# Lzcstan/DrugLAMP

Hardware: AMD Instinct MI355X
Metric: drug-protein pairs/sec training step (higher is better)
Workload: dtype bf16; 1 GPU; DrugLAMP training step (cls step, epoch 1; fwd+bwd+grad all-reduce+AdamW), BindingDB-shaped synthetic pairs (512 drug nodes/tokens, 2304 protein tokens = 256 sites, pre-extracted 384-d/640-d LLM embeddings), global batch 256 = 256 per GPU x 1; per_gpu_batch=256, global_batch=256, parallelism=dp1, step_kind=cls, epoch=1, hip_graph=False, protein_seq_len=2304, distinct_batches=8, first_touch_steps=8, padding_rows=computed once, protein_cnn_rows=distinct rows, streams=independent branches on side HIP streams

## Files before the change

### druglamp_amd/_lib.py

```python
from __future__ import annotations

import ctypes as C
import os

import torch

_HERE = os.path.dirname(os.path.abspath(__file__))
_variant = os.environ.get("DL_USE_STUDY_LIB", "")
if _variant and not _variant.endswith(".so"):
    raise RuntimeError("DL_USE_STUDY_LIB=%s: the -DDL_STUDY build (libdruglamp_hip_study.so) was removed; commit 97fb613 is the last "
                       "that builds it (python -m druglamp_amd.build --study).  Only a variant library name (libdruglamp_hip_<variant>.so) "
                       "is accepted." % _variant)
LIB_PATH = os.path.join(_HERE, "lib", _variant or "libdruglamp_hip.so")

DL_F32, DL_BF16 = 0, 1

c_i64, c_i32, c_f32, c_u64, c_vp, c_sz = C.c_int64, C.c_int32, C.c_float, C.c_uint64, C.c_void_p, C.c_size_t


class ReduceItem(C.Structure):
    _fields_ = [
        ("kind", c_i32), ("out_dtype", c_i32),
        ("src", c_vp), ("out", c_vp),
        ("mn", c_i64), ("ldc", c_i64),
        ("N", c_i32), ("splits", c_i32), ("accumulate", c_i32), ("M", c_i32),
        ("cs_slabs", c_vp), ("cs_out", c_vp),
    ]


REDUCE_BATCH_MAX = 24
GEMM_GROUP_MAX = 16


class GemmArgs(C.Structure):
    _fields_ = [
        ("X", c_vp), ("ldx", c_i64), ("x_kslow", c_i32),
        ("W", c_vp), ("ldw", c_i64), ("w_kslow", c_i32),
        ("C", c_vp), ("ldc", c_i64),
        ("M", c_i64), ("N", c_i64), ("K", c_i64),
        ("in_dtype", c_i32), ("out_dtype", c_i32),
        ("bias", c_vp),
        ("residual", c_vp), ("ldr", c_i64),
        ("res_row_mod", c_i64),
        ("res_before_dropout", c_i32),
        ("act", c_i32),
        ("pre_out", c_vp), ("ldp", c_i64),
        ("dact_pre", c_vp), ("lddp", c_i64),
        ("dropout_p", c_f32), ("dropout_seed", c_u64),
        ("accumulate", c_i32),
        ("split_k", c_i32), ("workspace", c_vp), ("workspace_bytes", c_sz),
        ("x_colsum", c_vp),
        ("dropout_seed_offset", c_vp),
        ("algo", c_i32),
        ("tile_tickets", c_vp),
        ("deferred", C.POINTER(ReduceItem)),
        ("prof_tag", c_i32),
    ]


FLAG_PROT_PERIOD, FLAG_DRUG_TOKEN_PAD, FLAG_GCN_NODE_PAD, FLAG_PLAN_ROWS, FLAG_PAIR_INDEX = 1, 2, 4, 8, 16
FLAG_KEY_TABLE = 32
TAG_OTHER, TAG_QKV_OUT, TAG_FFN, TAG_CONV, TAG_WGRAD, TAG_ADAPTOR = 0, 1, 2, 3, 4, 5
TAG_NAMES = {0: "other", 1: "qkv_out", 2: "ffn", 3: "conv", 4: "wgrad", 5: "adaptor"}


class AttnFwdArgs(C.Structure):
    _fields_ = [
        ("Q", c_vp), ("K", c_vp), ("V", c_vp), ("O", c_vp), ("LSE", c_vp), ("raw_logits", c_vp),
        ("q_ps", c_i64), ("q_hs", c_i64), ("q_rs", c_i64),
        ("k_ps", c_i64), ("k_hs", c_i64), ("k_rs", c_i64),
        ("v_ps", c_i64), ("v_hs", c_i64), ("v_rs", c_i64),
        ("o_ps", c_i64), ("o_hs", c_i64), ("o_rs", c_i64), ("o_ss", c_i64),
        ("n_problems", c_i32), ("n_heads", c_i32), ("n_segments", c_i32), ("partner_shift", c_i32),
        ("Lq", c_i32), ("Lk", c_i32), ("head_dim", c_i32), ("dtype", c_i32),
        ("scale", c_f32),
        ("algo", c_i32),
        ("key_tail_rows", c_i32), ("key_tail_weight", c_f32),
    ]


class AttnBwdArgs(C.Structure):
    _fields_ = [
        ("Q", c_vp), ("K", c_vp), ("V", c_vp), ("O", c_vp), ("dO", c_vp),
        ("LSE", c_vp), ("Delta", c_vp),
        ("dQ", c_vp), ("dK", c_vp), ("dV", c_vp),
        ("q_ps", c_i64), ("q_hs", c_i64), ("q_rs", c_i64),
        ("k_ps", c_i64), ("k_hs", c_i64), ("k_rs", c_i64),
        ("v_ps", c_i64), ("v_hs", c_i64), ("v_rs", c_i64),
        ("o_ps", c_i64), ("o_hs", c_i64), ("o_rs", c_i64), ("o_ss", c_i64),
        ("do_ps", c_i64), ("do_hs", c_i64), ("do_rs", c_i64), ("do_ss", c_i64),
        ("dq_ps", c_i64), ("dq_hs", c_i64), ("dq_rs", c_i64),
        ("dk_ps", c_i64), ("dk_hs", c_i64), ("dk_rs", c_i64),
        ("dv_ps", c_i64), ("dv_hs", c_i64), ("dv_rs", c_i64),
        ("n_problems", c_i32), ("n_heads", c_i32), ("n_segments", c_i32), ("partner_shift", c_i32),
        ("Lq", c_i32), ("Lk", c_i32), ("head_dim", c_i32), ("dtype", c_i32),
        ("scale", c_f32),
        ("algo", c_i32),
        ("key_tail_rows", c_i32), ("key_tail_weight", c_f32),
    ]


class AttnProbsArgs(C.Structure):
    _fields_ = [
        ("Q", c_vp), ("K", c_vp), ("LSE", c_vp), ("out", c_vp), ("out_ld", c_i64),
        ("q_ps", c_i64), ("q_hs", c_i64), ("q_rs", c_i64),
        ("k_ps", c_i64), ("k_hs", c_i64), ("k_rs", c_i64),
        ("n_problems", c_i32), ("n_heads", c_i32), ("n_segments", c_i32), ("partner_shift", c_i32),
        ("Lq", c_i32), ("Lk", c_i32), ("head_dim", c_i32), ("dtype", c_i32),
        ("scale", c_f32),
        ("head_mean", c_i32), ("key_tail_rows", c_i32), ("key_tail_weight", c_f32), ("expand_tail", c_i32),
        ("workspace", c_vp), ("workspace_bytes", c_sz),
    ]


class PgcaPairsArgs(C.Structure):
    _fields_ = [
        ("Q", c_vp), ("K", c_vp), ("V", c_vp), ("left", c_vp), ("out", c_vp), ("bias", c_vp),
        ("q_index", c_vp), ("kv_index", c_vp), ("flags", c_vp),
        ("q_es", c_i64), ("q_rs", c_i64), ("k_es", c_i64), ("k_rs", c_i64), ("v_es", c_i64), ("v_rs", c_i64),
        ("left_es", c_i64), ("left_rs", c_i64), ("out_ps", c_i64), ("out_rs", c_i64),
        ("n_pairs", c_i32), ("n_q", c_i32), ("n_kv", c_i32), ("Lq", c_i32), ("Lk", c_i32), ("head_dim", c_i32), ("dtype", c_i32),
        ("left_cols", c_i32), ("out_col0", c_i32),
        ("scale", c_f32),
        ("key_tail_rows", c_i32), ("key_tail_weight", c_f32),
    ]


class PgcaPairsRaggedArgs(C.Structure):
    _fields_ = [
        ("Q", c_vp), ("K", c_vp), ("V", c_vp), ("left", c_vp), ("out", c_vp), ("bias", c_vp),
        ("q_index", c_vp), ("kv_index", c_vp), ("kv_row0", c_vp), ("kv_keys", c_vp), ("kv_tail_weight", c_vp), ("flags", c_vp),
        ("q_es", c_i64), ("q_rs", c_i64), ("k_rs", c_i64), ("v_rs", c_i64),
        ("left_es", c_i64), ("left_rs", c_i64), ("out_ps", c_i64), ("out_rs", c_i64), ("kv_total_rows", c_i64),
        ("n_pairs", c_i32), ("n_q", c_i32), ("n_kv", c_i32), ("Lq", c_i32), ("head_dim", c_i32), ("dtype", c_i32),
        ("left_cols", c_i32), ("out_col0", c_i32),
        ("scale", c_f32),
        ("key_tail_rows", c_i32),
    ]


class NtxentSide(C.Structure):
    _fields_ = [("q", c_vp), ("k", c_vp), ("n", c_i64), ("gid_offset", c_i64), ("lse", c_vp)]


class NtxentArgs(C.Structure):
    _fields_ = [("a", NtxentSide), ("b", NtxentSide), ("n_global", c_i64), ("d", c_i64), ("dtype", c_i32),
                ("temperature", c_f32)]


SIGNATURES = {
    "dl_last_error": (C.c_char_p, []),
    "dl_version": (c_i32, []),
    "dl_gemm_workspace_bytes": (c_sz, [C.POINTER(GemmArgs)]),
    "dl_gemm": (c_i32, [C.POINTER(GemmArgs), c_vp]),
    "dl_gemm_pair": (c_i32, [C.POINTER(GemmArgs), C.POINTER(GemmArgs), c_vp]),
    "dl_gemm_group_plan": (c_i32, [C.POINTER(GemmArgs), c_i32, C.POINTER(c_i32)]),
    "dl_gemm_group": (c_i32, [C.POINTER(GemmArgs), c_i32, c_vp]),
    "dl_reduce_batch": (c_i32, [C.POINTER(ReduceItem), c_i32, c_vp]),
    "dl_colsum": (c_i32, [c_vp, c_i64, c_i64, c_i64, c_i32, c_vp, c_i32, c_vp, c_sz, c_vp]),
    "dl_colsum_workspace_bytes": (c_sz, [c_i64, c_i64]),
    "dl_bn_workspace_bytes": (c_sz, [c_i64, c_i64]),
    "dl_bn_stats": (c_i32, [c_vp, c_i64, c_i64, c_i64, c_i64, c_i64, c_i32, c_vp, c_vp, c_sz, c_vp]),
    "dl_bn_apply_fwd": (c_i32, [c_vp, c_vp, c_vp, c_vp, c_vp, c_vp, c_i64, c_i64, c_i64, c_i64, c_i64, c_i32, c_vp]),
    "dl_bn_bwd_reduce": (c_i32, [c_vp, c_vp, c_vp, c_vp, c_i64, c_i64, c_i64, c_i64, c_i64, c_i32, c_vp, c_vp, c_sz, c_vp]),
    "dl_bn_tail_fix": (c_i32, [c_vp, c_vp, c_vp, c_vp, c_vp, c_vp, c_f32, c_i32, c_i64, c_i64, c_i64, c_i64, c_i32, c_vp]),
    "dl_bn_apply_relu_fwd": (c_i32, [c_vp, c_vp, c_vp, c_vp, c_vp, c_vp, c_i64, c_i64, c_i32, c_vp]),
    "dl_bn_relu_bwd": (c_i32, [c_vp, c_vp, c_vp, c_vp, c_vp, c_vp, c_f32, c_vp, c_vp, c_i64, c_i64, c_i32, c_vp, c_sz, c_vp]),
    "dl_bn_bwd_apply": (c_i32, [c_vp, c_vp, c_vp, c_vp, c_vp, c_vp, c_f32, c_i32, c_vp, c_i64, c_i64, c_i64, c_i64, c_i64,
                                c_i32, c_vp]),
    "dl_layernorm_fwd": (c_i32, [c_vp, c_i64, c_vp, c_vp, c_vp, c_i64, c_vp, c_vp, c_i64, c_i64, c_f32, c_i32, c_vp]),
    "dl_layernorm_bwd_workspace_bytes": (c_sz, [c_i64, c_i64]),
    "dl_layernorm_bwd": (c_i32, [c_vp, c_i64, c_i64, c_vp, c_i64, c_vp, c_vp, c_vp, c_vp, c_i64, c_vp, c_i64, c_vp, c_vp,
                                 c_i32, c_i64, c_i64, c_i32, c_vp, c_sz, C.POINTER(ReduceItem), c_vp]),
    "dl_attn_fwd": (c_i32, [C.POINTER(AttnFwdArgs), c_vp]),
    "dl_attn_bwd": (c_i32, [C.POINTER(AttnBwdArgs), c_vp]),
    "dl_attn_probs_workspace_bytes": (c_sz, [C.POINTER(AttnProbsArgs)]),
    "dl_attn_probs": (c_i32, [C.POINTER(AttnProbsArgs), c_vp]),
    "dl_pgca_pairs_fwd": (c_i32, [C.POINTER(PgcaPairsArgs), c_vp]),
    "dl_pgca_pairs_ragged_fwd": (c_i32, [C.POINTER(PgcaPairsRaggedArgs), c_vp]),
    "dl_token_gate_fwd": (c_i32, [c_vp, c_vp, c_vp, c_vp, c_i64, c_i64, c_i64, c_i32, c_i32, c_i32, c_vp]),
    "dl_token_gate_bwd": (c_i32, [c_vp, c_vp, c_vp, c_vp, c_vp, c_i64, c_i64, c_i64, c_i32, c_i32, c_i32, c_vp]),
    "dl_gate_dpre": (c_i32, [c_vp, c_vp, c_vp, c_vp, c_i64, c_i64, c_i32, c_i32, c_vp]),
    "dl_add_rowmod_dropout": (c_i32, [c_vp, c_vp, c_vp, c_i64, c_i64, c_i64, c_f32, c_u64, c_vp, c_i32, c_vp]),
    "dl_dropout_apply": (c_i32, [c_vp, c_vp, c_i64, c_i64, c_i64, c_i64, c_f32, c_u64, c_vp, c_i32, c_vp]),
    "dl_fill_pool": (c_i32, [c_vp, c_vp, c_vp, c_i64, c_i64, c_i64, c_i32, c_i32, c_i32, c_vp]),
    "dl_cnn_sitepool_fwd": (c_i32, [c_vp, c_vp, c_i64, c_i64, c_i64, c_i32, c_i32, c_i32, c_vp]),
    "dl_cnn_sitepool_bwd": (c_i32, [c_vp, c_vp, c_i64, c_i64, c_i64, c_i32, c_i32, c_i32, c_vp]),
    "dl_bn_stats_finalize": (c_i32, [c_vp, c_i64, c_i64, c_i64, c_i64, c_i64, c_vp, c_i32, c_i64, c_f32, c_f32, c_vp, c_vp, c_vp, c_vp, c_vp, c_vp, c_vp, c_sz, c_vp]),
    "dl_bn_finalize": (c_i32, [c_vp, c_i64, c_f32, c_f32, c_vp, c_vp, c_vp, c_vp, c_vp, c_i64, c_vp]),
    "dl_interleave_streams": (c_i32, [c_vp, c_vp, c_i64, c_i64, c_i32, c_i32, c_vp]),
    "dl_norm_adjacency": (c_i32, [c_vp, c_vp, c_i64, c_i32, c_i32, c_vp]),
    "dl_graph_aggregate": (c_i32, [c_vp, c_vp, c_vp, c_i64, c_i32, c_i32, c_i32, c_i32, c_i32, c_vp]),
    "dl_concat2": (c_i32, [c_vp, c_vp, c_vp, c_i64, c_i64, c_i64, c_i32, c_vp]),
    "dl_gather_pad": (c_i32, [c_vp, c_vp, c_vp, c_vp, c_i64, c_i64, c_i64, c_i32, c_i32, c_vp]),
    "dl_embed_pad": (c_i32, [c_vp, c_vp, c_vp, c_vp, c_i64, c_i64, c_i32, c_i32, c_i32, c_i32, c_vp]),
    "dl_weight_prep": (c_i32, [c_vp, c_vp, c_i32, c_i32, c_vp]),
    "dl_gelu_bwd": (c_i32, [c_vp, c_vp, c_vp, c_i64, c_i32, c_vp]),
    "dl_cast": (c_i32, [c_vp, c_i32, c_vp, c_i32, c_i64, c_vp]),
    "dl_rowmod_sum": (c_i32, [c_vp, c_vp, c_i64, c_i64, c_i64, c_i32, c_i32, c_vp]),
    "dl_cos_rowloss_fwd": (c_i32, [c_vp, c_vp, c_vp, c_vp, c_i64, c_i64, c_vp]),
    "dl_cos_rowloss_bwd": (c_i32, [c_vp, c_vp, c_f32, c_vp, c_i64, c_i64, c_vp]),
    "dl_ntxent_fwd_ex": (c_i32, [C.POINTER(NtxentArgs), c_vp, c_vp, c_vp, c_vp]),
    "dl_ntxent_bwd_ex": (c_i32, [C.POINTER(NtxentArgs), c_f32, c_vp, c_vp, c_vp]),
    "dl_ntxent_workspace_bytes": (c_sz, [c_i64, c_i64]),
    "dl_ntxent_fwd": (c_i32, [c_vp, c_vp, c_i64, c_i64, c_f32, c_vp, c_vp, c_vp, c_sz, c_vp]),
    "dl_ntxent_bwd": (c_i32, [c_vp, c_vp, c_i64, c_i64, c_f32, c_vp, c_f32, c_vp, c_vp, c_vp]),
    "dl_triplet_sigcos_buffer_floats": (c_sz, [c_i64, c_i64]),
    "dl_triplet_sigcos_fwd": (c_i32, [c_vp, c_vp, c_vp, c_i64, c_i64, c_i64, c_f32, c_vp, c_vp, c_vp, c_vp]),
    "dl_triplet_sigcos_bwd": (c_i32, [c_vp, c_vp, c_vp, c_vp, c_i64, c_i64, c_i64, c_f32, c_vp, c_f32, c_vp, c_vp, c_vp]),
    "dl_adamw_step": (c_i32, [c_vp, c_vp, c_vp, c_vp, c_i64, c_f32, c_f32, c_f32, c_f32, c_f32, c_i64, c_f32, c_vp,
                              c_i32, c_vp]),
    "dl_bn_stats_rw": (c_i32, [c_vp, c_i64, c_i64, c_vp, c_i32, c_vp, c_vp, c_sz, c_vp]),
    "dl_bn_apply_fwd_rw": (c_i32, [c_vp, c_vp, c_vp, c_vp, c_vp, c_vp, c_i64, c_i64, c_vp, c_i32, c_vp]),
    "dl_bn_bwd_reduce_rw": (c_i32, [c_vp, c_vp, c_vp, c_vp, c_i64, c_i64, c_vp, c_i32, c_vp, c_vp, c_sz, c_vp]),
    "dl_bn_bwd_apply_rw": (c_i32, [c_vp, c_vp, c_vp, c_vp, c_vp, c_vp, c_f32, c_i32, c_vp, c_i64, c_i64, c_vp, c_i32, c_vp]),
    "dl_cnn_sitepool_rows_fwd": (c_i32, [c_vp, c_vp, c_vp, c_i64, c_i64, c_i64, c_i32, c_i32, c_vp]),
    "dl_cnn_sitepool_rows_bwd": (c_i32, [c_vp, c_vp, c_vp, c_vp, c_i64, c_i64, c_i64, c_i64, c_i32, c_i32, c_vp]),
    "dl_embed_rows": (c_i32, [c_vp, c_vp, c_vp, c_vp, c_vp, c_i64, c_i32, c_i32, c_vp, c_i64, c_i64, c_vp, c_i32, c_vp]),
    "dl_rows_gather": (c_i32, [c_vp, c_vp, c_vp, c_i64, c_i64, c_vp]),
    "dl_rows_sum_strided": (c_i32, [c_vp, c_vp, c_vp, c_i64, c_i64, c_i32, c_vp]),
    "dl_rows_equal_check": (c_i32, [c_vp, c_i64, c_i64, c_i64, c_i64, C.c_uint32, c_vp, c_vp]),
    "dl_ce_rows_workspace_bytes": (c_sz, [c_i64]),
    "dl_ce_rows_fwd": (c_i32, [c_vp, c_i64, c_vp, c_i64, c_i32, c_i64, c_i32, c_vp, c_vp, c_vp, c_sz, c_vp]),
    "dl_ce_rows_bwd": (c_i32, [c_vp, c_i64, c_vp, c_i64, c_i32, c_i64, c_i32, c_vp, c_vp, c_vp, c_vp, c_i64, c_i32, c_vp]),
    "dl_protein_plan_build": (c_i32, [c_vp, c_i64, c_i64, c_i64, c_vp, c_vp, c_vp, c_vp, c_vp, c_vp, c_vp]),
    "dl_prof_enable": (c_i32, [c_i32, c_i32]),
    "dl_prof_collect": (c_i32, [c_i32, C.POINTER(c_i64), C.POINTER(C.c_double), C.POINTER(C.c_double),
                                C.POINTER(C.c_double)]),
    "dl_prof_totals": (c_i32, [c_i32, C.POINTER(c_i64), C.POINTER(C.c_double), C.POINTER(C.c_double)]),
    "dl_prof_collect_tag": (c_i32, [c_i32, c_i32, C.POINTER(c_i64), C.POINTER(C.c_double), C.POINTER(C.c_double), C.POINTER(C.c_double),
                                    C.POINTER(c_i64), C.POINTER(C.c_double), C.POINTER(C.c_double)]),
}

_lib = None

AUDIT = os.environ.get("DL_GRAPH_PTR_AUDIT") == "1"
_audit_log = None


def audit_begin() -> None:
    global _audit_log
    _audit_log = []


def audit_end():
    global _audit_log
    log, _audit_log = _audit_log, None
    return log or []


def _struct_ptrs(obj, out, name):
    for fname, ftype in getattr(obj, "_fields_", []):
        v = getattr(obj, fname)
        if ftype is c_vp:
            if v:
                out.append(("%s.%s" % (name, fname), int(v)))
        elif isinstance(v, C.Structure):
            _struct_ptrs(v, out, "%s.%s" % (name, fname))


def _audited(name, fn, argtypes):
    def call(*args):
        if _audit_log is not None:
            import torch
            if torch.cuda.is_current_stream_capturing():
                found = []
                n_items = next((a for a, t in zip(args, argtypes) if t is c_i32), 0) if name == "dl_reduce_batch" else 0
                for i, (a, t) in enumerate(zip(args, argtypes)):
                    if t is c_vp:
                        v = a.value if isinstance(a, C.c_void_p) else a
                        if v:
                            found.append(("arg%d" % i, int(v)))
                    elif isinstance(a, C.Array):
                        for k in range(int(n_items) or len(a)):
                            _struct_ptrs(a[k], found, "arg%d[%d]" % (i, k))
                    elif isinstance(a, C.Structure):
                        _struct_ptrs(a, found, "arg%d" % i)
                    elif hasattr(a, "_obj") and isinstance(getattr(a, "_obj"), C.Structure):
                        _struct_ptrs(a._obj, found, "arg%d" % i)
                    elif hasattr(a, "contents") and a:
                        try:
                            _struct_ptrs(a.contents, found, "arg%d" % i)
                        except ValueError:
                            pass
                _audit_log.extend((name, w, v) for w, v in found)
        return fn(*args)
    return call


def lib():
    global _lib
    if _lib is None:
        if not os.path.exists(LIB_PATH):
            raise RuntimeError(
                "libdruglamp_hip.so is missing (%s). Build it with `python -m druglamp_amd.build`; "
                "the HIP hot path has no CPU fallback." % LIB_PATH)
        L = C.CDLL(LIB_PATH)
        for name, (res, args) in SIGNATURES.items():
            fn = getattr(L, name)
            fn.restype = res
            fn.argtypes = args
            if AUDIT and name not in ("dl_last_error", "dl_version") and not name.endswith("_bytes") and not name.endswith("_floats") \
                    and not name.startswith("dl_prof_"):
                setattr(L, name, _audited(name, fn, args))
        _lib = L
    return _lib


_DEBUG_SYNC = bool(os.environ.get("DL_DEBUG_SYNC"))


def check(rc: int, what: str = "") -> None:
    if _DEBUG_SYNC:
        import sys
        import torch
        print("[dl] %s" % what, file=sys.stderr, flush=True)
        torch.cuda.synchronize()
        print("[dl-ok] %s" % what, file=sys.stderr, flush=True)
    if rc != 0:
        msg = lib().dl_last_error()
        raise RuntimeError("druglamp_hip %s failed (status %d): %s" % (what, rc, msg.decode() if msg else "?"))
```

### druglamp_amd/csrc/norm.hip

```cpp
#include "common.cuh"

namespace {
constexpr int LN_MAXV = 8;
constexpr int LN_BWD_ROWS = 32;

constexpr int LN_FWD_RPW = 2;
template <typename T, int NV_>
__global__ __launch_bounds__(256) void ln_fwd_kernel(const T* __restrict__ x, int64_t ldx,
                                                     const float* __restrict__ gamma,
                                                     const float* __restrict__ beta, T* __restrict__ y,
                                                     int64_t ldy, float* __restrict__ mean_out,
                                                     float* __restrict__ rstd_out, int64_t M, int D,
                                                     float eps) {
  const int lane = threadIdx.x & 63, wave = threadIdx.x >> 6;
  const int64_t row0 = ((int64_t)blockIdx.x * 4 + wave) * LN_FWD_RPW;
  if (row0 >= M) return;
  const int nv = D >> 2;
  f32x4 v[LN_FWD_RPW][NV_];
#pragma unroll
  for (int r = 0; r < LN_FWD_RPW; ++r)
#pragma unroll
    for (int j = 0; j < NV_; ++j) {
      const int c = lane + 64 * j;
      v[r][j] = f32x4{0.f, 0.f, 0.f, 0.f};
      if (c < nv && row0 + r < M) v[r][j] = load4<T>(x + (row0 + r) * ldx + c * 4);
    }
  f32x4 gm[NV_], bt[NV_];
#pragma unroll
  for (int j = 0; j < NV_; ++j) {
    const int c = lane + 64 * j;
    gm[j] = bt[j] = f32x4{0.f, 0.f, 0.f, 0.f};
    if (c < nv) { gm[j] = *reinterpret_cast<const f32x4*>(gamma + c * 4); bt[j] = *reinterpret_cast<const f32x4*>(beta + c * 4); }
  }
#pragma unroll
  for (int r = 0; r < LN_FWD_RPW; ++r) {
    const int64_t row = row0 + r;
    if (row >= M) break;
    float s = 0.f;
#pragma unroll
    for (int j = 0; j < NV_; ++j) s += (v[r][j][0] + v[r][j][1]) + (v[r][j][2] + v[r][j][3]);
    const float mean = wave_sum(s) / (float)D;
    float q = 0.f;
#pragma unroll
    for (int j = 0; j < NV_; ++j) {
      const int c = lane + 64 * j;
      if (c < nv) {
#pragma unroll
        for (int e = 0; e < 4; ++e) { const float d = v[r][j][e] - mean; q += d * d; }
      }
    }
    const float var = wave_sum(q) / (float)D;
    const float rstd = rsqrtf(var + eps);
#pragma unroll
    for (int j = 0; j < NV_; ++j) {
      const int c = lane + 64 * j;
      if (c < nv) {
        f32x4 o;
#pragma unroll
        for (int e = 0; e < 4; ++e) o[e] = (v[r][j][e] - mean) * rstd * gm[j][e] + bt[j][e];
        store4<T>(y + row * ldy + c * 4, o);
      }
    }
    if (lane == 0) {
      if (mean_out) mean_out[row] = mean;
      if (rstd_out) rstd_out[row] = rstd;
    }
  }
}

template <typename T, int NV_>
__global__ __launch_bounds__(256) void ln_bwd_kernel(const T* __restrict__ dy, int64_t lddy, int64_t dy_share,
                                                     const T* __restrict__ x, int64_t ldx,
                                                     const float* __restrict__ mean,
                                                     const float* __restrict__ rstd,
                                                     const float* __restrict__ gamma,
                                                     const T* __restrict__ dres, int64_t lddres,
                                                     T* __restrict__ dx, int64_t lddx,
                                                     float* __restrict__ partial, int64_t M, int D) {
  extern __shared__ __attribute__((aligned(16))) char ln_smem[];
  float* sm = reinterpret_cast<float*>(ln_smem);
  const int lane = threadIdx.x & 63, wave = threadIdx.x >> 6;
  const int nv = D >> 2;
  f32x4 gm[NV_], dg[NV_], db[NV_];
#pragma unroll
  for (int j = 0; j < NV_; ++j) {
    const int c = lane + 64 * j;
    dg[j] = f32x4{0.f, 0.f, 0.f, 0.f};
    db[j] = f32x4{0.f, 0.f, 0.f, 0.f};
    gm[j] = (c < nv) ? *reinterpret_cast<const f32x4*>(gamma + c * 4) : f32x4{0.f, 0.f, 0.f, 0.f};
  }
  const int64_t r0 = (int64_t)blockIdx.x * LN_BWD_ROWS;
  for (int rr = wave; rr < LN_BWD_ROWS; rr += 8) {
    const int64_t rowA = r0 + rr, rowB = r0 + rr + 4;
    if (rowA >= M) break;
    const bool hasB = rowB < M;
    const int64_t dyA = dy_share == 1 ? rowA : rowA / dy_share, dyB = dy_share == 1 ? rowB : rowB / dy_share;
    f32x4 xa[NV_], da[NV_], xb[NV_], db_[NV_], ra[NV_], rb[NV_];
#pragma unroll
    for (int j = 0; j < NV_; ++j) {
      const int c = lane + 64 * j;
      ra[j] = f32x4{0.f, 0.f, 0.f, 0.f}; rb[j] = ra[j];
      if (c < nv) {
        xa[j] = load4<T>(x + rowA * ldx + c * 4);
        da[j] = load4<T>(dy + dyA * lddy + c * 4);
        if (dres) ra[j] = load4<T>(dres + rowA * lddres + c * 4);
        if (hasB) {
          xb[j] = load4<T>(x + rowB * ldx + c * 4);
          db_[j] = load4<T>(dy + dyB * lddy + c * 4);
          if (dres) rb[j] = load4<T>(dres + rowB * lddres + c * 4);
        }
      }
    }
#pragma unroll
    for (int half = 0; half < 2; ++half) {
      if (half == 1 && !hasB) break;
      const int64_t row = half == 0 ? rowA : rowB;
      const float mu = mean[row], rs = rstd[row];
      f32x4 xh[NV_], g[NV_];
      float c1 = 0.f, c2 = 0.f;
#pragma unroll
      for (int j = 0; j < NV_; ++j) {
        const int c = lane + 64 * j;
        if (c < nv) {
          const f32x4 xv = half == 0 ? xa[j] : xb[j];
          const f32x4 dv = half == 0 ? da[j] : db_[j];
#pragma unroll
          for (int e = 0; e < 4; ++e) {
            xh[j][e] = (xv[e] - mu) * rs;
            g[j][e] = dv[e] * gm[j][e];
            c1 += g[j][e];
            c2 += g[j][e] * xh[j][e];
            dg[j][e] += dv[e] * xh[j][e];
            db[j][e] += dv[e];
          }
        }
      }
      c1 = wave_sum(c1) / (float)D;
      c2 = wave_sum(c2) / (float)D;
#pragma unroll
      for (int j = 0; j < NV_; ++j) {
        const int c = lane + 64 * j;
        if (c < nv) {
          f32x4 o;
#pragma unroll
          for (int e = 0; e < 4; ++e) o[e] = rs * (g[j][e] - c1 - xh[j][e] * c2);
          o += half == 0 ? ra[j] : rb[j];
          store4<T>(dx + row * lddx + c * 4, o);
        }
      }
    }
  }
#pragma unroll
  for (int j = 0; j < NV_; ++j) {
    const int c = lane + 64 * j;
    if (c < nv) {
      *reinterpret_cast<f32x4*>(sm + (wave * 2 + 0) * D + c * 4) = dg[j];
      *reinterpret_cast<f32x4*>(sm + (wave * 2 + 1) * D + c * 4) = db[j];
    }
  }
  __syncthreads();
  for (int i = threadIdx.x; i < 2 * D; i += 256) {
    const int which = i / D, col = i % D;
    float s = 0.f;
#pragma unroll
    for (int w = 0; w < 4; ++w) s += sm[(w * 2 + which) * D + col];
    partial[((int64_t)blockIdx.x * 2 + which) * D + col] = s;
  }
}

template <int LPR> __device__ __forceinline__ float seg_sum(float v) {
  v = row16_sum(v);
  const float lo = lane_f32(v, 0) + lane_f32(v, 16), hi = lane_f32(v, 32) + lane_f32(v, 48);
  if constexpr (LPR == 64) return lo + hi;
  else return (threadIdx.x & 32) ? hi : lo;
}
__device__ __forceinline__ void unpack8(u32x4 w, float (&f)[8]) {
#pragma unroll
  for (int e = 0; e < 4; ++e) {
    f[2 * e] = bf16lo(w[e]); f[2 * e + 1] = bf16hi(w[e]);
#ifdef DL_UNPACK_NOP
    asm volatile("s_nop 1" : "+v"(f[2 * e]));
#endif
  }
}
__device__ __forceinline__ u32x4 pack8(const float (&f)[8]) {
  return u32x4{pack_bf16x2(f[0], f[1]), pack_bf16x2(f[2], f[3]), pack_bf16x2(f[4], f[5]), pack_bf16x2(f[6], f[7])};
}
constexpr int LN16_PASSES = 4;

template <int D>
__global__ __launch_bounds__(256) void ln_fwd16_kernel(const bf16_t* __restrict__ x, int64_t ldx, const float* __restrict__ gamma,
                                                       const float* __restrict__ beta, bf16_t* __restrict__ y, int64_t ldy,
                                                       float* __restrict__ mean_out, float* __restrict__ rstd_out, int64_t M, float eps) {
  constexpr int LPR = D / 8, RPP = 64 / LPR, P = LN16_PASSES;
  const int lane = threadIdx.x & 63, wave = threadIdx.x >> 6, sub = lane / LPR, cl = lane % LPR;
  const int64_t row0 = ((int64_t)blockIdx.x * 4 + wave) * (RPP * P) + sub;
  u32x4 w[P];
#pragma unroll
  for (int q = 0; q < P; ++q) {
    const int64_t row = row0 + q * RPP;
    w[q] = u32x4{0u, 0u, 0u, 0u};
    if (row < M) w[q] = *reinterpret_cast<const u32x4*>(x + row * ldx + cl * 8);
  }
  float gm[8], bt[8];
  { const f32x4 a = *reinterpret_cast<const f32x4*>(gamma + cl * 8), b = *reinterpret_cast<const f32x4*>(gamma + cl * 8 + 4);
    const f32x4 c = *reinterpret_cast<const f32x4*>(beta + cl * 8), d = *reinterpret_cast<const f32x4*>(beta + cl * 8 + 4);
#pragma unroll
    for (int e = 0; e < 4; ++e) { gm[e] = a[e]; gm[4 + e] = b[e]; bt[e] = c[e]; bt[4 + e] = d[e]; } }
#pragma unroll
  for (int q = 0; q < P; ++q) {
    const int64_t row = row0 + q * RPP;
    float v[8];
    unpack8(w[q], v);
    float s = 0.f;
#pragma unroll
    for (int e = 0; e < 8; ++e) s += v[e];
    const float mean = seg_sum<LPR>(s) * (1.0f / D);
    float sq = 0.f;
#pragma unroll
    for (int e = 0; e < 8; ++e) { const float d = v[e] - mean; sq += d * d; }
    const float rstd = rsqrtf(seg_sum<LPR>(sq) * (1.0f / D) + eps);
    if (row < M) {
      float o[8];
#pragma unroll
      for (int e = 0; e < 8; ++e) o[e] = (v[e] - mean) * rstd * gm[e] + bt[e];
      store16_fam<1>(y + row * ldy + cl * 8, pack8(o));
      if (cl == 0) {
        if (mean_out) mean_out[row] = mean;
        if (rstd_out) rstd_out[row] = rstd;
      }
    }
  }
}

template <int D>
__global__ __launch_bounds__(256) void ln_bwd16_kernel(const bf16_t* __restrict__ dy, int64_t lddy, int64_t dy_share,
                                                       const bf16_t* __restrict__ x, int64_t ldx, const float* __restrict__ mean,
                                                       const float* __restrict__ rstd, const float* __restrict__ gamma,
                                                       const bf16_t* __restrict__ dres, int64_t lddres, bf16_t* __restrict__ dx,
                                                       int64_t lddx, float* __restrict__ partial, int64_t M) {
  constexpr int LPR = D / 8, RPP = 64 / LPR, P = LN16_PASSES, NIT = LN_BWD_ROWS / (4 * RPP * P);
  static_assert(NIT >= 1 && NIT * 4 * RPP * P == LN_BWD_ROWS, "a workgroup covers LN_BWD_ROWS rows");
  __shared__ __attribute__((aligned(16))) float sm[4 * RPP * 2 * D];
  const int lane = threadIdx.x & 63, wave = threadIdx.x >> 6, sub = lane / LPR, cl = lane % LPR;
  float gm[8], dg[8], db[8];
  { const f32x4 a = *reinterpret_cast<const f32x4*>(gamma + cl * 8), b = *reinterpret_cast<const f32x4*>(gamma + cl * 8 + 4);
#pragma unroll
    for (int e = 0; e < 4; ++e) { gm[e] = a[e]; gm[4 + e] = b[e]; } }
#pragma unroll
  for (int e = 0; e < 8; ++e) { dg[e] = 0.f; db[e] = 0.f; }
#pragma unroll 1
  for (int it = 0; it < NIT; ++it) {
    const int64_t row0 = (int64_t)blockIdx.x * LN_BWD_ROWS + (it * 4 + wave) * (RPP * P) + sub;
    u32x4 wx[P], wd[P], wr[P];
    float mu[P], rs[P];
#pragma unroll
    for (int q = 0; q < P; ++q) {
      const int64_t row = row0 + q * RPP;
      wx[q] = wd[q] = wr[q] = u32x4{0u, 0u, 0u, 0u};
      mu[q] = 0.f; rs[q] = 0.f;
      if (row < M) {
        const int64_t dr = dy_share == 1 ? row : row / dy_share;
        wx[q] = (DL_NT_MASK & 16) ? load16_nt(x + row * ldx + cl * 8) : *reinterpret_cast<const u32x4*>(x + row * ldx + cl * 8);
        wd[q] = *reinterpret_cast<const u32x4*>(dy + dr * lddy + cl * 8);
        if (dres) wr[q] = *reinterpret_cast<const u32x4*>(dres + row * lddres + cl * 8);
        mu[q] = mean[row]; rs[q] = rstd[row];
      }
    }
#pragma unroll
    for (int q = 0; q < P; ++q) {
      const int64_t row = row0 + q * RPP;
      float xv[8], dv[8], g[8];
      unpack8(wx[q], xv);
      unpack8(wd[q], dv);
      float c1 = 0.f, c2 = 0.f;
#pragma unroll
      for (int e = 0; e < 8; ++e) {
        xv[e] = (xv[e] - mu[q]) * rs[q];
        g[e] = dv[e] * gm[e];
        c1 += g[e];
        c2 += g[e] * xv[e];
        dg[e] += dv[e] * xv[e];
        db[e] += dv[e];
      }
      c1 = seg_sum<LPR>(c1) * (1.0f / D);
      c2 = seg_sum<LPR>(c2) * (1.0f / D);
      if (row < M) {
        float rv[8], o[8];
        unpack8(wr[q], rv);
#pragma unroll
        for (int e = 0; e < 8; ++e) o[e] = rs[q] * (g[e] - c1 - xv[e] * c2) + rv[e];
        store16_fam<1>(dx + row * lddx + cl * 8, pack8(o));
      }
    }
  }
  float* mine = sm + (size_t)(wave * RPP + sub) * 2 * D;
  *reinterpret_cast<f32x4*>(mine + cl * 8) = f32x4{dg[0], dg[1], dg[2], dg[3]};
  *reinterpret_cast<f32x4*>(mine + cl * 8 + 4) = f32x4{dg[4], dg[5], dg[6], dg[7]};
  *reinterpret_cast<f32x4*>(mine + D + cl * 8) = f32x4{db[0], db[1], db[2], db[3]};
  *reinterpret_cast<f32x4*>(mine + D + cl * 8 + 4) = f32x4{db[4], db[5], db[6], db[7]};
  __syncthreads();
  for (int i = threadIdx.x; i < 2 * D; i += 256) {
    float s = 0.f;
#pragma unroll
    for (int w = 0; w < 4 * RPP; ++w) s += sm[(size_t)w * 2 * D + i];
    partial[(int64_t)blockIdx.x * 2 * D + i] = s;
  }
}

}

extern "C" int dl_layernorm_fwd(const void* x, int64_t ldx, const float* gamma, const float* beta,
                                void* y, int64_t ldy, float* mean, float* rstd, int64_t M, int64_t D,
                                float eps, int32_t dtype, dl_stream stream) {
  hipStream_t s = (hipStream_t)stream;
  DL_CHECK_ARG(x && y && gamma && beta, DL_ERR_ARG, "dl_layernorm_fwd: null pointer");
  DL_CHECK_ARG(M > 0 && D > 0 && D % 4 == 0 && D <= 256 * LN_MAXV, DL_ERR_SHAPE,
               "dl_layernorm_fwd: D=%ld must be a multiple of 4 and <= %d", (long)D, 256 * LN_MAXV);
  DL_CHECK_ARG(ldx % 4 == 0 && ldy % 4 == 0, DL_ERR_ALIGN, "dl_layernorm_fwd: ld must be multiple of 4");
  const uint32_t blocks = (uint32_t)((M + 4 * LN_FWD_RPW - 1) / (4 * LN_FWD_RPW));
  dl_prof_before(3, s);
  if (dtype == DL_BF16 && (D == 256 || D == 512) && ldx % 8 == 0 && ldy % 8 == 0 && (((uintptr_t)x | (uintptr_t)y) & 15) == 0 &&
      (((uintptr_t)gamma | (uintptr_t)beta) & 15) == 0) {
    if (D == 256) {
      constexpr int RPB = 4 * 2 * LN16_PASSES;
      const uint32_t nb = (uint32_t)((M + RPB - 1) / RPB);
      hipLaunchKernelGGL((ln_fwd16_kernel<256>), dim3(nb), dim3(256), 0, s, (const bf16_t*)x, ldx, gamma, beta, (bf16_t*)y, ldy, mean, rstd, M, eps);
    } else {
      constexpr int RPB = 4 * 1 * LN16_PASSES;
      const uint32_t nb = (uint32_t)((M + RPB - 1) / RPB);
      hipLaunchKernelGGL((ln_fwd16_kernel<512>), dim3(nb), dim3(256), 0, s, (const bf16_t*)x, ldx, gamma, beta, (bf16_t*)y, ldy, mean, rstd, M, eps);
    }
    DL_CHECK_LAUNCH("dl_layernorm_fwd");
    dl_prof_after(3, s, 8.0 * M * D, 2.0 * M * D * dl_dtype_size(dtype));
    return DL_OK;
  }
#define LN_FWD(TT, NVV) hipLaunchKernelGGL((ln_fwd_kernel<TT, NVV>), dim3(blocks), dim3(256), 0, s, (const TT*)x, ldx, \
                                          gamma, beta, (TT*)y, ldy, mean, rstd, M, (int)D, eps)
  const int nvg = (int)((D + 255) / 256);
  if (dtype == DL_BF16) { if (nvg <= 1) LN_FWD(bf16_t, 1); else if (nvg <= 2) LN_FWD(bf16_t, 2); else if (nvg <= 4) LN_FWD(bf16_t, 4); else LN_FWD(bf16_t, 8); }
  else { if (nvg <= 1) LN_FWD(float, 1); else if (nvg <= 2) LN_FWD(float, 2); else if (nvg <= 4) LN_FWD(float, 4); else LN_FWD(float, 8); }
#undef LN_FWD
  DL_CHECK_LAUNCH("dl_layernorm_fwd");
  dl_prof_after(3, s, 8.0 * M * D, 2.0 * M * D * dl_dtype_size(dtype));
  return DL_OK;
}

extern "C" size_t dl_layernorm_bwd_workspace_bytes(int64_t M, int64_t D) {
  const int64_t nb = (M + LN_BWD_ROWS - 1) / LN_BWD_ROWS;
  return (size_t)nb * 2 * (size_t)D * sizeof(float);
}

extern "C" int dl_layernorm_bwd(const void* dy, int64_t lddy, int64_t dy_share, const void* x, int64_t ldx,
                                const float* mean, const float* rstd, const float* gamma,
                                const void* dres, int64_t lddres, void* dx, int64_t lddx, float* dgamma,
                                float* dbeta, int32_t accumulate, int64_t M, int64_t D, int32_t dtype,
                                void* workspace, size_t workspace_bytes, dl_reduce_item* deferred, dl_stream stream) {
  hipStream_t s = (hipStream_t)stream;
  if (deferred) deferred->kind = DL_REDUCE_NONE;
  DL_CHECK_ARG(dy && x && mean && rstd && gamma && dx, DL_ERR_ARG, "dl_layernorm_bwd: null pointer");
  DL_CHECK_ARG(dy_share >= 1, DL_ERR_ARG, "dl_layernorm_bwd: dy_share=%ld must be >= 1", (long)dy_share);
  DL_CHECK_ARG(M > 0 && D > 0 && D % 4 == 0 && D <= 256 * LN_MAXV, DL_ERR_SHAPE,
               "dl_layernorm_bwd: D=%ld must be a multiple of 4 and <= %d", (long)D, 256 * LN_MAXV);
  DL_CHECK_ARG(workspace && workspace_bytes >= dl_layernorm_bwd_workspace_bytes(M, D),
               DL_ERR_WORKSPACE, "dl_layernorm_bwd: workspace too small");
  const int nb = (int)((M + LN_BWD_ROWS - 1) / LN_BWD_ROWS);
  const size_t smem = 4 * 2 * (size_t)D * sizeof(float);
#define LN_BWD(TT, NVV) hipLaunchKernelGGL((ln_bwd_kernel<TT, NVV>), dim3(nb), dim3(256), smem, s, (const TT*)dy, lddy, dy_share, \
                                          (const TT*)x, ldx, mean, rstd, gamma, (const TT*)dres, lddres, (TT*)dx, lddx, \
                                          (float*)workspace, M, (int)D)
  const int nvg = (int)((D + 255) / 256);
  const bool v16 = dtype == DL_BF16 && (D == 256 || D == 512) && lddy % 8 == 0 && ldx % 8 == 0 && lddx % 8 == 0 &&
                   (!dres || lddres % 8 == 0) && (((uintptr_t)dy | (uintptr_t)x | (uintptr_t)dx | (uintptr_t)dres | (uintptr_t)gamma) & 15) == 0;
  if (v16 && D == 256)
    hipLaunchKernelGGL((ln_bwd16_kernel<256>), dim3(nb), dim3(256), 0, s, (const bf16_t*)dy, lddy, dy_share, (const bf16_t*)x, ldx, mean, rstd,
                       gamma, (const bf16_t*)dres, lddres, (bf16_t*)dx, lddx, (float*)workspace, M);
  else if (v16)
    hipLaunchKernelGGL((ln_bwd16_kernel<512>), dim3(nb), dim3(256), 0, s, (const bf16_t*)dy, lddy, dy_share, (const bf16_t*)x, ldx, mean, rstd,
                       gamma, (const bf16_t*)dres, lddres, (bf16_t*)dx, lddx, (float*)workspace, M);
  else
  if (dtype == DL_BF16) { if (nvg <= 1) LN_BWD(bf16_t, 1); else if (nvg <= 2) LN_BWD(bf16_t, 2); else if (nvg <= 4) LN_BWD(bf16_t, 4); else LN_BWD(bf16_t, 8); }
  else { if (nvg <= 1) LN_BWD(float, 1); else if (nvg <= 2) LN_BWD(float, 2); else if (nvg <= 4) LN_BWD(float, 4); else LN_BWD(float, 8); }
#undef LN_BWD
  DL_CHECK_LAUNCH("dl_layernorm_bwd");
  if (dgamma && dbeta == dgamma + D && deferred) {
    dl_reduce_item& it = *deferred;
    it.kind = DL_REDUCE_PARTIALS; it.out_dtype = DL_F32; it.src = (const float*)workspace; it.out = dgamma;
    it.mn = 2 * D; it.ldc = 0; it.N = (int32_t)(2 * D); it.splits = nb; it.accumulate = accumulate; it.M = 0;
    it.cs_slabs = nullptr; it.cs_out = nullptr;
    return DL_OK;
  }
  if (dgamma && dbeta == dgamma + D) {
    hipLaunchKernelGGL(dl_reduce_partials_kernel, dim3((uint32_t)((2 * D + DL_REDUCE_COLS - 1) / DL_REDUCE_COLS)), dim3(1024), 0, s,
                       (const float*)workspace, nb, (int64_t)(2 * D), (int)(2 * D), dgamma, accumulate);
  } else {
    if (dgamma)
      hipLaunchKernelGGL(dl_reduce_partials_kernel, dim3((uint32_t)((D + DL_REDUCE_COLS - 1) / DL_REDUCE_COLS)), dim3(1024), 0, s,
                         (const float*)workspace, nb, (int64_t)(2 * D), (int)D, dgamma, accumulate);
    if (dbeta)
      hipLaunchKernelGGL(dl_reduce_partials_kernel, dim3((uint32_t)((D + DL_REDUCE_COLS - 1) / DL_REDUCE_COLS)), dim3(1024), 0, s,
                         (const float*)workspace + D, nb, (int64_t)(2 * D), (int)D, dbeta, accumulate);
  }
  DL_CHECK_LAUNCH("dl_layernorm_bwd(final)");
  return DL_OK;
}
```

### druglamp_amd/functional.py

```python
from __future__ import annotations

import functools
import contextlib
import os
import math
import weakref
from typing import List, Optional, Sequence

import torch

from . import ops

_param_epoch = 0
def _maybe_deferring():
    return contextlib.nullcontext() if os.environ.get("DL_DEFER_REDUCTIONS", "1") == "0" else ops.deferred_reductions()


def _deferring(fn):
    if os.environ.get("DL_DEFER_REDUCTIONS", "1") == "0":
        return fn

    @functools.wraps(fn)
    def wrapped(*a, **k):
        with ops.deferred_reductions():
            return fn(*a, **k)
    return wrapped


_lowp_cache = {}
_lowp_tables = {}
_lowp_retired = []
_derived_cache = {}


def bump_param_epoch() -> None:
    global _param_epoch
    _param_epoch += 1


def planned_image_count() -> int:
    return sum(1 for e in _lowp_cache.values() if e.planned)


class _LowpEntry:
    __slots__ = ("refs", "transpose", "dtype", "image", "versions", "epoch", "planned", "pad", "conv")

    def __init__(self, params, transpose, dtype, image, planned, pad=None, conv=None):
        self.refs = tuple(weakref.ref(p) for p in params)
        self.transpose, self.dtype, self.image, self.planned, self.pad = transpose, dtype, image, planned, pad
        self.conv = conv
        self.versions = tuple(p._version for p in params)
        self.epoch = _param_epoch

    def params(self):
        ps = tuple(r() for r in self.refs)
        return None if any(p is None for p in ps) else ps


def _build_conv_image(w, dtype, backward):
    with torch.no_grad():
        co, ci, k = w.shape
        g = w.detach().flip(2).permute(1, 2, 0).reshape(ci, k * co) if backward else w.detach().permute(0, 2, 1).reshape(co, k * ci)
        g = g.contiguous()
        return ops.cast(g, dtype) if g.dtype != dtype else g


def _build_image(params, dtype, transpose, pad=None):
    with torch.no_grad():
        w = params[0].detach() if len(params) == 1 else torch.cat([p.detach() for p in params], dim=0)
        if pad is not None:
            g = torch.zeros(pad, dtype=w.dtype, device=w.device)
            g[:w.shape[0], :w.shape[1]] = w
            w = g
        if transpose:
            w = w.t().contiguous()
        if w.dtype != dtype:
            w = ops.cast(w, dtype)
        elif not w.is_contiguous():
            w = w.contiguous()
    return w


def _refresh_all_images() -> None:
    import numpy as np
    groups = {}
    for key in list(_lowp_cache.keys()):
        e = _lowp_cache[key]
        ps = e.params()
        if ps is None:
            del _lowp_cache[key]
            continue
        if not e.planned:
            e.image = _build_conv_image(ps[0], e.dtype, e.conv == "b") if e.conv else _build_image(ps, e.dtype, e.transpose, e.pad)
            e.versions, e.epoch = tuple(p._version for p in ps), _param_epoch
            continue
        groups.setdefault((ps[0].device, e.dtype), []).append((e, ps))
    item_t = np.dtype([("src", "<u8"), ("dst", "<u8"), ("ld", "<i8"), ("rows", "<i4"), ("cols", "<i4"),
                       ("row0", "<i4"), ("transpose", "<i4"), ("cs", "<i8")])
    for gkey, lst in groups.items():
        tab = _lowp_tables.get(gkey)
        sig = tuple(id(e) for e, _ in lst) + tuple(p.data_ptr() for _, ps in lst for p in ps)
        if tab is None or tab[0] != sig:
            items, bmap = [], []
            for e, ps in lst:
                if e.conv:
                    co, ci, k = ps[0].shape
                    for o in range(co):
                        src = ps[0].data_ptr() + o * ci * k * 4
                        if e.conv == "f":
                            items.append((src, e.image.data_ptr(), 1, ci, k, o * k * ci, 2, ci))
                        else:
                            items.append((src, e.image.data_ptr(), k * co, ci, k, (k - 1) * co + o, 2, -co))
                        ntile = ((ci + 63) // 64) * ((k + 63) // 64)
                        bmap.extend((len(items) - 1, t) for t in range(ntile))
                    continue
                row0 = 0
                for p_ in ps:
                    r, c = p_.shape if p_.dim() == 2 else (1, p_.shape[0])
                    ld = e.image.shape[1] if e.image.dim() == 2 else c
                    items.append((p_.data_ptr(), e.image.data_ptr(), ld, r, c, row0, 1 if e.transpose else 0, 0))
                    ntile = ((r + 63) // 64) * ((c + 63) // 64)
                    bmap.extend((len(items) - 1, t) for t in range(ntile))
                    row0 += r
            items_np = np.array(items, dtype=item_t)
            items_dev = torch.from_numpy(items_np.view(np.uint8).copy()).to(gkey[0])
            bmap_dev = torch.tensor(bmap, dtype=torch.int32).reshape(-1).to(gkey[0])
            if tab is not None:
                _lowp_retired.append(tab)
            tab = (sig, items_dev, bmap_dev, len(bmap))
            _lowp_tables[gkey] = tab
        ops.weight_prep(tab[1], tab[2], tab[3], gkey[1])
        for e, ps in lst:
            e.versions, e.epoch = tuple(p._version for p in ps), _param_epoch


def refresh_images() -> None:
    _refresh_all_images()


def ensure_images_current() -> None:
    if any(e.epoch != _param_epoch for e in _lowp_cache.values()):
        _refresh_all_images()


def lowp(params: Sequence[torch.Tensor], dtype: torch.dtype, transpose: bool = False, pad=None) -> torch.Tensor:
    if len(params) == 1 and not transpose and pad is None and params[0].dtype == dtype:
        return params[0].detach()
    key = (tuple(id(p) for p in params) + (("T",) if transpose else ()) + (("pad",) + tuple(pad) if pad else ()), dtype)
    e = _lowp_cache.get(key)
    if e is not None and all(r() is p for r, p in zip(e.refs, params)):
        if e.epoch != _param_epoch or e.versions != tuple(p._version for p in params):
            _refresh_all_images()
        return e.image
    planned = all(p.dim() == 2 and p.dtype == torch.float32 and p.is_contiguous() and p.is_cuda for p in params) or \
        (not transpose and pad is None and len({p.shape for p in params}) == 1 and
         all(p.dim() == 1 and p.dtype == torch.float32 and p.is_contiguous() and p.is_cuda for p in params))
    if len(_lowp_cache) > 4096:
        _lowp_retired.append((dict(_lowp_cache), dict(_lowp_tables)))
        _lowp_cache.clear()
        _lowp_tables.clear()
    image = _build_image(params, dtype, transpose, pad)
    _lowp_cache[key] = _LowpEntry(params, transpose, dtype, image, planned, pad)
    return image


def _f32(t: Optional[torch.Tensor]) -> Optional[torch.Tensor]:
    return None if t is None else t.detach()


def _n_params(paired: bool) -> int:
    return 18 if paired else 16


class _Stream:

    def __init__(self, ps: Sequence[torch.Tensor], paired: bool, cdt: torch.dtype):
        it = iter(ps)
        self.ln1w, self.ln1b = next(it), next(it)
        qw, qb, kw, kb, vw, vb = (next(it) for _ in range(6))
        self.qkv_w = lowp((qw, kw, vw), cdt)
        self.qkv_wT = lowp((qw, kw, vw), cdt, True)
        self.qkv_b = lowp((qb, kb, vb), torch.float32)
        if paired:
            fw, fb = next(it), next(it)
            self.fc_w, self.fc_b = lowp((fw,), cdt), _f32(fb)
            self.fc_wT = lowp((fw,), cdt, True)
        ow, ob = next(it), next(it)
        self.out_w, self.out_b = lowp((ow,), cdt), _f32(ob)
        self.out_wT = lowp((ow,), cdt, True)
        self.ln2w, self.ln2b = next(it), next(it)
        w1, b1, w2, b2 = (next(it) for _ in range(4))
        self.w1, self.b1 = lowp((w1,), cdt), _f32(b1)
        self.w2, self.b2 = lowp((w2,), cdt), _f32(b2)
        self.w1T, self.w2T = lowp((w1,), cdt, True), lowp((w2,), cdt, True)


from ._lib import TAG_QKV_OUT as _TAG_QKV_OUT, TAG_FFN as _TAG_FFN, TAG_CONV as _TAG_CONV, TAG_ADAPTOR as _TAG_ADAPTOR

PAIR_GEMMS = os.environ.get("DL_PAIR_GEMMS", "1") != "0"
GATE_DPRE_KERNEL = os.environ.get("DL_GATE_DPRE", "1") != "0"


def _gemm_s(xs, ws, **kw):
    if len(xs) == 2 and PAIR_GEMMS:
        return list(ops.gemm_pair(xs, ws, **kw))
    if len(xs) == 2:
        return [ops.gemm(xs[i], ws[i], **{k: (v[i] if isinstance(v, (tuple, list)) else v) for k, v in kw.items()}) for i in range(2)]
    return [ops.gemm(xs[0], ws[0], **{k: (v[0] if isinstance(v, (tuple, list)) else v) for k, v in kw.items()})]


class TransformerBlockFn(torch.autograd.Function):

    @staticmethod
    def forward(ctx, x, paired, H, p_drop, training, eps, *params):
        S, B, L, d = x.shape
        assert S == (2 if paired else 1)
        cdt = x.dtype
        M = B * L
        npar = _n_params(paired)
        streams = [_Stream(params[s * npar:(s + 1) * npar], paired, cdt) for s in range(S)]
        x = x.contiguous()
        xs = [x[s].reshape(M, d) for s in range(S)]
        nseg = 2 if paired else 1
        hd = d // H
        p_eff = float(p_drop) if (training and p_drop > 0) else 0.0

        qkv = torch.empty((S, M, 3 * d), dtype=cdt, device=x.device)
        xn, stats1 = [], []
        for s, st in enumerate(streams):
            y, mean, rstd = ops.layernorm_fwd(xs[s], st.ln1w.detach(), st.ln1b.detach(), eps)
            xn.append(y)
            stats1.append((mean, rstd))
        with ops.prof_tag(_TAG_QKV_OUT):
            _gemm_s(xn, [st.qkv_w for st in streams], M=M, N=3 * d, K=d, bias=[st.qkv_b for st in streams],
                    out=[qkv[s] for s in range(S)])
        a = torch.empty((S, M, nseg * d), dtype=cdt, device=x.device)
        qs = (L * 3 * d, hd, 3 * d)
        os_ = (L * nseg * d, hd, nseg * d)
        lse = ops.attn_fwd(qkv, qkv[..., d:], qkv[..., 2 * d:], n_problems=S * B, n_heads=H, n_segments=nseg,
                           partner_shift=B if paired else 0, Lq=L, Lk=L, head_dim=hd, scale=1.0 / math.sqrt(hd),
                           q_strides=qs, k_strides=qs, v_strides=qs, out=a, o_strides=os_, o_ss=d)
        out = torch.empty_like(x)
        saved: List[torch.Tensor] = [x, qkv, a, lse]
        seeds = [((ops.next_seed(), ops.next_seed()) if p_eff > 0 else (0, 0)) for _ in range(S)]
        with ops.prof_tag(_TAG_QKV_OUT):
            if paired:
                f = _gemm_s([a[s] for s in range(S)], [st.fc_w for st in streams], M=M, N=d, K=2 * d, bias=[st.fc_b for st in streams])
            else:
                f = [a[s] for s in range(S)]
            x1 = _gemm_s(f, [st.out_w for st in streams], M=M, N=d, K=d, bias=[st.out_b for st in streams], residual=xs)
        ln2 = [ops.layernorm_fwd(x1[s], st.ln2w.detach(), st.ln2b.detach(), eps) for s, st in enumerate(streams)]
        hn = [t[0] for t in ln2]
        pre = [torch.empty((M, 4 * d), dtype=cdt, device=x.device) for _ in range(S)]
        with ops.prof_tag(_TAG_FFN):
            act = _gemm_s(hn, [st.w1 for st in streams], M=M, N=4 * d, K=d, bias=[st.b1 for st in streams], act=1, pre_out=pre,
                          dropout_p=p_eff, seed=[sd[0] for sd in seeds])
            _gemm_s(act, [st.w2 for st in streams], M=M, N=d, K=4 * d, bias=[st.b2 for st in streams], dropout_p=p_eff,
                    seed=[sd[1] for sd in seeds], residual=x1, out=[out[s].reshape(M, d) for s in range(S)])
        for s, st in enumerate(streams):
            saved += [xn[s], stats1[s][0], stats1[s][1], f[s], x1[s], hn[s], ln2[s][1], ln2[s][2], pre[s], act[s],
                      st.qkv_wT, st.out_wT, st.w1T, st.w2T, st.fc_wT if paired else st.out_wT,
                      st.ln1w.detach(), st.ln2w.detach()]
        ctx.save_for_backward(*saved)
        ctx.cfg = (paired, H, p_eff, S, B, L, d, seeds)
        return out

    @staticmethod
    @_deferring
    def backward(ctx, dout):
        paired, H, p_eff, S, B, L, d, seeds = ctx.cfg
        sv = ctx.saved_tensors
        x, qkv, a, lse = sv[:4]
        per = 17
        M = B * L
        nseg = 2 if paired else 1
        hd = d // H
        cdt = x.dtype
        dout = dout.contiguous()
        da = torch.empty_like(a)
        SV = [sv[4 + s * per: 4 + (s + 1) * per] for s in range(S)]
        col = lambda i: [SV[s][i] for s in range(S)]
        (xn_, _m1, _r1, f_, x1_, hn_, mean2_, rstd2_, pre_, act_, qkvw_, outw_, w1_, w2_, fcw_, _l1, ln2w_) = [col(i) for i in range(per)]
        dys = [dout[s].reshape(M, d) for s in range(S)]
        g2 = [ops.dropout_apply(dys[s], p_eff, seeds[s][1]) if p_eff > 0 else dys[s] for s in range(S)]
        wg2 = [_wgrad(g2[s], act_[s], d, 4 * d, M, d, 4 * d) for s in range(S)]
        with ops.prof_tag(_TAG_FFN):
            g1 = _gemm_s(g2, w2_, M=M, N=4 * d, K=d, dact_pre=pre_, dropout_p=p_eff, seed=[seeds[s][0] for s in range(S)])
            wg1 = [_wgrad(g1[s], hn_[s], 4 * d, d, M, 4 * d, d) for s in range(S)]
            dhn = _gemm_s(g1, w1_, M=M, N=d, K=4 * d)
        lnb = [ops.layernorm_bwd(dhn[s], x1_[s], mean2_[s], rstd2_[s], ln2w_[s], dres=dys[s]) for s in range(S)]
        dx1_all = [t[0] for t in lnb]
        wgo = [_wgrad(dx1_all[s], f_[s], d, d, M, d, d) for s in range(S)]
        grads_tail = []
        _tag_qo = ops.prof_tag(_TAG_QKV_OUT)
        _tag_qo.__enter__()
        if paired:
            df = _gemm_s(dx1_all, outw_, M=M, N=d, K=d)
            wgf = [_wgrad(df[s], a[s], d, 2 * d, M, d, 2 * d) for s in range(S)]
            _gemm_s(df, fcw_, M=M, N=2 * d, K=d, out=[da[s] for s in range(S)])
            for s in range(S):
                grads_tail.append((wgf[s][0], wgf[s][1], wgo[s][0], wgo[s][1], lnb[s][1], lnb[s][2], wg1[s][0], wg1[s][1],
                                   wg2[s][0], wg2[s][1]))
        else:
            _gemm_s(dx1_all, outw_, M=M, N=d, K=d, out=[da[s] for s in range(S)])
            for s in range(S):
                grads_tail.append((wgo[s][0], wgo[s][1], lnb[s][1], lnb[s][2], wg1[s][0], wg1[s][1], wg2[s][0], wg2[s][1]))
        _tag_qo.__exit__(None, None, None)
        dqkv = torch.empty_like(qkv)
        qs = (L * 3 * d, hd, 3 * d)
        os_ = (L * nseg * d, hd, nseg * d)
        ops.attn_bwd(qkv, qkv[..., d:], qkv[..., 2 * d:], a, da, lse, n_problems=S * B, n_heads=H, n_segments=nseg,
                     partner_shift=B if paired else 0, Lq=L, Lk=L, head_dim=hd, scale=1.0 / math.sqrt(hd),
                     q_strides=qs, k_strides=qs, v_strides=qs, o_strides=os_, o_ss=d, do_strides=os_, do_ss=d,
                     dq=dqkv, dq_strides=qs, dk=dqkv[..., d:], dk_strides=qs, dv=dqkv[..., 2 * d:], dv_strides=qs)
        dx = torch.empty_like(x)
        out_grads: List[Optional[torch.Tensor]] = []
        wgq = [_wgrad(dqkv[s], xn_[s], 3 * d, d, M, 3 * d, d) for s in range(S)]
        with ops.prof_tag(_TAG_QKV_OUT):
            dxn = _gemm_s([dqkv[s] for s in range(S)], qkvw_, M=M, N=d, K=3 * d)
        for s in range(S):
            dwqkv, dbqkv = wgq[s]
            _, dg1, dbt1 = ops.layernorm_bwd(dxn[s], x[s].reshape(M, d), SV[s][1], SV[s][2], SV[s][15], dres=dx1_all[s],
                                             out=dx[s].reshape(M, d))
            out_grads += [dg1, dbt1, dwqkv[0:d], dbqkv[0:d], dwqkv[d:2 * d], dbqkv[d:2 * d], dwqkv[2 * d:],
                          dbqkv[2 * d:]]
            out_grads += list(grads_tail[s])
        return (dx, None, None, None, None, None) + tuple(out_grads)


def transformer_block(x, paired: bool, H: int, p_drop: float, training: bool, eps: float, params):
    return TransformerBlockFn.apply(x, paired, H, p_drop, training, eps, *params)


class LinearFn(torch.autograd.Function):

    @staticmethod
    def forward(ctx, x, weight, bias, pe, p_drop, training):
        cdt = x.dtype
        K, N = x.shape[-1], weight.shape[0]
        x2 = x.reshape(-1, K).contiguous()
        M = x2.shape[0]
        w = lowp((weight,), cdt)
        wT = lowp((weight,), cdt, transpose=True) if (ctx.needs_input_grad[0] and cdt == torch.bfloat16 and N % 8 == 0) else None
        p_eff = float(p_drop) if (training and p_drop > 0) else 0.0
        seed = ops.next_seed() if p_eff > 0 else 0
        if pe is None:
            y = ops.gemm(x2, w, M=M, N=N, K=K, bias=_f32(bias))
        else:
            pe2 = lowp((pe,), cdt).reshape(-1, N)
            y = ops.gemm(x2, w, M=M, N=N, K=K, bias=_f32(bias), residual=pe2, res_row_mod=pe2.shape[0],
                         res_before_dropout=True, dropout_p=p_eff, seed=seed)
        ctx.save_for_backward(x2, w, wT)
        ctx.cfg = (x.shape, M, N, K, p_eff, seed, bias is not None, None if pe is None else tuple(pe.shape))
        return y.reshape(*x.shape[:-1], N)

    @staticmethod
    def backward(ctx, dy):
        x2, w, wT = ctx.saved_tensors
        xshape, M, N, K, p_eff, seed, has_bias, pe_shape = ctx.cfg
        g = dy.reshape(M, N).contiguous()
        if p_eff > 0:
            g = ops.dropout_apply(g, p_eff, seed)
        dx = None
        if ctx.needs_input_grad[0]:
            dx = (ops.gemm(g, wT, M=M, N=K, K=N) if wT is not None else ops.gemm(g, w, M=M, N=K, K=N, w_kslow=True, ldw=K)).reshape(xshape)
        want_b = has_bias and ctx.needs_input_grad[2]
        if ctx.needs_input_grad[1]:
            dw, db = _wgrad(g, x2, N, K, M, N, K, want_bias=want_b)
        else:
            dw, db = None, (ops.colsum(g) if want_b else None)
        dpe = None
        if pe_shape is not None and ctx.needs_input_grad[3]:
            dpe = ops.rowmod_sum(g, pe_shape[-2]).reshape(pe_shape)
        return dx, dw, db, dpe, None, None


def linear(x, weight, bias=None):
    return LinearFn.apply(x, weight, bias, None, 0.0, False)


class AddPeDropoutFn(torch.autograd.Function):

    @staticmethod
    def forward(ctx, x, pe, p_drop, training):
        D = x.shape[-1]
        x2 = x.reshape(-1, D).contiguous()
        p_eff = float(p_drop) if (training and p_drop > 0) else 0.0
        seed = ops.next_seed() if p_eff > 0 else 0
        y = ops.add_rowmod_dropout(x2, lowp((pe,), x.dtype).reshape(-1, D), p_eff, seed)
        ctx.cfg = (x.shape, tuple(pe.shape), p_eff, seed)
        return y.reshape(x.shape)

    @staticmethod
    def backward(ctx, dy):
        xshape, pe_shape, p_eff, seed = ctx.cfg
        D = xshape[-1]
        g = dy.reshape(-1, D).contiguous()
        if p_eff > 0:
            g = ops.dropout_apply(g, p_eff, seed)
        dpe = ops.rowmod_sum(g, pe_shape[-2]).reshape(pe_shape) if ctx.needs_input_grad[1] else None
        return g.reshape(xshape), dpe, None, None


class LayerNormFn(torch.autograd.Function):
    @staticmethod
    def forward(ctx, x, weight, bias, eps):
        D = x.shape[-1]
        x2 = x.reshape(-1, D).contiguous()
        y, mean, rstd = ops.layernorm_fwd(x2, weight.detach(), bias.detach(), eps)
        ctx.save_for_backward(x2, mean, rstd, weight.detach())
        ctx.shape = x.shape
        return y.reshape(x.shape)

    @staticmethod
    def backward(ctx, dy):
        x2, mean, rstd, w = ctx.saved_tensors
        if dy.dim() == 3 and dy.stride(1) == 0 and dy.stride(2) == 1 and dy.shape[1] > 1:
            dx, dg, db = ops.layernorm_bwd(dy[:, 0], x2, mean, rstd, w, dy_share=dy.shape[1])
        else:
            dx, dg, db = ops.layernorm_bwd(dy.reshape(x2.shape).contiguous(), x2, mean, rstd, w)
        return dx.reshape(ctx.shape), dg, db, None


def layer_norm(x, weight, bias, eps):
    return LayerNormFn.apply(x, weight, bias, eps)


class GuidedCrossAttentionFn(torch.autograd.Function):

    @staticmethod
    def forward(ctx, query, key, in_w, in_b, out_w, out_b, H, need_raw, key_tail=None, need_probs=False):
        if need_raw and need_probs:
            raise ValueError("GuidedCrossAttentionFn: need_raw and need_probs are alternatives for the second output")
        Lq, B, E = query.shape
        Lk = key.shape[0]
        cdt = query.dtype
        hd = E // H
        q2 = query.transpose(0, 1).contiguous().view(B * Lq, E)
        k2 = key.transpose(0, 1).contiguous().view(B * Lk, E)
        w = lowp((in_w,), cdt)
        b = _f32(in_b)
        qp = ops.gemm(q2, w[:E], M=B * Lq, N=E, K=E, bias=None if b is None else b[:E])
        kv = ops.gemm(k2, w[E:], M=B * Lk, N=2 * E, K=E, bias=None if b is None else b[E:])
        o = torch.empty((B * Lq, E), dtype=cdt, device=query.device)
        raw = torch.empty((B, H, Lq, Lk), dtype=torch.float32, device=query.device) if need_raw else None
        scale = float(hd) ** -0.5
        lse = ops.attn_fwd(qp, kv, kv[:, E:], n_problems=B, n_heads=H, n_segments=1, partner_shift=0, Lq=Lq, Lk=Lk,
                           head_dim=hd, scale=scale, q_strides=(Lq * E, hd, E), k_strides=(Lk * 2 * E, hd, 2 * E),
                           v_strides=(Lk * 2 * E, hd, 2 * E), out=o, o_strides=(Lq * E, hd, E), o_ss=0, raw_logits=raw,
                           key_tail=key_tail)
        if need_probs:
            raw = ops.attn_probs(qp, kv, lse=lse, head_mean=True, key_tail=key_tail, expand_tail=key_tail is not None,
                                 n_problems=B, n_heads=H, n_segments=1, partner_shift=0, Lq=Lq, Lk=Lk, head_dim=hd, scale=scale,
                                 q_strides=(Lq * E, hd, E), k_strides=(Lk * 2 * E, hd, 2 * E))[0]
        ow = lowp((out_w,), cdt)
        y = ops.gemm(o, ow, M=B * Lq, N=E, K=E, bias=_f32(out_b))
        wT = lowp((in_w,), cdt, transpose=True) if cdt == torch.bfloat16 else None
        owT = lowp((out_w,), cdt, transpose=True) if cdt == torch.bfloat16 else None
        ctx.save_for_backward(q2, k2, w, qp, kv, o, lse, ow, wT, owT)
        if key_tail is not None and need_raw:
            raise ValueError("GuidedCrossAttentionFn: the raw logits are those of all key rows; not available with key_tail")
        ctx.cfg = (Lq, Lk, B, E, H, scale, in_b is not None, out_b is not None, key_tail)
        ctx.mark_non_differentiable(*([raw] if raw is not None else []))
        ctx.set_materialize_grads(False)
        return y.view(B, Lq, E).transpose(0, 1), raw

    @staticmethod
    @_deferring
    def backward(ctx, dy, _draw):
        q2, k2, w, qp, kv, o, lse, ow, wT, owT = ctx.saved_tensors
        Lq, Lk, B, E, H, scale, has_inb, has_outb, key_tail = ctx.cfg
        hd = E // H
        g = dy.transpose(0, 1).contiguous().view(B * Lq, E)
        dwo, dbo = _wgrad(g, o, E, E, Lq * B, E, E, want_bias=has_outb)
        do = ops.gemm(g, owT, M=Lq * B, N=E, K=E) if owT is not None else ops.gemm(g, ow, M=Lq * B, N=E, K=E, w_kslow=True, ldw=E)
        dqp = torch.empty_like(qp)
        dkv = torch.empty_like(kv)
        ops.attn_bwd(qp, kv, kv[:, E:], o, do, lse, n_problems=B, n_heads=H, n_segments=1, partner_shift=0, Lq=Lq,
                     Lk=Lk, head_dim=hd, scale=scale, q_strides=(Lq * E, hd, E), k_strides=(Lk * 2 * E, hd, 2 * E),
                     v_strides=(Lk * 2 * E, hd, 2 * E), o_strides=(Lq * E, hd, E), o_ss=0, do_strides=(Lq * E, hd, E),
                     do_ss=0, dq=dqp, dq_strides=(Lq * E, hd, E), dk=dkv, dk_strides=(Lk * 2 * E, hd, 2 * E),
                     dv=dkv[:, E:], dv_strides=(Lk * 2 * E, hd, 2 * E), key_tail=key_tail)
        din_w = torch.empty((3 * E, E), dtype=torch.float32, device=g.device)
        din_b = torch.empty(3 * E, dtype=torch.float32, device=g.device) if has_inb else None
        _wgrad(dqp, q2, E, E, Lq * B, E, E, want_bias=has_inb, out_w=din_w[:E], out_b=None if din_b is None else din_b[:E])
        _wgrad(dkv, k2, 2 * E, E, Lk * B, 2 * E, E, want_bias=has_inb, out_w=din_w[E:], out_b=None if din_b is None else din_b[E:])
        if wT is not None:
            dquery = ops.gemm(dqp, wT, M=Lq * B, N=E, K=E, ldw=3 * E).view(B, Lq, E).transpose(0, 1)
            dkey = ops.gemm(dkv, wT[:, E:], M=Lk * B, N=E, K=2 * E, ldw=3 * E).view(B, Lk, E).transpose(0, 1)
        else:
            dquery = ops.gemm(dqp, w[:E], M=Lq * B, N=E, K=E, w_kslow=True, ldw=E).view(B, Lq, E).transpose(0, 1)
            dkey = ops.gemm(dkv, w[E:], M=Lk * B, N=E, K=2 * E, w_kslow=True, ldw=E).view(B, Lk, E).transpose(0, 1)
        return dquery, dkey, din_w, din_b, dwo, dbo, None, None, None, None


class TokenGateFn(torch.autograd.Function):

    @staticmethod
    def forward(ctx, v, w1, b1, w2, b2, H, add_residual):
        B, L, D = v.shape
        cdt = v.dtype
        M = B * L
        dd = w1.shape[0]
        v2 = v.reshape(M, D).contiguous()
        lw1, lw2 = lowp((w1,), cdt), lowp((w2,), cdt)
        pre = torch.empty((M, dd), dtype=cdt, device=v.device)
        hid = ops.gemm(v2, lw1, M=M, N=dd, K=D, bias=_f32(b1), act=1, pre_out=pre)
        logits = ops.gemm(hid, lw2, M=M, N=H, K=dd, bias=_f32(b2))
        out, gate = ops.token_gate_fwd(v2.reshape(B, L, D), logits.reshape(B, L, H), H, add_residual)
        ctx.save_for_backward(v2, lw1, lw2, pre, hid, gate)
        ctx.cfg = (B, L, D, H, dd, add_residual)
        ctx.w1, ctx.w2 = w1, w2
        return out

    @staticmethod
    @_deferring
    def backward(ctx, dout):
        v2, lw1, lw2, pre, hid, gate = ctx.saved_tensors
        B, L, D, H, dd, add_residual = ctx.cfg
        M = B * L
        cdt = v2.dtype
        dv_gate, dlogits = ops.token_gate_bwd(dout.contiguous(), v2.reshape(B, L, D), gate, H, add_residual)
        dl2 = dlogits.reshape(M, H)
        dw2, db2 = _wgrad(dl2, hid, H, dd, M, H, dd)
        if GATE_DPRE_KERNEL and H == 8 and dd % 8 == 0 and dd <= 2048 and dl2.is_contiguous():
            dpre = ops.gate_dpre(dl2, lw2, pre)
        elif cdt == torch.bfloat16 and H <= 64 and dd % 8 == 0:
            dl2p = torch.zeros((M, 64), dtype=cdt, device=dl2.device)
            dl2p[:, :H] = dl2
            w2t = lowp((ctx.w2,), cdt, transpose=True, pad=(64, dd))
            dpre = ops.gemm(dl2p, w2t, M=M, N=dd, K=64, dact_pre=pre)
        else:
            dpre = ops.gemm(dl2, lw2, M=M, N=dd, K=H, w_kslow=True, ldw=dd, dact_pre=pre)
        dw1, db1 = _wgrad(dpre, v2, dd, D, M, dd, D)
        dv = ops.gemm(dpre, lowp((ctx.w1,), cdt, transpose=True), M=M, N=D, K=dd, residual=dv_gate.reshape(M, D))
        return dv.reshape(B, L, D), dw1, db1, dw2, db2, None, None


def _cast_keep_layout(x: torch.Tensor, dtype: torch.dtype) -> torch.Tensor:
    if x.is_contiguous():
        return ops.cast(x, dtype)
    perm = sorted(range(x.dim()), key=lambda i: -x.stride(i))
    xp = x.permute(perm)
    if not xp.is_contiguous():
        return ops.cast(x.contiguous(), dtype)
    inv = [0] * len(perm)
    for i, d in enumerate(perm):
        inv[d] = i
    return ops.cast(xp, dtype).permute(inv)


class CastFn(torch.autograd.Function):
    @staticmethod
    def forward(ctx, x, dtype):
        ctx.src = x.dtype
        return _cast_keep_layout(x, dtype)

    @staticmethod
    def backward(ctx, dy):
        return _cast_keep_layout(dy, ctx.src), None


def cast(x: torch.Tensor, dtype: torch.dtype) -> torch.Tensor:
    return x if x.dtype == dtype else CastFn.apply(x, dtype)


@torch.no_grad()
def attention_maps(x, blk, H: int, paired: bool):
    S, B, L, d = x.shape
    hd = d // H
    M = B * L
    maps = []
    qkvs = []
    for s in range(S):
        ps = blk.stream_params(s)
        xn, _, _ = ops.layernorm_fwd(x[s].reshape(M, d).contiguous(), ps[0].detach(), ps[1].detach(), 1e-6)
        w = lowp((ps[2], ps[4], ps[6]), x.dtype)
        b = lowp((ps[3], ps[5], ps[7]), torch.float32)
        qkvs.append(ops.gemm(xn, w, M=M, N=3 * d, K=d, bias=b))
    qs = (L * 3 * d, hd, 3 * d)

    def raw_of(qbuf, kbuf):
        raw = torch.empty((B, H, L, L), dtype=torch.float32, device=x.device)
        scratch = torch.empty((M, d), dtype=x.dtype, device=x.device)
        ops.attn_fwd(qbuf, kbuf[:, d:], kbuf[:, 2 * d:], n_problems=B, n_heads=H, n_segments=1, partner_shift=0, Lq=L,
                     Lk=L, head_dim=hd, scale=1.0 / math.sqrt(hd), q_strides=qs, k_strides=qs, v_strides=qs,
                     out=scratch, o_strides=(L * d, hd, d), o_ss=0, need_lse=False, raw_logits=raw)
        return torch.softmax(raw, dim=-1)

    w = raw_of(qkvs[0], qkvs[0])
    gw = raw_of(qkvs[1], qkvs[0]) if paired else None
    return w, gw


def _wgrad(g, x, M, N, K, ldx, ldw, want_bias=True, out_w=None, out_b=None):
    db = (out_b if out_b is not None else torch.empty(M, dtype=torch.float32, device=g.device)) if want_bias else None
    dw = ops.gemm(g, x, M=M, N=N, K=K, x_kslow=True, w_kslow=True, ldx=ldx, ldw=ldw, out_dtype=torch.float32,
                  split_k=0, x_colsum=db, out=out_w)
    return dw, db


class CosRowLossFn(torch.autograd.Function):

    @staticmethod
    def forward(ctx, x, y):
        x = x.float().contiguous()
        y = y.detach().float().contiguous()
        rows = ops.cos_rowloss_fwd(x, y)
        ctx.save_for_backward(x, y)
        return rows

    @staticmethod
    def backward(ctx, drows):
        x, y = ctx.saved_tensors
        dx = ops.cos_rowloss_bwd(x, y, 1.0)
        return dx * drows.unsqueeze(-1), None


class CrossEntropyRowsFn(torch.autograd.Function):

    @staticmethod
    def forward(ctx, logits, labels, C, ignore_index):
        logits = logits if logits.stride(-1) == 1 else logits.contiguous()
        labels = labels.reshape(-1).contiguous()
        out2, lse = ops.ce_rows_fwd(logits, labels, C, ignore_index)
        ctx.save_for_backward(logits, labels, lse, out2)
        ctx.cfg = (C, ignore_index)
        return out2[0]

    @staticmethod
    def backward(ctx, g):
        logits, labels, lse, out2 = ctx.saved_tensors
        C, ignore_index = ctx.cfg
        return ops.ce_rows_bwd(logits, labels, C, ignore_index, lse, out2, g.float().contiguous()), None, None, None


class NTXentFn(torch.autograd.Function):

    @staticmethod
    def forward(ctx, q, k, temperature, global_batch=False):
        import torch.distributed as dist
        if q.dtype not in (torch.float32, torch.bfloat16):
            q = q.float()
        q = q.contiguous()
        k = k.to(q.dtype).contiguous()
        world = dist.get_world_size() if (global_batch and dist.is_available() and dist.is_initialized()) else 1
        n = q.shape[0]
        if world > 1:
            rank = dist.get_rank()
            qa = torch.empty((world * n, q.shape[1]), dtype=q.dtype, device=q.device)
            ka = torch.empty_like(qa)
            dist.all_gather_into_tensor(qa, q)
            dist.all_gather_into_tensor(ka, k)
            loss, lse, _ = ops.ntxent_fwd_ex(q, k, qa, ka, rank * n, 0, world * n, temperature)
            ctx.save_for_backward(q, k, lse, qa, ka)
            ctx.dist = (rank, world)
        else:
            loss, lse, _ = ops.ntxent_fwd_ex(q, k, q, k, 0, 0, n, temperature)
            ctx.save_for_backward(q, k, lse)
            ctx.dist = None
        ctx.t = temperature
        return loss.reshape(())

    @staticmethod
    def backward(ctx, dl):
        t = ctx.t
        if ctx.dist is None:
            q, k, lse = ctx.saved_tensors
            n = q.shape[0]
            dq, dk = ops.ntxent_bwd_ex(q, k, q, k, 0, 0, n, t, lse, lse, 1.0 / (2 * n))
            return (dq * dl).to(q.dtype), (dk * dl).to(k.dtype), None, None
        import torch.distributed as dist
        q, k, lse, qa, ka = ctx.saved_tensors
        rank, world = ctx.dist
        n = q.shape[0]
        gs = 1.0 / (2 * n)
        dq, dk = ops.ntxent_bwd_ex(q, k, qa, ka, rank * n, 0, world * n, t, lse, None, gs)
        dqa, dka = ops.ntxent_bwd_ex(qa, ka, q, k, 0, rank * n, world * n, t, None, lse, gs)
        both = torch.stack((dqa, dka)).reshape(2, world, n, -1).transpose(0, 1).contiguous()
        mine = torch.empty((2, n, q.shape[1]), dtype=torch.float32, device=q.device)
        if dist.get_backend() == "gloo":
            dist.all_reduce(both, op=dist.ReduceOp.SUM)
            mine.copy_(both[rank])
        else:
            dist.reduce_scatter_tensor(mine, both, op=dist.ReduceOp.SUM)
        return ((dq + mine[0]) * dl).to(q.dtype), ((dk + mine[1]) * dl).to(k.dtype), None, None


class TripletSigCosFn(torch.autograd.Function):

    @staticmethod
    def forward(ctx, p_lats, d_lats, gt, margin):
        p = p_lats.float().contiguous()
        d = d_lats.float().contiguous()
        loss, ntri, buf = ops.triplet_sigcos_fwd(p, d, gt, margin)
        ctx.save_for_backward(p, d, gt, buf, ntri)
        ctx.margin = margin
        return loss.reshape(())

    @staticmethod
    def backward(ctx, dl):
        p, d, gt, buf, ntri = ctx.saved_tensors
        dp, dd = ops.triplet_sigcos_bwd(p, d, gt, ctx.margin, buf, ntri, 1.0)
        return dp * dl, dd * dl, None, None


_CNN_HALO = 4


def _conv_weight(w: torch.Tensor, dtype: torch.dtype, backward: bool) -> torch.Tensor:
    key = ((id(w), "convb" if backward else "convf"), dtype)
    e = _lowp_cache.get(key)
    if e is not None and e.refs[0]() is w:
        if e.epoch != _param_epoch or e.versions != (w._version,):
            _refresh_all_images()
        return e.image
    planned = w.dim() == 3 and w.dtype == torch.float32 and w.is_contiguous() and w.is_cuda
    image = _build_conv_image(w, dtype, backward)
    _lowp_cache[key] = _LowpEntry((w,), False, dtype, image, planned, None, "b" if backward else "f")
    return image


class ProteinCNNFn(torch.autograd.Function):

    @staticmethod
    def forward(ctx, x, training, eps, pool_site_len, momenta, raw_dx, rw, n_stat, *params):
        if rw is not None:
            if x.dim() != 2 or pool_site_len:
# ... 523 lines not shown
```

### druglamp_amd/model/PMMA.py

```python
from __future__ import annotations

import copy

import torch
import torch.nn as nn

from .. import functional as Fn


def _cfg_get(cfg, name):
    return cfg[name] if isinstance(cfg, dict) and name in cfg else getattr(cfg, name)


class Attention(nn.Module):

    def __init__(self, config, vis, mm=True):
        super().__init__()
        self.vis = vis
        hs = config.hidden_size
        self.num_attention_heads = _cfg_get(config.transformer, "num_heads")
        self.attn_head_size = int(hs / self.num_attention_heads)
        self.query, self.key, self.value = nn.Linear(hs, hs), nn.Linear(hs, hs), nn.Linear(hs, hs)
        if mm:
            self.query_mol, self.key_mol, self.value_mol = nn.Linear(hs, hs), nn.Linear(hs, hs), nn.Linear(hs, hs)
            self.out_mol = nn.Linear(hs, hs)
            self.fc = nn.Linear(hs * 2, hs)
            self.fc_mol = nn.Linear(hs * 2, hs)
        self.out = nn.Linear(hs, hs)


class Mlp(nn.Module):

    def __init__(self, config):
        super().__init__()
        self.fc1 = nn.Linear(config.hidden_size, config.hidden_size * 4)
        self.fc2 = nn.Linear(config.hidden_size * 4, config.hidden_size)
        nn.init.xavier_uniform_(self.fc1.weight)
        nn.init.xavier_uniform_(self.fc2.weight)
        nn.init.normal_(self.fc1.bias, std=1e-6)
        nn.init.normal_(self.fc2.bias, std=1e-6)


class PMMABlock(nn.Module):

    def __init__(self, config, vis, mm=False):
        super().__init__()
        self.hidden_size = config.hidden_size
        self.mm = mm
        self.attention_norm = nn.LayerNorm(config.hidden_size, eps=1e-6)
        self.ffn_norm = nn.LayerNorm(config.hidden_size, eps=1e-6)
        if mm:
            self.att_norm_mol = nn.LayerNorm(config.hidden_size, eps=1e-6)
            self.ffn_norm_mol = nn.LayerNorm(config.hidden_size, eps=1e-6)
            self.ffn_mol = Mlp(config)
        self.ffn = Mlp(config)
        self.attn = Attention(config, vis, mm)

    def stream_params(self, s: int):
        a = self.attn
        if s == 0:
            ln1, ln2, ffn = self.attention_norm, self.ffn_norm, self.ffn
            q, k, v, out = a.query, a.key, a.value, a.out
            fc = a.fc if self.mm else None
        else:
            ln1, ln2, ffn = self.att_norm_mol, self.ffn_norm_mol, self.ffn_mol
            q, k, v, out, fc = a.query_mol, a.key_mol, a.value_mol, a.out_mol, a.fc_mol
        ps = [ln1.weight, ln1.bias, q.weight, q.bias, k.weight, k.bias, v.weight, v.bias]
        if fc is not None:
            ps += [fc.weight, fc.bias]
        ps += [out.weight, out.bias, ln2.weight, ln2.bias, ffn.fc1.weight, ffn.fc1.bias, ffn.fc2.weight, ffn.fc2.bias]
        return ps


class Embeddings(nn.Module):

    def __init__(self, config, mol_len):
        super().__init__()
        self.embedding = nn.Linear(config.hidden_size, config.hidden_size)
        self.mol_embeddings = nn.Linear(config.hidden_size, config.hidden_size)
        self.pe_prot = nn.Parameter(torch.zeros(1, config.feat_len, config.hidden_size))
        self.pe_mol = nn.Parameter(torch.zeros(1, mol_len, config.hidden_size))
        self.p_drop = _cfg_get(config.transformer, "dropout_rate")


class Encoder(nn.Module):

    def __init__(self, config, vis):
        super().__init__()
        self.vis = vis
        self.layer_with_mol = nn.ModuleList()
        self.encoder_norm = nn.LayerNorm(config.hidden_size * 2, eps=1e-6)
        for i in range(_cfg_get(config.transformer, "num_p_plus_s_layers")):
            if i < 2:
                layer = PMMABlock(config, vis, mm=True)
            else:
                if i == 2:
                    config.hidden_size = config.hidden_size * 2
                layer = PMMABlock(config, vis)
            self.layer_with_mol.append(copy.deepcopy(layer))


class PairedMultimodelAttention(nn.Module):

    def __init__(self, config, vis=True):
        super().__init__()
        self.num_heads = _cfg_get(config.transformer, "num_heads")
        self.p_drop = _cfg_get(config.transformer, "dropout_rate")
        self.embeddings = Embeddings(config, mol_len=config.mol_len)
        self.encoder = Encoder(config, vis)
        self.vis = vis
        self.compute_dtype = torch.float32
        self.keep_compute_dtype = False

    def forward(self, prot, mol=None):
        if mol is None:
            raise ValueError("PairedMultimodelAttention needs both streams (the reference's mol=None path "
                             "fails at encoder.py:50 as well)")
        if prot.shape != mol.shape:
            raise RuntimeError("PMMA paired attention needs equal-shaped streams, got %s and %s"
                               % (tuple(prot.shape), tuple(mol.shape)))
        cdt = self.compute_dtype
        emb, enc = self.embeddings, self.encoder
        H, p, tr = self.num_heads, self.p_drop, self.training
        prot = Fn.cast(prot, cdt)
        mol = Fn.cast(mol, cdt)
        mol = Fn.LinearFn.apply(mol, emb.mol_embeddings.weight, emb.mol_embeddings.bias, emb.pe_mol, p, tr)
        prot = Fn.AddPeDropoutFn.apply(prot, emb.pe_prot, p, tr)
        x = torch.stack((prot, mol), dim=0)
        attn_maps, guided_maps = [], []
        for i, blk in enumerate(enc.layer_with_mol):
            if i < 2:
                if self.vis:
                    w, gw = Fn.attention_maps(x, blk, H, paired=True)
                    attn_maps.append(w)
                    guided_maps.append(gw)
                x = Fn.transformer_block(x, True, H, p, tr, 1e-6, blk.stream_params(0) + blk.stream_params(1))
            else:
                if i == 2:
                    x = _concat_streams(x)
                if self.vis:
                    w, _ = Fn.attention_maps(x, blk, H, paired=False)
                    attn_maps.append(w)
                    guided_maps.append(None)
                x = Fn.transformer_block(x, False, H, p, tr, 1e-6, blk.stream_params(0))
        if x.shape[0] == 2:
            x = _concat_streams(x)
        encoded = Fn.layer_norm(x.reshape(x.shape[1:]), enc.encoder_norm.weight, enc.encoder_norm.bias, 1e-6)
        return (encoded if self.keep_compute_dtype else Fn.cast(encoded, torch.float32)), attn_maps, guided_maps


class _ConcatStreamsFn(torch.autograd.Function):

    @staticmethod
    def forward(ctx, x):
        from .. import ops
        return ops.interleave_streams(x).unsqueeze(0)

    @staticmethod
    def backward(ctx, g):
        from .. import ops
        return ops.interleave_streams(g[0], inverse=True)


def _concat_streams(x):
    S, B, L, d = x.shape
    if S == 2 and x.is_cuda and (d * x.element_size()) % 16 == 0:
        return _ConcatStreamsFn.apply(x)
    return x.permute(1, 2, 0, 3).reshape(1, B, L, S * d)


class MultiHeadLinearAttention(nn.Module):

    def __init__(self, d_model, nhead, d_diff=32, dropout=0.1, activation="tanh"):
        super().__init__()
        if activation != "gelu":
            raise NotImplementedError("MultiHeadLinearAttention: only activation='gelu' is implemented")
        if dropout not in (0, 0.0):
            raise NotImplementedError("MultiHeadLinearAttention: dropout must be 0 (mlha_dropout = 0)")
        self.nhead = nhead
        self.lin1 = nn.Linear(d_model, d_diff)
        self.lin2 = nn.Linear(d_diff, nhead)
        self.compute_dtype = torch.float32

    def forward(self, v, add_residual: bool = False):
        x = Fn.cast(v, self.compute_dtype)
        out = Fn.TokenGateFn.apply(x, self.lin1.weight, self.lin1.bias, self.lin2.weight, self.lin2.bias, self.nhead,
                                   add_residual)
        return Fn.cast(out, v.dtype)
```

### druglamp_amd/ops.py

```python
from __future__ import annotations

import contextlib
import ctypes as C
import math
import os
from typing import Optional

import torch

from . import _lib
from ._lib import DL_BF16, DL_F32, AttnBwdArgs, AttnFwdArgs, AttnProbsArgs, GemmArgs, PgcaPairsArgs, PgcaPairsRaggedArgs, check

_DT = {torch.float32: DL_F32, torch.bfloat16: DL_BF16}


def _dt(t: torch.Tensor) -> int:
    try:
        return _DT[t.dtype]
    except KeyError:
        raise TypeError("druglamp_amd: unsupported dtype %s (float32 / bfloat16 only)" % t.dtype)


_raw_stream = getattr(torch._C, "_cuda_getCurrentRawStream", None)
_cur_device = getattr(torch._C, "_cuda_getDevice", None)


def _stream() -> int:
    if _raw_stream is not None and _cur_device is not None:
        return _raw_stream(_cur_device())
    return torch.cuda.current_stream().cuda_stream


def _need_gpu(*ts: torch.Tensor) -> None:
    for t in ts:
        if t is not None and not t.is_cuda:
            raise RuntimeError("druglamp_amd: the HIP hot path needs device tensors (got a %s tensor); "
                               "there is no CPU fallback" % t.device)


def _ptr(t: Optional[torch.Tensor]):
    return None if t is None else t.data_ptr()


class _Workspace:

    def __init__(self):
        self.bufs = {}

    def get(self, nbytes: int, device) -> torch.Tensor:
        if device.type == "cuda" and torch.cuda.is_current_stream_capturing():
            return torch.empty(max(nbytes, 16), dtype=torch.uint8, device=device)
        key = (device.type, device.index, _stream() if device.type == "cuda" else 0)
        buf = self.bufs.get(key)
        if buf is None or buf.numel() < nbytes:
            buf = torch.empty(max(nbytes, 1 << 20), dtype=torch.uint8, device=device)
            self.bufs[key] = buf
        return buf


_ws = _Workspace()
_ws2 = _Workspace()


_prof_tag = 0


class prof_tag:
    __slots__ = ("tag", "prev")

    def __init__(self, tag: int):
        self.tag = tag

    def __enter__(self):
        global _prof_tag
        self.prev = _prof_tag
        _prof_tag = self.tag
        return self

    def __exit__(self, *exc):
        global _prof_tag
        _prof_tag = self.prev
        return False


def _gemm_args(x: torch.Tensor, w: torch.Tensor, *, M: int, N: int, K: int, x_kslow=False, w_kslow=False,
               ldx: Optional[int] = None, ldw: Optional[int] = None, bias=None, residual=None, res_row_mod=0,
               res_before_dropout=False, act=0, pre_out=None, dact_pre=None, dropout_p=0.0, seed=0, out=None,
               out_dtype=None, accumulate=False, split_k=-1, x_colsum=None, algo=0):
    _need_gpu(x, w)
    out_dtype = out_dtype or x.dtype
    if out is None:
        out = torch.empty((M, N), dtype=out_dtype, device=x.device)
    a = GemmArgs()
    a.X, a.W, a.C = x.data_ptr(), w.data_ptr(), out.data_ptr()
    a.ldx = ldx if ldx is not None else (M if x_kslow else K)
    a.ldw = ldw if ldw is not None else (N if w_kslow else K)
    a.ldc = out.stride(0) if out.dim() == 2 else N
    a.x_kslow, a.w_kslow = int(x_kslow), int(w_kslow)
    a.M, a.N, a.K = M, N, K
    a.in_dtype, a.out_dtype = _dt(x), _dt(out)
    a.bias = _ptr(bias)
    a.residual = _ptr(residual)
    a.ldr = N if residual is None else residual.stride(-2)
    a.res_row_mod = res_row_mod
    a.res_before_dropout = int(res_before_dropout)
    a.act = act
    a.pre_out = _ptr(pre_out)
    a.ldp = N
    a.dact_pre = _ptr(dact_pre)
    a.lddp = N
    a.dropout_p = float(dropout_p)
    a.dropout_seed = int(seed)
    a.accumulate = int(accumulate)
    a.split_k = split_k
    a.x_colsum = _ptr(x_colsum)
    a.dropout_seed_offset = _seed_offset_ptr(x.device) if dropout_p > 0 else None
    a.algo = algo
    a.tile_tickets = _tickets_ptr(x.device)
    a.prof_tag = _lib.TAG_WGRAD if (x_kslow and w_kslow and _prof_tag != _lib.TAG_CONV) else _prof_tag
    return a, out


def gemm(x: torch.Tensor, w: torch.Tensor, **kw) -> torch.Tensor:
    a, out = _gemm_args(x, w, **kw)
    accumulate, x_colsum = kw.get("accumulate", False), kw.get("x_colsum")
    if (_wgroup is not None and a.x_kslow and a.w_kslow and a.split_k == 0 and not accumulate
            and (a.K <= group_wgrad_max_k or a.M * a.N < group_wgrad_small_mn)
            and x.dtype == torch.bfloat16 and out.dtype == torch.float32 and a.bias is None and a.residual is None and not a.act):
        _wgroup.append((a, out, x_colsum, x, w))
        return out
    _gemm_launch(a, out, x, accumulate, x_colsum)
    return out


def _gemm_launch(a, out, x, accumulate, x_colsum) -> None:
    L = _lib.lib()
    if accumulate and (_pending or _wgroup):
        flush_reductions()
    nbytes = L.dl_gemm_workspace_bytes(C.byref(a))
    item = None
    if nbytes:
        if _pending is not None and not accumulate:
            ws = torch.empty(nbytes, dtype=torch.uint8, device=x.device)
            item = _lib.ReduceItem()
            a.deferred = C.pointer(item)
        else:
            ws = _ws.get(nbytes, x.device)
        a.workspace, a.workspace_bytes = ws.data_ptr(), ws.numel()
    check(L.dl_gemm(C.byref(a), _stream()), "dl_gemm")
    if item is not None and item.kind != 0:
        _pending.append((item, ws, out, x_colsum))


group_wgrad_max_k = int(os.environ.get("DL_GROUP_WGRAD_MAX_K", "65536"))
group_wgrad_small_mn = int(os.environ.get("DL_GROUP_WGRAD_SMALL_MN", "655360"))
group_wgrad_min_n = 2
_wgroup = None


def flush_wgrads() -> None:
    if not _wgroup:
        return
    L = _lib.lib()
    todo = list(_wgroup)
    del _wgroup[:]
    for i in range(0, len(todo), _lib.GEMM_GROUP_MAX):
        part = todo[i:i + _lib.GEMM_GROUP_MAX]
        n = len(part)
        arr = (GemmArgs * n)(*[t[0] for t in part])
        splits = (C.c_int32 * n)()
        if n < group_wgrad_min_n or L.dl_gemm_group_plan(arr, n, splits) != 0:
            for a, out, x_colsum, x, _w in part:
                _gemm_launch(a, out, x, False, x_colsum)
            continue
        keep = []
        for k, (a, out, x_colsum, x, _w) in enumerate(part):
            nbytes = int(splits[k]) * a.M * (a.N + (1 if x_colsum is not None else 0)) * 4
            ws = torch.empty(nbytes, dtype=torch.uint8, device=x.device)
            item = _lib.ReduceItem()
            arr[k].workspace, arr[k].workspace_bytes = ws.data_ptr(), nbytes
            arr[k].deferred = C.pointer(item)
            keep.append((item, ws, out, x_colsum))
        check(L.dl_gemm_group(arr, n, _stream()), "dl_gemm_group")
        _pending.extend(keep)


def gemm_pair(xs, ws, **kw):
    L = _lib.lib()
    per = [{k: (v[i] if isinstance(v, (tuple, list)) else v) for k, v in kw.items()} for i in range(2)]
    (a0, o0), (a1, o1) = _gemm_args(xs[0], ws[0], **per[0]), _gemm_args(xs[1], ws[1], **per[1])
    if L.dl_gemm_workspace_bytes(C.byref(a0)) or L.dl_gemm_workspace_bytes(C.byref(a1)):
        return gemm(xs[0], ws[0], **per[0]), gemm(xs[1], ws[1], **per[1])
    check(L.dl_gemm_pair(C.byref(a0), C.byref(a1), _stream()), "dl_gemm_pair")
    return o0, o1


_pending = None


@contextlib.contextmanager
def deferred_reductions():
    global _pending, _wgroup
    if _pending is not None:
        yield
        return
    _pending = []
    _wgroup = [] if (group_wgrad_max_k > 0 or group_wgrad_small_mn > 0) else None
    try:
        yield
    finally:
        try:
            flush_reductions()
        finally:
            _pending = None
            _wgroup = None


def flush_reductions() -> None:
    flush_wgrads()
    if not _pending:
        return
    L = _lib.lib()
    todo = list(_pending)
    del _pending[:]
    for i in range(0, len(todo), _lib.REDUCE_BATCH_MAX):
        part = todo[i:i + _lib.REDUCE_BATCH_MAX]
        arr = (_lib.ReduceItem * len(part))(*[t[0] for t in part])
        check(L.dl_reduce_batch(arr, len(part), _stream()), "dl_reduce_batch")


_tickets = {}
_tickets_on = False


def dynamic_tiles(on: bool) -> None:
    global _tickets_on
    _tickets_on = bool(on)


def reset_tickets() -> None:
    for t in _tickets.values():
        t.zero_()


def _tickets_ptr(device):
    if not _tickets_on:
        return None
    key = (device.type, device.index)
    t = _tickets.get(key)
    if t is None:
        t = _tickets[key] = torch.zeros(2, dtype=torch.int32, device=device)
    return t.data_ptr()


def colsum(x2d: torch.Tensor, out: Optional[torch.Tensor] = None, accumulate=False) -> torch.Tensor:
    _need_gpu(x2d)
    L = _lib.lib()
    M, N = x2d.shape
    if out is None:
        out = torch.empty(N, dtype=torch.float32, device=x2d.device)
    ws = _ws2.get(L.dl_colsum_workspace_bytes(M, N), x2d.device)
    check(L.dl_colsum(x2d.data_ptr(), x2d.stride(0), M, N, _dt(x2d), out.data_ptr(), int(accumulate),
                      ws.data_ptr(), ws.numel(), _stream()), "dl_colsum")
    return out


def layernorm_fwd(x2d, gamma, beta, eps):
    _need_gpu(x2d, gamma, beta)
    L = _lib.lib()
    M, D = x2d.shape
    y = torch.empty_like(x2d)
    mean = torch.empty(M, dtype=torch.float32, device=x2d.device)
    rstd = torch.empty(M, dtype=torch.float32, device=x2d.device)
    check(L.dl_layernorm_fwd(x2d.data_ptr(), x2d.stride(0), gamma.data_ptr(), beta.data_ptr(), y.data_ptr(),
                             y.stride(0), mean.data_ptr(), rstd.data_ptr(), M, D, float(eps), _dt(x2d), _stream()),
          "dl_layernorm_fwd")
    return y, mean, rstd


def layernorm_bwd(dy2d, x2d, mean, rstd, gamma, dres=None, need_param_grads=True, out=None, dy_share=1):
    L = _lib.lib()
    M, D = x2d.shape
    if dy2d.shape[0] * dy_share != M:
        raise ValueError("layernorm_bwd: dy has %d rows, x %d, dy_share %d" % (dy2d.shape[0], M, dy_share))
    dx = torch.empty_like(x2d) if out is None else out
    dgamma = dbeta = None
    if need_param_grads:
        gb = torch.empty((2, D), dtype=torch.float32, device=x2d.device)
        dgamma, dbeta = gb[0], gb[1]
    nbytes = L.dl_layernorm_bwd_workspace_bytes(M, D)
    item = None
    if _pending is not None and need_param_grads:
        ws = torch.empty(nbytes, dtype=torch.uint8, device=x2d.device)
        item = _lib.ReduceItem()
    else:
        ws = _ws.get(nbytes, x2d.device)
    check(L.dl_layernorm_bwd(dy2d.data_ptr(), dy2d.stride(0), int(dy_share), x2d.data_ptr(), x2d.stride(0), mean.data_ptr(),
                             rstd.data_ptr(), gamma.data_ptr(), _ptr(dres), 0 if dres is None else dres.stride(0),
                             dx.data_ptr(), dx.stride(0), _ptr(dgamma), _ptr(dbeta), 0, M, D, _dt(x2d),
                             ws.data_ptr(), ws.numel(), None if item is None else C.pointer(item), _stream()), "dl_layernorm_bwd")
    if item is not None and item.kind != 0:
        _pending.append((item, ws, gb, None))
    return dx, dgamma, dbeta


def cast(src: torch.Tensor, dtype: torch.dtype) -> torch.Tensor:
    if src.dtype == dtype:
        return src
    _need_gpu(src)
    src = src.contiguous()
    dst = torch.empty(src.shape, dtype=dtype, device=src.device)
    check(_lib.lib().dl_cast(src.data_ptr(), _dt(src), dst.data_ptr(), _DT[dtype], src.numel(), _stream()), "dl_cast")
    return dst


def attn_fwd(q, k, v, *, n_problems, n_heads, n_segments, partner_shift, Lq, Lk, head_dim, scale,
             q_strides, k_strides, v_strides, out, o_strides, o_ss, need_lse=True, raw_logits=None, algo=0, key_tail=None):
    _need_gpu(q, k, v, out)
    a = AttnFwdArgs()
    a.Q, a.K, a.V, a.O = q.data_ptr(), k.data_ptr(), v.data_ptr(), out.data_ptr()
    lse = None
    if need_lse:
        lse = torch.empty((n_segments, n_problems, n_heads, Lq), dtype=torch.float32, device=q.device)
    a.LSE = _ptr(lse)
    a.raw_logits = _ptr(raw_logits)
    a.q_ps, a.q_hs, a.q_rs = q_strides
    a.k_ps, a.k_hs, a.k_rs = k_strides
    a.v_ps, a.v_hs, a.v_rs = v_strides
    a.o_ps, a.o_hs, a.o_rs = o_strides
    a.o_ss = o_ss
    a.n_problems, a.n_heads, a.n_segments, a.partner_shift = n_problems, n_heads, n_segments, partner_shift
    a.Lq, a.Lk, a.head_dim, a.dtype = Lq, Lk, head_dim, _dt(q)
    a.scale = float(scale)
    a.algo = algo
    if key_tail is not None:
        a.key_tail_rows, a.key_tail_weight = int(key_tail[0]), float(key_tail[1])
    check(_lib.lib().dl_attn_fwd(C.byref(a), _stream()), "dl_attn_fwd")
    return lse


_ATTN_BWD_ALGO = int(os.environ.get("DL_ATTN_BWD_ALGO", "0"))


def attn_bwd(q, k, v, o, do, lse, *, n_problems, n_heads, n_segments, partner_shift, Lq, Lk, head_dim, scale,
             q_strides, k_strides, v_strides, o_strides, o_ss, do_strides, do_ss, dq, dq_strides, dk, dk_strides,
             dv, dv_strides, algo=0, key_tail=None):
    _need_gpu(q, k, v, o, do)
    a = AttnBwdArgs()
    delta = torch.empty_like(lse)
    a.Q, a.K, a.V, a.O, a.dO = q.data_ptr(), k.data_ptr(), v.data_ptr(), o.data_ptr(), do.data_ptr()
    a.LSE, a.Delta = lse.data_ptr(), delta.data_ptr()
    a.dQ, a.dK, a.dV = dq.data_ptr(), dk.data_ptr(), dv.data_ptr()
    a.q_ps, a.q_hs, a.q_rs = q_strides
    a.k_ps, a.k_hs, a.k_rs = k_strides
    a.v_ps, a.v_hs, a.v_rs = v_strides
    a.o_ps, a.o_hs, a.o_rs = o_strides
    a.o_ss = o_ss
    a.do_ps, a.do_hs, a.do_rs = do_strides
    a.do_ss = do_ss
    a.dq_ps, a.dq_hs, a.dq_rs = dq_strides
    a.dk_ps, a.dk_hs, a.dk_rs = dk_strides
    a.dv_ps, a.dv_hs, a.dv_rs = dv_strides
    a.n_problems, a.n_heads, a.n_segments, a.partner_shift = n_problems, n_heads, n_segments, partner_shift
    a.Lq, a.Lk, a.head_dim, a.dtype = Lq, Lk, head_dim, _dt(q)
    a.scale = float(scale)
    a.algo = algo if algo else _ATTN_BWD_ALGO
    if key_tail is not None:
        a.key_tail_rows, a.key_tail_weight = int(key_tail[0]), float(key_tail[1])
    check(_lib.lib().dl_attn_bwd(C.byref(a), _stream()), "dl_attn_bwd")


def attn_probs(q, k, *, n_problems, n_heads, n_segments, partner_shift, Lq, Lk, head_dim, scale, q_strides, k_strides,
               lse=None, head_mean=False, key_tail=None, expand_tail=False, out=None, out_ld=None):
    _need_gpu(q, k, lse, out)
    a = AttnProbsArgs()
    a.Q, a.K, a.LSE = q.data_ptr(), k.data_ptr(), _ptr(lse)
    a.q_ps, a.q_hs, a.q_rs = q_strides
    a.k_ps, a.k_hs, a.k_rs = k_strides
    a.n_problems, a.n_heads, a.n_segments, a.partner_shift = n_problems, n_heads, n_segments, partner_shift
    a.Lq, a.Lk, a.head_dim, a.dtype = Lq, Lk, head_dim, _dt(q)
    a.scale = float(scale)
    a.head_mean, a.expand_tail = int(bool(head_mean)), int(bool(expand_tail))
    cols = Lk
    if key_tail is not None:
        a.key_tail_rows, a.key_tail_weight = int(key_tail[0]), float(key_tail[1])
        if expand_tail:
            cols = Lk - int(key_tail[0]) + int(key_tail[0]) * int(key_tail[1])
    if lse is not None and (lse.dtype != torch.float32 or not lse.is_contiguous() or lse.numel() != n_segments * n_problems * n_heads * Lq):
        raise ValueError("attn_probs: lse must be a contiguous float32 tensor of (n_segments, n_problems, n_heads, Lq)")
    if out is None:
        shape = (n_segments, n_problems, Lq, cols) if head_mean else (n_segments, n_problems, n_heads, Lq, cols)
        out = torch.empty(shape, dtype=torch.float32, device=q.device)
        out_ld = cols
    else:
        rows = n_segments * n_problems * (1 if head_mean else n_heads) * Lq
        if out.dtype != torch.float32 or out_ld is None or not out.is_contiguous() or out.device != q.device:
            raise ValueError("attn_probs: out must be a contiguous float32 tensor on q's device and come with its row pitch out_ld")
        if out_ld < cols or out.numel() < (rows - 1) * int(out_ld) + cols:
            raise ValueError("attn_probs: out holds %d elements, %d rows of %d columns at pitch %d need %d"
                             % (out.numel(), rows, cols, out_ld, (rows - 1) * int(out_ld) + cols))
    a.out, a.out_ld = out.data_ptr(), int(out_ld)
    L = _lib.lib()
    if lse is None:
        ws = _ws.get(L.dl_attn_probs_workspace_bytes(C.byref(a)), q.device)
        a.workspace, a.workspace_bytes = ws.data_ptr(), ws.numel()
    check(L.dl_attn_probs(C.byref(a), _stream()), "dl_attn_probs")
    return out


def _pgca_pairs_common(who, a, q, store, store_name, store_dims, q_index, kv_index, scale, left, bias, out):
    if (q.dim() != 3 or store.dim() != len(store_dims) + 1 or q.shape[2] != 128 or store.shape[-1] != 256 or q.stride(2) != 1
            or store.stride(-1) != 1):
        raise ValueError("%s: q must be (n_q, Lq, 128) and %s (%s, 256) with contiguous columns" % (who, store_name, ", ".join(store_dims)))
    if store.dtype != q.dtype:
        raise ValueError("%s: q is %s, %s is %s" % (who, q.dtype, store_name, store.dtype))
    for t in (q_index, kv_index):
        if t.dtype != torch.int32 or t.dim() != 1 or not t.is_contiguous() or t.numel() != q_index.numel():
            raise ValueError("%s: q_index / kv_index must be contiguous int32 vectors of one length" % who)
    n_pairs, (n_q, Lq, E) = q_index.numel(), q.shape
    left_cols = 0
    if left is not None:
        if left.dim() != 3 or left.shape[:2] != q.shape[:2] or left.dtype != q.dtype or left.stride(2) != 1:
            raise ValueError("%s: left must be (n_q, Lq, cols) of q's dtype with contiguous columns" % who)
        left_cols = left.shape[2]
    if bias is not None and (bias.dtype != torch.float32 or bias.numel() != E or not bias.is_contiguous()):
        raise ValueError("%s: bias must be a contiguous float32 vector of %d" % (who, E))
    cols = left_cols + E
    if out is None:
        out = torch.empty((n_pairs, Lq, cols), dtype=q.dtype, device=q.device)
    elif (out.dim() != 3 or out.dtype != q.dtype or out.device != q.device or out.shape[0] != n_pairs or out.shape[1] != Lq
          or out.shape[2] < cols or out.stride(2) != 1 or out.stride(1) < cols or (n_pairs > 1 and out.stride(0) < (Lq - 1) * out.stride(1) + cols)):
        raise ValueError("%s: out must be a %s tensor of (%d, %d, >= %d) on q's device with contiguous columns and "
                         "non-overlapping rows (got %s, strides %s)" % (who, q.dtype, n_pairs, Lq, cols, tuple(out.shape), out.stride()))
    a.Q, a.K, a.V, a.left, a.out, a.bias = q.data_ptr(), store.data_ptr(), store.data_ptr() + E * store.element_size(), _ptr(left), out.data_ptr(), _ptr(bias)
    a.q_index, a.kv_index, a.flags = q_index.data_ptr(), kv_index.data_ptr(), guard_flags(q.device).data_ptr()
    a.q_es, a.q_rs = q.stride(0), q.stride(1)
    a.k_rs = a.v_rs = store.stride(-2)
    if left is not None:
        a.left_es, a.left_rs = left.stride(0), left.stride(1)
    a.out_ps, a.out_rs = out.stride(0), out.stride(1)
    a.n_pairs, a.n_q, a.Lq, a.head_dim, a.dtype = n_pairs, n_q, Lq, E, _dt(q)
    a.left_cols, a.out_col0 = left_cols, left_cols
    a.scale = float(scale)
    return out


def pgca_pairs(q, kv, q_index, kv_index, *, scale, left=None, bias=None, key_tail=None, out=None):
    _need_gpu(q, kv, q_index, kv_index, left, bias, out)
    a = PgcaPairsArgs()
    out = _pgca_pairs_common("pgca_pairs", a, q, kv, "kv", ("n_kv", "Lk"), q_index, kv_index, scale, left, bias, out)
    a.k_es = a.v_es = kv.stride(0)
    a.n_kv, a.Lk = kv.shape[:2]
    if key_tail is not None:
        a.key_tail_rows, a.key_tail_weight = int(key_tail[0]), float(key_tail[1])
    check(_lib.lib().dl_pgca_pairs_fwd(C.byref(a), _stream()), "dl_pgca_pairs_fwd")
    return out


def pgca_pairs_ragged(q, rows, row0, n_keys, tail_weight, q_index, kv_index, *, scale, key_tail_rows, left=None, bias=None, out=None):
    _need_gpu(q, rows, row0, n_keys, tail_weight, q_index, kv_index, left, bias, out)
    for t, dt, what in ((row0, torch.int64, "row0 int64"), (n_keys, torch.int32, "n_keys int32"), (tail_weight, torch.float32, "tail_weight float32")):
        if t.dtype != dt or t.dim() != 1 or not t.is_contiguous() or t.numel() != row0.numel() or t.device != q.device:
            raise ValueError("pgca_pairs_ragged: the key table is three contiguous vectors of one length on q's device "
                             "(row0 int64, n_keys int32, tail_weight float32); %s is %s %s" % (what, t.dtype, tuple(t.shape)))
    if int(key_tail_rows) < 0:
        raise ValueError("pgca_pairs_ragged: key_tail_rows %d is negative" % int(key_tail_rows))
    a = PgcaPairsRaggedArgs()
    out = _pgca_pairs_common("pgca_pairs_ragged", a, q, rows, "rows", ("R",), q_index, kv_index, scale, left, bias, out)
    a.kv_row0, a.kv_keys, a.kv_tail_weight = row0.data_ptr(), n_keys.data_ptr(), tail_weight.data_ptr()
    a.kv_total_rows, a.n_kv = rows.shape[0], row0.numel()
    a.key_tail_rows = int(key_tail_rows)
    check(_lib.lib().dl_pgca_pairs_ragged_fwd(C.byref(a), _stream()), "dl_pgca_pairs_ragged_fwd")
    return out


def dropout_apply(x2d: torch.Tensor, p: float, seed: int) -> torch.Tensor:
    y = torch.empty_like(x2d)
    rows, D = x2d.shape
    check(_lib.lib().dl_dropout_apply(x2d.data_ptr(), y.data_ptr(), rows, D, x2d.stride(0), y.stride(0), float(p),
                                      int(seed), _seed_offset_ptr(x2d.device), _dt(x2d), _stream()), "dl_dropout_apply")
    return y


_seed_gen = torch.Generator(device="cpu")
_seed_gen.manual_seed(0x5EED)


def manual_seed(seed: int) -> None:
    _seed_gen.manual_seed(int(seed))


_seed_offsets = {}
_seed_offset_on = False


def seed_offset_tensor(device) -> torch.Tensor:
    key = (device.type, device.index)
    t = _seed_offsets.get(key)
    if t is None:
        t = torch.zeros(1, dtype=torch.int64, device=device)
        _seed_offsets[key] = t
    return t


def use_seed_offset(on: bool) -> None:
    global _seed_offset_on
    _seed_offset_on = bool(on)


def _seed_offset_ptr(device):
    return seed_offset_tensor(device).data_ptr() if _seed_offset_on else None


def next_seed() -> int:
    return int(torch.randint(0, 2 ** 62, (1,), generator=_seed_gen).item())


def rowmod_sum(x2d: torch.Tensor, L: int) -> torch.Tensor:
    M, D = x2d.shape
    out = torch.empty((L, D), dtype=torch.float32, device=x2d.device)
    check(_lib.lib().dl_rowmod_sum(x2d.data_ptr(), out.data_ptr(), M, D, L, 0, _dt(x2d), _stream()), "dl_rowmod_sum")
    return out


def add_rowmod_dropout(x2d: torch.Tensor, pe2d: Optional[torch.Tensor], p: float, seed: int) -> torch.Tensor:
    M, D = x2d.shape
    y = torch.empty_like(x2d)
    Lr = pe2d.shape[0] if pe2d is not None else 1
    check(_lib.lib().dl_add_rowmod_dropout(x2d.data_ptr(), _ptr(pe2d), y.data_ptr(), M, D, Lr, float(p), int(seed),
                                           _seed_offset_ptr(x2d.device) if p > 0 else None, _dt(x2d), _stream()),
          "dl_add_rowmod_dropout")
    return y


def token_gate_fwd(v: torch.Tensor, logits: torch.Tensor, H: int, add_residual: bool):
    B, L, D = v.shape
    out = torch.empty_like(v)
    gate = torch.empty((B, H, L), dtype=torch.float32, device=v.device)
    check(_lib.lib().dl_token_gate_fwd(v.data_ptr(), logits.data_ptr(), out.data_ptr(), gate.data_ptr(), B, L, D, H,
                                       int(add_residual), _dt(v), _stream()), "dl_token_gate_fwd")
    return out, gate


def token_gate_bwd(dout, v, gate, H: int, add_residual: bool):
    B, L, D = v.shape
    dv = torch.empty_like(v)
    dlogits = torch.empty((B, L, H), dtype=v.dtype, device=v.device)
    check(_lib.lib().dl_token_gate_bwd(dout.data_ptr(), v.data_ptr(), gate.data_ptr(), dv.data_ptr(),
                                       dlogits.data_ptr(), B, L, D, H, int(add_residual), _dt(v), _stream()),
          "dl_token_gate_bwd")
    return dv, dlogits


def adamw_step(param, grad, exp_avg, exp_avg_sq, *, lr, beta1=0.9, beta2=0.999, eps=1e-8, weight_decay=1e-2, step,
               grad_scale=1.0, lowp=None):
    n = param.numel()
    check(_lib.lib().dl_adamw_step(param.data_ptr(), grad.data_ptr(), exp_avg.data_ptr(), exp_avg_sq.data_ptr(), n,
                                   float(lr), float(beta1), float(beta2), float(eps), float(weight_decay), int(step),
                                   float(grad_scale), _ptr(lowp), _DT[lowp.dtype] if lowp is not None else 0,
                                   _stream()), "dl_adamw_step")


def cos_rowloss_fwd(x, y):
    n, D = x.shape
    row = torch.empty(n, dtype=torch.float32, device=x.device)
    check(_lib.lib().dl_cos_rowloss_fwd(x.data_ptr(), y.data_ptr(), row.data_ptr(), None, n, D, _stream()),
          "dl_cos_rowloss_fwd")
    return row


def cos_rowloss_bwd(x, y, grad_scale: float):
    n, D = x.shape
    dx = torch.empty_like(x)
    check(_lib.lib().dl_cos_rowloss_bwd(x.data_ptr(), y.data_ptr(), float(grad_scale), dx.data_ptr(), n, D, _stream()),
          "dl_cos_rowloss_bwd")
    return dx


def ntxent_fwd(q, k, temperature: float):
    n, d = q.shape
    L = _lib.lib()
    loss = torch.empty(1, dtype=torch.float32, device=q.device)
    lse = torch.empty(2 * n, dtype=torch.float32, device=q.device)
    ws = _ws.get(L.dl_ntxent_workspace_bytes(n, d), q.device)
    check(L.dl_ntxent_fwd(q.data_ptr(), k.data_ptr(), n, d, float(temperature), loss.data_ptr(), lse.data_ptr(),
                          ws.data_ptr(), ws.numel(), _stream()), "dl_ntxent_fwd")
    return loss, lse


def ntxent_bwd(q, k, temperature: float, lse, grad_out: float):
    n, d = q.shape
    dq, dk = torch.empty_like(q), torch.empty_like(k)
    check(_lib.lib().dl_ntxent_bwd(q.data_ptr(), k.data_ptr(), n, d, float(temperature), lse.data_ptr(),
                                   float(grad_out), dq.data_ptr(), dk.data_ptr(), _stream()), "dl_ntxent_bwd")
    return dq, dk


def _ntx_args(aq, ak, bq, bk, off_a, off_b, n_global, temperature, lse_a=None, lse_b=None):
    _need_gpu(aq, ak, bq, bk)
    assert aq.dtype == ak.dtype == bq.dtype == bk.dtype and aq.dtype in (torch.float32, torch.bfloat16)
    assert aq.is_contiguous() and ak.is_contiguous() and bq.is_contiguous() and bk.is_contiguous()
    assert aq.shape == ak.shape and bq.shape == bk.shape and aq.shape[1] == bq.shape[1]
    a = _lib.NtxentArgs()
    a.a.q, a.a.k, a.a.n, a.a.gid_offset = aq.data_ptr(), ak.data_ptr(), aq.shape[0], int(off_a)
    a.b.q, a.b.k, a.b.n, a.b.gid_offset = bq.data_ptr(), bk.data_ptr(), bq.shape[0], int(off_b)
    a.a.lse = lse_a.data_ptr() if lse_a is not None else None
    a.b.lse = lse_b.data_ptr() if lse_b is not None else None
    a.n_global, a.d, a.dtype, a.temperature = int(n_global), aq.shape[1], _dt(aq), float(temperature)
    return a


def ntxent_fwd_ex(aq, ak, bq, bk, off_a: int, off_b: int, n_global: int, temperature: float):
    a = _ntx_args(aq, ak, bq, bk, off_a, off_b, n_global, temperature)
    n2 = 2 * aq.shape[0]
    loss = torch.empty(1, dtype=torch.float32, device=aq.device)
    lse = torch.empty(n2, dtype=torch.float32, device=aq.device)
    row_loss = torch.empty(n2, dtype=torch.float32, device=aq.device)
    check(_lib.lib().dl_ntxent_fwd_ex(a, lse.data_ptr(), row_loss.data_ptr(), loss.data_ptr(), _stream()), "dl_ntxent_fwd_ex")
    return loss, lse, row_loss


def ntxent_bwd_ex(aq, ak, bq, bk, off_a: int, off_b: int, n_global: int, temperature: float, lse_a, lse_b, grad_scale: float):
    a = _ntx_args(aq, ak, bq, bk, off_a, off_b, n_global, temperature, lse_a, lse_b)
    da_q = torch.empty(aq.shape, dtype=torch.float32, device=aq.device)
    da_k = torch.empty(ak.shape, dtype=torch.float32, device=aq.device)
    check(_lib.lib().dl_ntxent_bwd_ex(a, float(grad_scale), da_q.data_ptr(), da_k.data_ptr(), _stream()), "dl_ntxent_bwd_ex")
    return da_q, da_k


def triplet_sigcos_fwd(p_lats, d_lats, gt_i8, margin: float):
    n_p, dim = p_lats.shape
    n_d = d_lats.shape[0]
    L = _lib.lib()
    buf = torch.empty(L.dl_triplet_sigcos_buffer_floats(n_p, n_d), dtype=torch.float32, device=p_lats.device)
    loss = torch.empty(1, dtype=torch.float32, device=p_lats.device)
    ntri = torch.empty(1, dtype=torch.float32, device=p_lats.device)
    check(L.dl_triplet_sigcos_fwd(p_lats.data_ptr(), d_lats.data_ptr(), gt_i8.data_ptr(), n_p, n_d, dim, float(margin),
                                  buf.data_ptr(), loss.data_ptr(), ntri.data_ptr(), _stream()), "dl_triplet_sigcos_fwd")
    return loss, ntri, buf


def triplet_sigcos_bwd(p_lats, d_lats, gt_i8, margin: float, buf, ntri, grad_out: float):
    n_p, dim = p_lats.shape
    n_d = d_lats.shape[0]
    dp, dd = torch.empty_like(p_lats), torch.empty_like(d_lats)
    check(_lib.lib().dl_triplet_sigcos_bwd(p_lats.data_ptr(), d_lats.data_ptr(), gt_i8.data_ptr(), buf.data_ptr(), n_p,
                                           n_d, dim, float(margin), ntri.data_ptr(), float(grad_out), dp.data_ptr(),
                                           dd.data_ptr(), _stream()), "dl_triplet_sigcos_bwd")
    return dp, dd


def bn_stats(y2d, win, halo, valid, rw=None):
    R, Cc = y2d.shape
    L = _lib.lib()
    sums = torch.empty(2 * Cc, dtype=torch.float32, device=y2d.device)
    ws = _ws2.get(L.dl_bn_workspace_bytes(R, Cc), y2d.device)
    if rw is not None:
        check(L.dl_bn_stats_rw(y2d.data_ptr(), R, Cc, rw.data_ptr(), _dt(y2d), sums.data_ptr(), ws.data_ptr(), ws.numel(),
                               _stream()), "dl_bn_stats_rw")
        return sums
    check(L.dl_bn_stats(y2d.data_ptr(), R, Cc, win, halo, valid, _dt(y2d), sums.data_ptr(), ws.data_ptr(), ws.numel(),
                        _stream()), "dl_bn_stats")
    return sums


def bn_stats_finalize(y2d, win, halo, valid, n, eps, momentum=0.0, running_mean=None, running_var=None, rw=None):
    R, Cc = y2d.shape
    L = _lib.lib()
    out = torch.empty((3, Cc), dtype=torch.float32, device=y2d.device)
    ws = _ws2.get(L.dl_bn_workspace_bytes(R, Cc), y2d.device)
    check(L.dl_bn_stats_finalize(y2d.data_ptr(), R, Cc, win, halo, valid, _ptr(rw), _dt(y2d), int(n), float(eps), float(momentum), None,
                                 out[0].data_ptr(), out[1].data_ptr(), out[2].data_ptr(), _ptr(running_mean), _ptr(running_var),
                                 ws.data_ptr(), ws.numel(), _stream()), "dl_bn_stats_finalize")
    return out[0], out[1], out[2]


def bn_finalize(sums, n, eps, momentum=0.0, running_mean=None, running_var=None):
    Cc = sums.numel() // 2
    out = torch.empty((3, Cc), dtype=torch.float32, device=sums.device)
    check(_lib.lib().dl_bn_finalize(sums.data_ptr(), int(n), float(eps), float(momentum), out[0].data_ptr(), out[1].data_ptr(),
                                    out[2].data_ptr(), _ptr(running_mean), _ptr(running_var), Cc, _stream()), "dl_bn_finalize")
    return out[0], out[1], out[2]


def bn_apply_fwd(y2d, mean, rstd, gamma, beta, win, halo, valid, rw=None):
    R, Cc = y2d.shape
    z = torch.empty_like(y2d)
    if rw is not None:
        check(_lib.lib().dl_bn_apply_fwd_rw(y2d.data_ptr(), z.data_ptr(), mean.data_ptr(), rstd.data_ptr(), gamma.data_ptr(),
                                            beta.data_ptr(), R, Cc, rw.data_ptr(), _dt(y2d), _stream()), "dl_bn_apply_fwd_rw")
        return z
    check(_lib.lib().dl_bn_apply_fwd(y2d.data_ptr(), z.data_ptr(), mean.data_ptr(), rstd.data_ptr(), gamma.data_ptr(),
                                     beta.data_ptr(), R, Cc, win, halo, valid, _dt(y2d), _stream()), "dl_bn_apply_fwd")
    return z


def bn_bwd_reduce(dz2d, y2d, mean, rstd, win, halo, valid, rw=None):
    R, Cc = y2d.shape
    L = _lib.lib()
    sums = torch.empty(2 * Cc, dtype=torch.float32, device=y2d.device)
    ws = _ws2.get(L.dl_bn_workspace_bytes(R, Cc), y2d.device)
    if rw is not None:
        check(L.dl_bn_bwd_reduce_rw(dz2d.data_ptr(), y2d.data_ptr(), mean.data_ptr(), rstd.data_ptr(), R, Cc, rw.data_ptr(),
                                    _dt(y2d), sums.data_ptr(), ws.data_ptr(), ws.numel(), _stream()), "dl_bn_bwd_reduce_rw")
        return sums
    check(L.dl_bn_bwd_reduce(dz2d.data_ptr(), y2d.data_ptr(), mean.data_ptr(), rstd.data_ptr(), R, Cc, win, halo, valid,
                             _dt(y2d), sums.data_ptr(), ws.data_ptr(), ws.numel(), _stream()), "dl_bn_bwd_reduce")
    return sums


def bn_bwd_apply(dz2d, y2d, mean, rstd, gamma, sums, inv_n, relu_mask, win, halo, valid, rw=None):
    R, Cc = y2d.shape
    dy = torch.empty_like(y2d)
    if rw is not None:
        check(_lib.lib().dl_bn_bwd_apply_rw(dz2d.data_ptr(), y2d.data_ptr(), mean.data_ptr(), rstd.data_ptr(), gamma.data_ptr(),
                                            sums.data_ptr(), float(inv_n), int(relu_mask), dy.data_ptr(), R, Cc, rw.data_ptr(),
                                            _dt(y2d), _stream()), "dl_bn_bwd_apply_rw")
        return dy
    check(_lib.lib().dl_bn_bwd_apply(dz2d.data_ptr(), y2d.data_ptr(), mean.data_ptr(), rstd.data_ptr(), gamma.data_ptr(),
                                     sums.data_ptr(), float(inv_n), int(relu_mask), dy.data_ptr(), R, Cc, win, halo, valid,
                                     _dt(y2d), _stream()), "dl_bn_bwd_apply")
    return dy


def bn_apply_relu_fwd(y2d, mean, rstd, gamma, beta):
    R, Cc = y2d.shape
    z = torch.empty_like(y2d)
    check(_lib.lib().dl_bn_apply_relu_fwd(y2d.data_ptr(), z.data_ptr(), mean.data_ptr(), rstd.data_ptr(), gamma.data_ptr(), beta.data_ptr(),
                                          R, Cc, _dt(y2d), _stream()), "dl_bn_apply_relu_fwd")
    return z


def bn_relu_bwd(dz2d, y2d, mean, rstd, gamma, beta, inv_n):
    R, Cc = y2d.shape
    L = _lib.lib()
    dy = torch.empty_like(y2d)
    sums = torch.empty(2 * Cc, dtype=torch.float32, device=y2d.device)
    ws = _ws2.get(L.dl_bn_workspace_bytes(R, Cc), y2d.device)
    check(L.dl_bn_relu_bwd(dz2d.data_ptr(), y2d.data_ptr(), mean.data_ptr(), rstd.data_ptr(), gamma.data_ptr(), beta.data_ptr(),
                           float(inv_n), dy.data_ptr(), sums.data_ptr(), R, Cc, _dt(y2d), ws.data_ptr(), ws.numel(), _stream()),
          "dl_bn_relu_bwd")
    return dy, sums


def bn_tail_fix(dy2d, y2d, mean, rstd, gamma, sums, inv_n, w, win, lead):
    R, Cc = y2d.shape
    check(_lib.lib().dl_bn_tail_fix(dy2d.data_ptr(), y2d.data_ptr(), mean.data_ptr(), rstd.data_ptr(), gamma.data_ptr(),
                                    sums.data_ptr(), float(inv_n), int(w), R, Cc, int(win), int(lead), _dt(y2d), _stream()),
          "dl_bn_tail_fix")
    return dy2d


def ce_rows_fwd(logits2d, labels, C: int, ignore_index: int):
    _need_gpu(logits2d, labels)
    N, ld = logits2d.shape[0], logits2d.stride(0)
    L = _lib.lib()
    lse = torch.empty(N, dtype=torch.float32, device=logits2d.device)
    out2 = torch.empty(2, dtype=torch.float32, device=logits2d.device)
    ws = _ws2.get(L.dl_ce_rows_workspace_bytes(N), logits2d.device)
    check(L.dl_ce_rows_fwd(logits2d.data_ptr(), ld, labels.data_ptr(), N, C, int(ignore_index), _dt(logits2d), lse.data_ptr(),
                           out2.data_ptr(), ws.data_ptr(), ws.numel(), _stream()), "dl_ce_rows_fwd")
    return out2, lse


def ce_rows_bwd(logits2d, labels, C: int, ignore_index: int, lse, out2, grad_out):
    N, Cp = logits2d.shape
    d = torch.empty((N, Cp), dtype=logits2d.dtype, device=logits2d.device)
    check(_lib.lib().dl_ce_rows_bwd(logits2d.data_ptr(), logits2d.stride(0), labels.data_ptr(), N, C, int(ignore_index), _dt(logits2d),
                                    lse.data_ptr(), out2.data_ptr(), grad_out.data_ptr(), d.data_ptr(), Cp, Cp, _stream()), "dl_ce_rows_bwd")
    return d


def gate_dpre(dl2d, w2, pre2d):
    _need_gpu(dl2d, w2, pre2d)
    M, H = dl2d.shape
    dd = pre2d.shape[1]
    out = torch.empty_like(pre2d)
    check(_lib.lib().dl_gate_dpre(dl2d.data_ptr(), w2.data_ptr(), pre2d.data_ptr(), out.data_ptr(), M, dd, H, _dt(pre2d), _stream()),
          "dl_gate_dpre")
    return out


def gelu_bwd(dy2d, pre2d):
    dx = torch.empty_like(dy2d)
    check(_lib.lib().dl_gelu_bwd(dy2d.data_ptr(), pre2d.data_ptr(), dx.data_ptr(), dy2d.numel(), _dt(dy2d), _stream()),
          "dl_gelu_bwd")
    return dx


def fill_pool(x: torch.Tensor, site_len: int, out_dtype: torch.dtype):
    _need_gpu(x)
    x = x.contiguous()
    B, S, F = x.shape
    Fp = (F + 1 + 7) // 8 * 8
    fill = torch.empty((B, S), dtype=x.dtype, device=x.device)
    pooled = torch.empty((B, S // site_len, Fp), dtype=out_dtype, device=x.device)
    check(_lib.lib().dl_fill_pool(x.data_ptr(), fill.data_ptr(), pooled.data_ptr(), B, S, F, site_len, _dt(x),
                                  _DT[out_dtype], _stream()), "dl_fill_pool")
    return fill, pooled


_weight_prep_launches = 0


def weight_prep_launches() -> int:
    return _weight_prep_launches


def weight_prep(items_dev: torch.Tensor, block_map_dev: torch.Tensor, n_blocks: int, out_dtype: torch.dtype) -> None:
    global _weight_prep_launches
    _need_gpu(items_dev, block_map_dev)
    _weight_prep_launches += 1
    check(_lib.lib().dl_weight_prep(items_dev.data_ptr(), block_map_dev.data_ptr(), int(n_blocks), _DT[out_dtype],
                                    _stream()), "dl_weight_prep")


def cnn_sitepool_fwd(z: torch.Tensor, L: int, halo: int, site_len: int) -> torch.Tensor:
    _need_gpu(z)
    B, LP, C = z.shape
    out = torch.empty((B, L // site_len, C), dtype=z.dtype, device=z.device)
    check(_lib.lib().dl_cnn_sitepool_fwd(z.data_ptr(), out.data_ptr(), B, L, C, halo, site_len, _dt(z), _stream()),
          "dl_cnn_sitepool_fwd")
    return out


def cnn_sitepool_bwd(dpooled: torch.Tensor, L: int, halo: int, site_len: int) -> torch.Tensor:
    _need_gpu(dpooled)
    dpooled = dpooled.contiguous()
    B, _, C = dpooled.shape
    dz = torch.empty((B, L + 2 * halo, C), dtype=dpooled.dtype, device=dpooled.device)
# ... 198 lines not shown
```

### include/druglamp_hip.h

```cpp
#ifndef DRUGLAMP_HIP_H
#define DRUGLAMP_HIP_H

#include <stddef.h>
#include <stdint.h>

#ifdef __cplusplus
extern "C" {
#endif

typedef enum { DL_OK = 0, DL_ERR_ARG = -1, DL_ERR_SHAPE = -2, DL_ERR_ALIGN = -3,
               DL_ERR_WORKSPACE = -4, DL_ERR_LAUNCH = -5, DL_ERR_UNSUPPORTED = -6 } dl_status;

typedef enum { DL_F32 = 0, DL_BF16 = 1 } dl_dtype;

typedef void* dl_stream;

const char* dl_last_error(void);
int dl_version(void);

typedef struct dl_reduce_item {
  int32_t kind;
  int32_t out_dtype;
  const float* src;
  void* out;
  int64_t mn;
  int64_t ldc;
  int32_t N;
  int32_t splits;
  int32_t accumulate;
  int32_t M;
  const float* cs_slabs;
  float* cs_out;
} dl_reduce_item;
enum { DL_REDUCE_NONE = 0, DL_REDUCE_SPLITK = 1, DL_REDUCE_PARTIALS = 2 };
enum { DL_REDUCE_BATCH_MAX = 24 };
int dl_reduce_batch(const dl_reduce_item* items, int32_t n, dl_stream s);

typedef struct {
  const void* X; int64_t ldx; int32_t x_kslow;
  const void* W; int64_t ldw; int32_t w_kslow;
  void* C; int64_t ldc;
  int64_t M, N, K;
  int32_t in_dtype, out_dtype;
  const float* bias;
  const void* residual; int64_t ldr;
  int64_t res_row_mod;
  int32_t res_before_dropout;
  int32_t act;
  void* pre_out; int64_t ldp;
  const void* dact_pre; int64_t lddp;
  float dropout_p; uint64_t dropout_seed;
  int32_t accumulate;
  int32_t split_k; void* workspace; size_t workspace_bytes;
  float* x_colsum;
  const uint64_t* dropout_seed_offset;
  int32_t algo;
  int32_t* tile_tickets;
  dl_reduce_item* deferred;
  int32_t prof_tag;
} dl_gemm_args;
enum { DL_TAG_OTHER = 0, DL_TAG_QKV_OUT = 1, DL_TAG_FFN = 2, DL_TAG_CONV = 3, DL_TAG_WGRAD = 4, DL_TAG_ADAPTOR = 5 };
enum { DL_GEMM_ALGO_AUTO = 0, DL_GEMM_ALGO_TILE128 = 1 };

size_t dl_gemm_workspace_bytes(const dl_gemm_args* a);
int dl_gemm(const dl_gemm_args* a, dl_stream s);
int dl_gemm_pair(const dl_gemm_args* a, const dl_gemm_args* b, dl_stream s);
int dl_gemm_group_plan(const dl_gemm_args* args, int32_t n, int32_t* splits_out);
int dl_gemm_group(const dl_gemm_args* args, int32_t n, dl_stream s);

int dl_colsum(const void* X, int64_t ldx, int64_t M, int64_t N, int32_t dtype, float* out,
              int32_t accumulate, void* workspace, size_t workspace_bytes, dl_stream s);
size_t dl_colsum_workspace_bytes(int64_t M, int64_t N);

size_t dl_bn_workspace_bytes(int64_t R, int64_t C);
int dl_bn_stats(const void* y, int64_t R, int64_t C, int64_t win, int64_t halo, int64_t valid,
                int32_t dtype, float* sums, void* workspace, size_t workspace_bytes, dl_stream s);
int dl_bn_finalize(const float* sums, int64_t n, float eps, float momentum, float* mean, float* var, float* rstd,
                   float* running_mean, float* running_var, int64_t C, dl_stream s);
int dl_bn_apply_fwd(const void* y, void* z, const float* mean, const float* rstd, const float* gamma,
                    const float* beta, int64_t R, int64_t C, int64_t win, int64_t halo, int64_t valid,
                    int32_t dtype, dl_stream s);
int dl_bn_bwd_reduce(const void* dz, const void* y, const float* mean, const float* rstd, int64_t R,
                     int64_t C, int64_t win, int64_t halo, int64_t valid, int32_t dtype, float* sums,
                     void* workspace, size_t workspace_bytes, dl_stream s);
int dl_bn_bwd_apply(const void* dz, const void* y, const float* mean, const float* rstd,
                    const float* gamma, const float* sums, float inv_n, int32_t relu_mask, void* dy,
                    int64_t R, int64_t C, int64_t win, int64_t halo, int64_t valid, int32_t dtype,
                    dl_stream s);
int dl_bn_stats_rw(const void* y, int64_t R, int64_t C, const float* row_w, int32_t dtype, float* sums, void* workspace,
                   size_t workspace_bytes, dl_stream s);
int dl_bn_stats_finalize(const void* y, int64_t R, int64_t C, int64_t win, int64_t halo, int64_t valid, const float* row_w,
                         int32_t dtype, int64_t n, float eps, float momentum, float* sums, float* mean, float* var, float* rstd,
                         float* running_mean, float* running_var, void* workspace, size_t workspace_bytes, dl_stream s);
int dl_bn_apply_fwd_rw(const void* y, void* z, const float* mean, const float* rstd, const float* gamma, const float* beta,
                       int64_t R, int64_t C, const float* row_w, int32_t dtype, dl_stream s);
int dl_bn_bwd_reduce_rw(const void* dz, const void* y, const float* mean, const float* rstd, int64_t R, int64_t C,
                        const float* row_w, int32_t dtype, float* sums, void* workspace, size_t workspace_bytes, dl_stream s);
int dl_bn_bwd_apply_rw(const void* dz, const void* y, const float* mean, const float* rstd, const float* gamma,
                       const float* sums, float inv_n, int32_t relu_mask, void* dy, int64_t R, int64_t C, const float* row_w,
                       int32_t dtype, dl_stream s);
int dl_bn_tail_fix(void* dy, const void* y, const float* mean, const float* rstd, const float* gamma, const float* sums,
                   float inv_n, int32_t w, int64_t R, int64_t C, int64_t win, int64_t lead, int32_t dtype, dl_stream s);
int dl_bn_apply_relu_fwd(const void* y, void* z, const float* mean, const float* rstd, const float* gamma, const float* beta,
                         int64_t R, int64_t C, int32_t dtype, dl_stream s);
int dl_bn_relu_bwd(const void* dz, const void* y, const float* mean, const float* rstd, const float* gamma, const float* beta,
                   float inv_n, void* dy, float* sums, int64_t R, int64_t C, int32_t dtype, void* workspace, size_t workspace_bytes,
                   dl_stream s);

int dl_layernorm_fwd(const void* x, int64_t ldx, const float* gamma, const float* beta, void* y,
                     int64_t ldy, float* mean, float* rstd, int64_t M, int64_t D, float eps,
                     int32_t dtype, dl_stream s);
size_t dl_layernorm_bwd_workspace_bytes(int64_t M, int64_t D);
int dl_layernorm_bwd(const void* dy, int64_t lddy, int64_t dy_share, const void* x, int64_t ldx, const float* mean,
                     const float* rstd, const float* gamma, const void* dres, int64_t lddres,
                     void* dx, int64_t lddx, float* dgamma, float* dbeta, int32_t accumulate,
                     int64_t M, int64_t D, int32_t dtype, void* workspace, size_t workspace_bytes,
                     dl_reduce_item* deferred, dl_stream s);

typedef struct {
  const void* Q; const void* K; const void* V; void* O; float* LSE; float* raw_logits;
  int64_t q_ps, q_hs, q_rs, k_ps, k_hs, k_rs, v_ps, v_hs, v_rs, o_ps, o_hs, o_rs, o_ss;
  int32_t n_problems, n_heads, n_segments, partner_shift, Lq, Lk, head_dim, dtype;
  float scale;
  int32_t algo;
  int32_t key_tail_rows;
  float key_tail_weight;
} dl_attn_fwd_args;
enum { DL_ATTN_ALGO_AUTO = 0, DL_ATTN_ALGO_STREAM = 1, DL_ATTN_ALGO_TWO_PASS = 2, DL_ATTN_ALGO_ONE_PASS = 3 };
int dl_attn_fwd(const dl_attn_fwd_args* a, dl_stream s);

typedef struct {
  const void* Q; const void* K; const void* V; const void* O; const void* dO;
  const float* LSE; float* Delta;
  void* dQ; void* dK; void* dV;
  int64_t q_ps, q_hs, q_rs, k_ps, k_hs, k_rs, v_ps, v_hs, v_rs, o_ps, o_hs, o_rs, o_ss;
  int64_t do_ps, do_hs, do_rs, do_ss, dq_ps, dq_hs, dq_rs, dk_ps, dk_hs, dk_rs, dv_ps, dv_hs, dv_rs;
  int32_t n_problems, n_heads, n_segments, partner_shift, Lq, Lk, head_dim, dtype;
  float scale;
  int32_t algo;
  int32_t key_tail_rows;
  float key_tail_weight;
} dl_attn_bwd_args;
int dl_attn_bwd(const dl_attn_bwd_args* a, dl_stream s);

typedef struct {
  const void* Q; const void* K; const float* LSE; float* out; int64_t out_ld;
  int64_t q_ps, q_hs, q_rs, k_ps, k_hs, k_rs;
  int32_t n_problems, n_heads, n_segments, partner_shift, Lq, Lk, head_dim, dtype;
  float scale;
  int32_t head_mean, key_tail_rows; float key_tail_weight; int32_t expand_tail;
  void* workspace; size_t workspace_bytes;
} dl_attn_probs_args;
size_t dl_attn_probs_workspace_bytes(const dl_attn_probs_args* a);
int dl_attn_probs(const dl_attn_probs_args* a, dl_stream s);

typedef struct {
  const void* Q; const void* K; const void* V; const void* left; void* out; const float* bias;
  const int32_t* q_index; const int32_t* kv_index; uint32_t* flags;
  int64_t q_es, q_rs, k_es, k_rs, v_es, v_rs, left_es, left_rs, out_ps, out_rs;
  int32_t n_pairs, n_q, n_kv, Lq, Lk, head_dim, dtype;
  int32_t left_cols, out_col0;
  float scale;
  int32_t key_tail_rows; float key_tail_weight;
} dl_pgca_pairs_args;
int dl_pgca_pairs_fwd(const dl_pgca_pairs_args* a, dl_stream s);

typedef struct {
  const void* Q; const void* K; const void* V; const void* left; void* out; const float* bias;
  const int32_t* q_index; const int32_t* kv_index;
  const int64_t* kv_row0; const int32_t* kv_keys; const float* kv_tail_weight; uint32_t* flags;
  int64_t q_es, q_rs, k_rs, v_rs, left_es, left_rs, out_ps, out_rs, kv_total_rows;
  int32_t n_pairs, n_q, n_kv, Lq, head_dim, dtype;
  int32_t left_cols, out_col0;
  float scale;
  int32_t key_tail_rows;
} dl_pgca_pairs_ragged_args;
int dl_pgca_pairs_ragged_fwd(const dl_pgca_pairs_ragged_args* a, dl_stream s);


int dl_token_gate_fwd(const void* v, const void* logits, void* out, float* gate_out, int64_t B,
                      int64_t L, int64_t D, int32_t H, int32_t add_residual, int32_t dtype,
                      dl_stream s);
int dl_token_gate_bwd(const void* dout, const void* v, const float* gate, void* dv, void* dlogits,
                      int64_t B, int64_t L, int64_t D, int32_t H, int32_t add_residual,
                      int32_t dtype, dl_stream s);
int dl_gate_dpre(const void* dlogits, const void* w2, const void* pre, void* dpre, int64_t M, int64_t d_diff, int32_t H,
                 int32_t dtype, dl_stream s);

int dl_interleave_streams(const void* src, void* dst, int64_t R, int64_t row_bytes, int32_t S, int32_t inverse,
                          dl_stream s);
int dl_norm_adjacency(const float* adj, void* ahat, int64_t B, int32_t n, int32_t out_dtype, dl_stream s);
int dl_graph_aggregate(const void* ahat, const void* feat, void* out, int64_t B, int32_t n, int32_t N, int32_t C,
                       int32_t transpose, int32_t dtype, dl_stream s);
int dl_concat2(void* a, void* b, void* cat, int64_t R, int64_t a_row_bytes, int64_t b_row_bytes, int32_t inverse,
               dl_stream s);

int dl_add_rowmod_dropout(const void* x, const void* pe, void* y, int64_t M, int64_t D,
                          int64_t L, float p, uint64_t seed, const uint64_t* seed_offset, int32_t dtype, dl_stream s);
int dl_dropout_apply(const void* x, void* y, int64_t n_rows, int64_t D, int64_t ldx, int64_t ldy,
                     float p, uint64_t seed, const uint64_t* seed_offset, int32_t dtype, dl_stream s);
int dl_fill_pool(const void* x, void* fill, void* pooled, int64_t B, int64_t S, int64_t F, int32_t site_len,
                 int32_t in_dtype, int32_t out_dtype, dl_stream s);
int dl_gelu_bwd(const void* dy, const void* pre, void* dx, int64_t n, int32_t dtype, dl_stream s);
int dl_cast(const void* src, int32_t src_dtype, void* dst, int32_t dst_dtype, int64_t n,
            dl_stream s);
int dl_gather_pad(const void* store, const int64_t* offsets, const int32_t* lengths, void* out, int64_t B,
                  int64_t S, int64_t F, int32_t repeat, int32_t dtype, dl_stream s);
int dl_embed_pad(const int64_t* ids, const void* weight, const void* fill, void* out, int64_t B, int64_t L,
                 int32_t V, int32_t D, int32_t halo, int32_t dtype, dl_stream s);
enum { DL_FLAG_PROT_PERIOD = 1, DL_FLAG_DRUG_TOKEN_PAD = 2, DL_FLAG_GCN_NODE_PAD = 4, DL_FLAG_PLAN_ROWS = 8,
       DL_FLAG_PAIR_INDEX = 16 ,
       DL_FLAG_KEY_TABLE = 32  };
int dl_embed_rows(const int64_t* ids, const void* weight, const void* fill, const int32_t* src, void* out, int64_t R,
                  int32_t V, int32_t D, const int32_t* period, int64_t B, int64_t L, uint32_t* flags, int32_t dtype, dl_stream s);
int dl_rows_gather(const void* src, const int32_t* index, void* out, int64_t N, int64_t row_bytes, dl_stream s);
int dl_rows_sum_strided(const void* x, const int32_t* rep, void* out, int64_t R, int64_t C, int32_t dtype, dl_stream s);
int dl_rows_equal_check(const void* x, int64_t B, int64_t N, int64_t row_bytes, int64_t row0, uint32_t code, uint32_t* flags,
                        dl_stream s);
int dl_protein_plan_build(const int32_t* lengths, int64_t B, int64_t S, int64_t R, int32_t* src, float* w, int32_t* rep,
                          int32_t* row_of, int32_t* period, uint32_t* flags, dl_stream s);
int dl_cnn_sitepool_fwd(const void* z, void* pooled, int64_t B, int64_t L, int64_t C, int32_t halo,
                        int32_t site_len, int32_t dtype, dl_stream s);
int dl_cnn_sitepool_bwd(const void* dpooled, void* dz, int64_t B, int64_t L, int64_t C, int32_t halo,
                        int32_t site_len, int32_t dtype, dl_stream s);
int dl_cnn_sitepool_rows_fwd(const void* z, const int32_t* row_of, void* pooled, int64_t B, int64_t L, int64_t C,
                             int32_t site_len, int32_t dtype, dl_stream s);
int dl_cnn_sitepool_rows_bwd(const void* dpooled, const int32_t* rep, const int32_t* row_of, void* dz, int64_t B, int64_t L,
                             int64_t C, int64_t R, int32_t site_len, int32_t dtype, dl_stream s);
typedef struct dl_wprep_item {
  const float* src;
  void* dst;
  int64_t ld;
  int32_t rows, cols;
  int32_t row0;
  int32_t transpose;
  int64_t cs;
} dl_wprep_item;
int dl_weight_prep(const dl_wprep_item* items_dev, const int32_t* block_map_dev, int32_t n_blocks,
                   int32_t out_dtype, dl_stream s);
int dl_rowmod_sum(const void* x, float* out, int64_t M, int64_t D, int64_t L, int32_t accumulate,
                  int32_t dtype, dl_stream s);

int dl_cos_rowloss_fwd(const float* x, const float* y, float* row_loss, float* loss_sum,
                       int64_t n_rows, int64_t D, dl_stream s);
int dl_cos_rowloss_bwd(const float* x, const float* y, float grad_scale, float* dx, int64_t n_rows,
                       int64_t D, dl_stream s);
size_t dl_ce_rows_workspace_bytes(int64_t N);
int dl_ce_rows_fwd(const void* logits, int64_t ld, const int64_t* labels, int64_t N, int32_t C, int64_t ignore_index, int32_t dtype,
                   float* lse, float* out2, void* workspace, size_t workspace_bytes, dl_stream s);
int dl_ce_rows_bwd(const void* logits, int64_t ld, const int64_t* labels, int64_t N, int32_t C, int64_t ignore_index, int32_t dtype,
                   const float* lse, const float* out2, const float* grad_out, void* dlogits, int64_t ldd, int32_t Cp, dl_stream s);
typedef struct dl_ntxent_side {
  const void* q;
  const void* k;
  int64_t n;
  int64_t gid_offset;
  const float* lse;
} dl_ntxent_side;
typedef struct dl_ntxent_args {
  dl_ntxent_side a, b;
  int64_t n_global;
  int64_t d;
  int32_t dtype;
  float temperature;
} dl_ntxent_args;
int dl_ntxent_fwd_ex(const dl_ntxent_args* a, float* row_lse, float* row_loss, float* loss, dl_stream s);
int dl_ntxent_bwd_ex(const dl_ntxent_args* a, float grad_scale, float* da_q, float* da_k, dl_stream s);
size_t dl_ntxent_workspace_bytes(int64_t n, int64_t d);
int dl_ntxent_fwd(const float* q, const float* k, int64_t n, int64_t d, float temperature,
                  float* loss, float* row_lse, void* workspace, size_t workspace_bytes,
                  dl_stream s);
int dl_ntxent_bwd(const float* q, const float* k, int64_t n, int64_t d, float temperature,
                  const float* row_lse, float grad_out, float* dq, float* dk, dl_stream s);
size_t dl_triplet_sigcos_buffer_floats(int64_t n_p, int64_t n_d);
int dl_triplet_sigcos_fwd(const float* p_lats, const float* d_lats, const int8_t* gt, int64_t n_p,
                          int64_t n_d, int64_t dim, float margin, float* dist, float* loss,
                          float* n_tri, dl_stream s);
int dl_triplet_sigcos_bwd(const float* p_lats, const float* d_lats, const int8_t* gt,
                          const float* dist, int64_t n_p, int64_t n_d, int64_t dim, float margin,
                          const float* n_tri, float grad_out, float* dp, float* dd, dl_stream s);

int dl_adamw_step(float* param, const float* grad, float* exp_avg, float* exp_avg_sq, int64_t n,
                  float lr, float beta1, float beta2, float eps, float weight_decay, int64_t step,
                  float grad_scale, void* param_lowp, int32_t lowp_dtype, dl_stream s);

int dl_prof_enable(int32_t family, int32_t on);
int dl_prof_collect(int32_t family, int64_t* launches, double* total_ms, double* total_flops,
                    double* total_bytes);
int dl_prof_totals(int32_t family, int64_t* launches, double* total_flops, double* total_bytes);
int dl_prof_collect_tag(int32_t family, int32_t tag, int64_t* timed_launches, double* timed_ms, double* timed_flops,
                        double* timed_bytes, int64_t* all_launches, double* all_flops, double* all_bytes);

#ifdef __cplusplus
}
#endif
#endif
```

Before: 21070 pairs/s.

## Fuse PMMA encoder into single autograd node with masked-dropout LayerNorm backward

```diff
diff --git a/druglamp_amd/_lib.py b/druglamp_amd/_lib.py
--- a/druglamp_amd/_lib.py
+++ b/druglamp_amd/_lib.py
@@ -26,6 +26,10 @@
         ("N", c_i32), ("splits", c_i32), ("accumulate", c_i32), ("M", c_i32),
         ("cs_slabs", c_vp), ("cs_out", c_vp),
     ]
+
+
+class LnMask(C.Structure):
+    _fields_ = [("out", c_vp), ("ld", c_i64), ("p", c_f32), ("seed", c_u64), ("seed_offset", c_vp)]
 
 
 REDUCE_BATCH_MAX = 24
@@ -172,6 +176,8 @@
     "dl_layernorm_bwd_workspace_bytes": (c_sz, [c_i64, c_i64]),
     "dl_layernorm_bwd": (c_i32, [c_vp, c_i64, c_i64, c_vp, c_i64, c_vp, c_vp, c_vp, c_vp, c_i64, c_vp, c_i64, c_vp, c_vp,
                                  c_i32, c_i64, c_i64, c_i32, c_vp, c_sz, C.POINTER(ReduceItem), c_vp]),
+    "dl_layernorm_bwd_masked": (c_i32, [c_vp, c_i64, c_i64, c_vp, c_i64, c_vp, c_vp, c_vp, c_vp, c_i64, c_vp, c_i64, c_vp, c_vp,
+                                        c_i32, c_i64, c_i64, c_i32, c_vp, c_sz, C.POINTER(ReduceItem), C.POINTER(LnMask), c_i32, c_vp]),
     "dl_attn_fwd": (c_i32, [C.POINTER(AttnFwdArgs), c_vp]),
     "dl_attn_bwd": (c_i32, [C.POINTER(AttnBwdArgs), c_vp]),
     "dl_attn_probs_workspace_bytes": (c_sz, [C.POINTER(AttnProbsArgs)]),
diff --git a/druglamp_amd/csrc/norm.hip b/druglamp_amd/csrc/norm.hip
--- a/druglamp_amd/csrc/norm.hip
+++ b/druglamp_amd/csrc/norm.hip
@@ -3,6 +3,22 @@
 namespace {
 constexpr int LN_MAXV = 8;
 constexpr int LN_BWD_ROWS = 32;
+
+struct LnMask {
+  void* out[2];
+  int64_t ld[2];
+  uint64_t seed[2];
+  const uint64_t* seed_off[2];
+  uint32_t thr16[2];
+  float inv_keep[2];
+  int32_t nseg;
+};
+template <typename T> __device__ __forceinline__ f32x4 round4(f32x4 v);
+template <> __device__ __forceinline__ f32x4 round4<float>(f32x4 v) { return v; }
+template <> __device__ __forceinline__ f32x4 round4<bf16_t>(f32x4 v) {
+  const uint32_t a = pack_bf16x2(v[0], v[1]), b = pack_bf16x2(v[2], v[3]);
+  return f32x4{bf16lo(a), bf16hi(a), bf16lo(b), bf16hi(b)};
+}
 
 constexpr int LN_FWD_RPW = 2;
 template <typename T, int NV_>
@@ -68,7 +84,7 @@
   }
 }
 
-template <typename T, int NV_>
+template <typename T, int NV_, bool MASKED>
 __global__ __launch_bounds__(256) void ln_bwd_kernel(const T* __restrict__ dy, int64_t lddy, int64_t dy_share,
                                                      const T* __restrict__ x, int64_t ldx,
                                                      const float* __restrict__ mean,
@@ -76,7 +92,7 @@
                                                      const float* __restrict__ gamma,
                                                      const T* __restrict__ dres, int64_t lddres,
                                                      T* __restrict__ dx, int64_t lddx,
-                                                     float* __restrict__ partial, int64_t M, int D) {
+                                                     float* __restrict__ partial, int64_t M, int D, LnMask mk) {
   extern __shared__ __attribute__((aligned(16))) char ln_smem[];
   float* sm = reinterpret_cast<float*>(ln_smem);
   const int lane = threadIdx.x & 63, wave = threadIdx.x >> 6;
@@ -88,6 +104,13 @@
     dg[j] = f32x4{0.f, 0.f, 0.f, 0.f};
     db[j] = f32x4{0.f, 0.f, 0.f, 0.f};
     gm[j] = (c < nv) ? *reinterpret_cast<const f32x4*>(gamma + c * 4) : f32x4{0.f, 0.f, 0.f, 0.f};
+  }
+  uint64_t mseed0 = 0, mseed1 = 0;
+  int W = D;
+  if constexpr (MASKED) {
+    W = D / mk.nseg;
+    mseed0 = dl_eff_seed(mk.seed[0], mk.seed_off[0]);
+    if (mk.nseg > 1) mseed1 = dl_eff_seed(mk.seed[1], mk.seed_off[1]);
   }
   const int64_t r0 = (int64_t)blockIdx.x * LN_BWD_ROWS;
   for (int rr = wave; rr < LN_BWD_ROWS; rr += 8) {
@@ -145,7 +168,16 @@
 #pragma unroll
           for (int e = 0; e < 4; ++e) o[e] = rs * (g[j][e] - c1 - xh[j][e] * c2);
           o += half == 0 ? ra[j] : rb[j];
-          store4<T>(dx + row * lddx + c * 4, o);
+          if constexpr (MASKED) {
+            if (dx) store4<T>(dx + row * lddx + c * 4, o);
+            const bool sg = c * 4 >= W;
+            const int lc = sg ? c * 4 - W : c * 4;
+            const f32x4 m = dl_dropout4_idx(round4<T>(o), sg ? mseed1 : mseed0, ((uint64_t)row * (uint64_t)W + (uint64_t)lc) >> 2,
+                                            sg ? mk.thr16[1] : mk.thr16[0], sg ? mk.inv_keep[1] : mk.inv_keep[0]);
+            store4<T>(reinterpret_cast<T*>(sg ? mk.out[1] : mk.out[0]) + row * (sg ? mk.ld[1] : mk.ld[0]) + lc, m);
+          } else {
+            store4<T>(dx + row * lddx + c * 4, o);
+          }
         }
       }
     }
@@ -233,12 +265,12 @@
   }
 }
 
-template <int D>
+template <int D, bool MASKED>
 __global__ __launch_bounds__(256) void ln_bwd16_kernel(const bf16_t* __restrict__ dy, int64_t lddy, int64_t dy_share,
                                                        const bf16_t* __restrict__ x, int64_t ldx, const float* __restrict__ mean,
                                                        const float* __restrict__ rstd, const float* __restrict__ gamma,
                                                        const bf16_t* __restrict__ dres, int64_t lddres, bf16_t* __restrict__ dx,
-                                                       int64_t lddx, float* __restrict__ partial, int64_t M) {
+                                                       int64_t lddx, float* __restrict__ partial, int64_t M, LnMask mk) {
   constexpr int LPR = D / 8, RPP = 64 / LPR, P = LN16_PASSES, NIT = LN_BWD_ROWS / (4 * RPP * P);
   static_assert(NIT >= 1 && NIT * 4 * RPP * P == LN_BWD_ROWS, "a workgroup covers LN_BWD_ROWS rows");
   __shared__ __attribute__((aligned(16))) float sm[4 * RPP * 2 * D];
@@ -249,6 +281,20 @@
     for (int e = 0; e < 4; ++e) { gm[e] = a[e]; gm[4 + e] = b[e]; } }
 #pragma unroll
   for (int e = 0; e < 8; ++e) { dg[e] = 0.f; db[e] = 0.f; }
+  bf16_t* mout = nullptr;
+  int64_t mld = 0;
+  uint64_t mseed = 0;
+  uint32_t mthr = 0;
+  float minv = 1.f;
+  int mW = D, mlc = 0;
+  if constexpr (MASKED) {
+    mW = D / mk.nseg;
+    const bool sg = cl * 8 >= mW;
+    mlc = sg ? cl * 8 - mW : cl * 8;
+    mout = reinterpret_cast<bf16_t*>(sg ? mk.out[1] : mk.out[0]); mld = sg ? mk.ld[1] : mk.ld[0];
+    mseed = sg ? dl_eff_seed(mk.seed[1], mk.seed_off[1]) : dl_eff_seed(mk.seed[0], mk.seed_off[0]);
+    mthr = sg ? mk.thr16[1] : mk.thr16[0]; minv = sg ? mk.inv_keep[1] : mk.inv_keep[0];
+  }
 #pragma unroll 1
   for (int it = 0; it < NIT; ++it) {
     const int64_t row0 = (int64_t)blockIdx.x * LN_BWD_ROWS + (it * 4 + wave) * (RPP * P) + sub;
@@ -290,7 +336,19 @@
         unpack8(wr[q], rv);
 #pragma unroll
         for (int e = 0; e < 8; ++e) o[e] = rs[q] * (g[e] - c1 - xv[e] * c2) + rv[e];
-        store16_fam<1>(dx + row * lddx + cl * 8, pack8(o));
+        if constexpr (MASKED) {
+          const u32x4 pk = pack8(o);
+          if (dx) store16_fam<1>(dx + row * lddx + cl * 8, pk);
+          float ob[8];
+          unpack8(pk, ob);
+          const uint64_t grp = ((uint64_t)row * (uint64_t)mW + (uint64_t)mlc) >> 2;
+          const f32x4 m0 = dl_dropout4_idx(f32x4{ob[0], ob[1], ob[2], ob[3]}, mseed, grp, mthr, minv);
+          const f32x4 m1 = dl_dropout4_idx(f32x4{ob[4], ob[5], ob[6], ob[7]}, mseed, grp + 1, mthr, minv);
+          const float om[8] = {m0[0], m0[1], m0[2], m0[3], m1[0], m1[1], m1[2], m1[3]};
+          store16_fam<1>(mout + row * mld + mlc, pack8(om));
+        } else {
+          store16_fam<1>(dx + row * lddx + cl * 8, pack8(o));
+        }
       }
     }
   }
@@ -356,32 +414,61 @@
                                 const void* dres, int64_t lddres, void* dx, int64_t lddx, float* dgamma,
                                 float* dbeta, int32_t accumulate, int64_t M, int64_t D, int32_t dtype,
                                 void* workspace, size_t workspace_bytes, dl_reduce_item* deferred, dl_stream stream) {
+  return dl_layernorm_bwd_masked(dy, lddy, dy_share, x, ldx, mean, rstd, gamma, dres, lddres, dx, lddx, dgamma, dbeta, accumulate, M, D,
+                                 dtype, workspace, workspace_bytes, deferred, nullptr, 0, stream);
+}
+
+extern "C" int dl_layernorm_bwd_masked(const void* dy, int64_t lddy, int64_t dy_share, const void* x, int64_t ldx,
+                                       const float* mean, const float* rstd, const float* gamma,
+                                       const void* dres, int64_t lddres, void* dx, int64_t lddx, float* dgamma,
+                                       float* dbeta, int32_t accumulate, int64_t M, int64_t D, int32_t dtype,
+                                       void* workspace, size_t workspace_bytes, dl_reduce_item* deferred,
+                                       const dl_ln_mask* masks, int32_t nseg, dl_stream stream) {
   hipStream_t s = (hipStream_t)stream;
   if (deferred) deferred->kind = DL_REDUCE_NONE;
-  DL_CHECK_ARG(dy && x && mean && rstd && gamma && dx, DL_ERR_ARG, "dl_layernorm_bwd: null pointer");
+  DL_CHECK_ARG(nseg >= 0 && nseg <= 2 && (nseg == 0 || masks), DL_ERR_ARG, "dl_layernorm_bwd: nseg=%d must be 0, 1 or 2", (int)nseg);
+  DL_CHECK_ARG(dy && x && mean && rstd && gamma && (dx || nseg > 0), DL_ERR_ARG, "dl_layernorm_bwd: null pointer");
   DL_CHECK_ARG(dy_share >= 1, DL_ERR_ARG, "dl_layernorm_bwd: dy_share=%ld must be >= 1", (long)dy_share);
   DL_CHECK_ARG(M > 0 && D > 0 && D % 4 == 0 && D <= 256 * LN_MAXV, DL_ERR_SHAPE,
                "dl_layernorm_bwd: D=%ld must be a multiple of 4 and <= %d", (long)D, 256 * LN_MAXV);
   DL_CHECK_ARG(workspace && workspace_bytes >= dl_layernorm_bwd_workspace_bytes(M, D),
                DL_ERR_WORKSPACE, "dl_layernorm_bwd: workspace too small");
+  LnMask mk = {};
+  mk.nseg = nseg;
+  bool m16 = true;
+  if (nseg > 0) {
+    DL_CHECK_ARG(D % (4 * nseg) == 0, DL_ERR_SHAPE, "dl_layernorm_bwd: D=%ld must be a multiple of %d for %d masked outputs", (long)D,
+                 4 * nseg, (int)nseg);
+    const int64_t W = D / nseg;
+    for (int j = 0; j < nseg; ++j) {
+      DL_CHECK_ARG(masks[j].out && masks[j].ld >= W && masks[j].ld % 4 == 0, DL_ERR_ARG, "dl_layernorm_bwd: bad masked output %d", j);
+      DL_CHECK_ARG(masks[j].p >= 0.f && masks[j].p < 1.f, DL_ERR_ARG, "dl_layernorm_bwd: masked output %d: p must be in [0,1)", j);
+      mk.out[j] = masks[j].out; mk.ld[j] = masks[j].ld; mk.seed[j] = masks[j].seed; mk.seed_off[j] = masks[j].seed_offset;
+      mk.thr16[j] = masks[j].p > 0.f ? dl_dropout_thr16(masks[j].p) : 0u;
+      mk.inv_keep[j] = masks[j].p > 0.f ? 1.0f / (1.0f - masks[j].p) : 1.0f;
+      m16 = m16 && masks[j].ld % 8 == 0 && ((uintptr_t)masks[j].out & 15) == 0;
+    }
+    m16 = m16 && W % 8 == 0;
+  }
   const int nb = (int)((M + LN_BWD_ROWS - 1) / LN_BWD_ROWS);
   const size_t smem = 4 * 2 * (size_t)D * sizeof(float);
-#define LN_BWD(TT, NVV) hipLaunchKernelGGL((ln_bwd_kernel<TT, NVV>), dim3(nb), dim3(256), smem, s, (const TT*)dy, lddy, dy_share, \
-                                          (const TT*)x, ldx, mean, rstd, gamma, (const TT*)dres, lddres, (TT*)dx, lddx, \
-                                          (float*)workspace, M, (int)D)
+#define LN_BWD_(TT, NVV, MK) hipLaunchKernelGGL((ln_bwd_kernel<TT, NVV, MK>), dim3(nb), dim3(256), smem, s, (const TT*)dy, lddy, dy_share, \
+                                               (const TT*)x, ldx, mean, rstd, gamma, (const TT*)dres, lddres, (TT*)dx, lddx, \
+                                               (float*)workspace, M, (int)D, mk)
+#define LN_BWD(TT, NVV) do { if (nseg > 0) LN_BWD_(TT, NVV, true); else LN_BWD_(TT, NVV, false); } while (0)
+#define LN_BWD16(DD, MK) hipLaunchKernelGGL((ln_bwd16_kernel<DD, MK>), dim3(nb), dim3(256), 0, s, (const bf16_t*)dy, lddy, dy_share, \
+                                            (const bf16_t*)x, ldx, mean, rstd, gamma, (const bf16_t*)dres, lddres, (bf16_t*)dx, lddx, \
+                                            (float*)workspace, M, mk)
   const int nvg = (int)((D + 255) / 256);
-  const bool v16 = dtype == DL_BF16 && (D == 256 || D == 512) && lddy % 8 == 0 && ldx % 8 == 0 && lddx % 8 == 0 &&
+  const bool v16 = dtype == DL_BF16 && (D == 256 || D == 512) && lddy % 8 == 0 && ldx % 8 == 0 && lddx % 8 == 0 && m16 &&
                    (!dres || lddres % 8 == 0) && (((uintptr_t)dy | (uintptr_t)x | (uintptr_t)dx | (uintptr_t)dres | (uintptr_t)gamma) & 15) == 0;
-  if (v16 && D == 256)
-    hipLaunchKernelGGL((ln_bwd16_kernel<256>), dim3(nb), dim3(256), 0, s, (const bf16_t*)dy, lddy, dy_share, (const bf16_t*)x, ldx, mean, rstd,
-                       gamma, (const bf16_t*)dres, lddres, (bf16_t*)dx, lddx, (float*)workspace, M);
-  else if (v16)
-    hipLaunchKernelGGL((ln_bwd16_kernel<512>), dim3(nb), dim3(256), 0, s, (const bf16_t*)dy, lddy, dy_share, (const bf16_t*)x, ldx, mean, rstd,
-                       gamma, (const bf16_t*)dres, lddres, (bf16_t*)dx, lddx, (float*)workspace, M);
-  else
-  if (dtype == DL_BF16) { if (nvg <= 1) LN_BWD(bf16_t, 1); else if (nvg <= 2) LN_BWD(bf16_t, 2); else if (nvg <= 4) LN_BWD(bf16_t, 4); else LN_BWD(bf16_t, 8); }
+  if (v16 && D == 256) { if (nseg > 0) LN_BWD16(256, true); else LN_BWD16(256, false); }
+  else if (v16) { if (nseg > 0) LN_BWD16(512, true); else LN_BWD16(512, false); }
+  else if (dtype == DL_BF16) { if (nvg <= 1) LN_BWD(bf16_t, 1); else if (nvg <= 2) LN_BWD(bf16_t, 2); else if (nvg <= 4) LN_BWD(bf16_t, 4); else LN_BWD(bf16_t, 8); }
   else { if (nvg <= 1) LN_BWD(float, 1); else if (nvg <= 2) LN_BWD(float, 2); else if (nvg <= 4) LN_BWD(float, 4); else LN_BWD(float, 8); }
+#undef LN_BWD16
 #undef LN_BWD
+#undef LN_BWD_
   DL_CHECK_LAUNCH("dl_layernorm_bwd");
   if (dgamma && dbeta == dgamma + D && deferred) {
     dl_reduce_item& it = *deferred;
diff --git a/druglamp_amd/functional.py b/druglamp_amd/functional.py
--- a/druglamp_amd/functional.py
+++ b/druglamp_amd/functional.py
@@ -209,123 +209,137 @@
     return [ops.gemm(xs[0], ws[0], **{k: (v[0] if isinstance(v, (tuple, list)) else v) for k, v in kw.items()})]
 
 
+def _block_forward(x, outs, paired, H, p_drop, training, eps, params):
+    S, B, L, d = x.shape
+    assert S == (2 if paired else 1)
+    cdt = x.dtype
+    M = B * L
+    npar = _n_params(paired)
+    streams = [_Stream(params[s * npar:(s + 1) * npar], paired, cdt) for s in range(S)]
+    xs = [x[s].reshape(M, d) for s in range(S)]
+    nseg = 2 if paired else 1
+    hd = d // H
+    p_eff = float(p_drop) if (training and p_drop > 0) else 0.0
+
+    qkv = torch.empty((S, M, 3 * d), dtype=cdt, device=x.device)
+    xn, stats1 = [], []
+    for s, st in enumerate(streams):
+        y, mean, rstd = ops.layernorm_fwd(xs[s], st.ln1w.detach(), st.ln1b.detach(), eps)
+        xn.append(y)
+        stats1.append((mean, rstd))
+    with ops.prof_tag(_TAG_QKV_OUT):
+        _gemm_s(xn, [st.qkv_w for st in streams], M=M, N=3 * d, K=d, bias=[st.qkv_b for st in streams],
+                out=[qkv[s] for s in range(S)])
+    a = torch.empty((S, M, nseg * d), dtype=cdt, device=x.device)
+    qs = (L * 3 * d, hd, 3 * d)
+    os_ = (L * nseg * d, hd, nseg * d)
+    lse = ops.attn_fwd(qkv, qkv[..., d:], qkv[..., 2 * d:], n_problems=S * B, n_heads=H, n_segments=nseg,
+                       partner_shift=B if paired else 0, Lq=L, Lk=L, head_dim=hd, scale=1.0 / math.sqrt(hd),
+                       q_strides=qs, k_strides=qs, v_strides=qs, out=a, o_strides=os_, o_ss=d)
+    saved: List[torch.Tensor] = [x, qkv, a, lse]
+    seeds = [((ops.next_seed(), ops.next_seed()) if p_eff > 0 else (0, 0)) for _ in range(S)]
+    with ops.prof_tag(_TAG_QKV_OUT):
+        if paired:
+            f = _gemm_s([a[s] for s in range(S)], [st.fc_w for st in streams], M=M, N=d, K=2 * d, bias=[st.fc_b for st in streams])
+        else:
+            f = [a[s] for s in range(S)]
+        x1 = _gemm_s(f, [st.out_w for st in streams], M=M, N=d, K=d, bias=[st.out_b for st in streams], residual=xs)
+    ln2 = [ops.layernorm_fwd(x1[s], st.ln2w.detach(), st.ln2b.detach(), eps) for s, st in enumerate(streams)]
+    hn = [t[0] for t in ln2]
+    pre = [torch.empty((M, 4 * d), dtype=cdt, device=x.device) for _ in range(S)]
+    with ops.prof_tag(_TAG_FFN):
+        act = _gemm_s(hn, [st.w1 for st in streams], M=M, N=4 * d, K=d, bias=[st.b1 for st in streams], act=1, pre_out=pre,
+                      dropout_p=p_eff, seed=[sd[0] for sd in seeds])
+        _gemm_s(act, [st.w2 for st in streams], M=M, N=d, K=4 * d, bias=[st.b2 for st in streams], dropout_p=p_eff,
+                seed=[sd[1] for sd in seeds], residual=x1, out=list(outs))
+    for s, st in enumerate(streams):
+        saved += [xn[s], stats1[s][0], stats1[s][1], f[s], x1[s], hn[s], ln2[s][1], ln2[s][2], pre[s], act[s],
+                  st.qkv_wT, st.out_wT, st.w1T, st.w2T, st.fc_wT if paired else st.out_wT,
+                  st.ln1w.detach(), st.ln2w.detach()]
+    return saved, (paired, H, p_eff, S, B, L, d, seeds)
+
+
+def _block_backward(sv, cfg, dys, g2=None, emit=None, want_dx=True):
+    paired, H, p_eff, S, B, L, d, seeds = cfg
+    x, qkv, a, lse = sv[:4]
+    per = 17
+    M = B * L
+    nseg = 2 if paired else 1
+    hd = d // H
+    da = torch.empty_like(a)
+    SV = [sv[4 + s * per: 4 + (s + 1) * per] for s in range(S)]
+    col = lambda i: [SV[s][i] for s in range(S)]
+    (xn_, _m1, _r1, f_, x1_, hn_, mean2_, rstd2_, pre_, act_, qkvw_, outw_, w1_, w2_, fcw_, _l1, ln2w_) = [col(i) for i in range(per)]
+    if g2 is None:
+        g2 = [ops.dropout_apply(dys[s], p_eff, seeds[s][1]) if p_eff > 0 else dys[s] for s in range(S)]
+    wg2 = [_wgrad(g2[s], act_[s], d, 4 * d, M, d, 4 * d) for s in range(S)]
+    with ops.prof_tag(_TAG_FFN):
+        g1 = _gemm_s(g2, w2_, M=M, N=4 * d, K=d, dact_pre=pre_, dropout_p=p_eff, seed=[seeds[s][0] for s in range(S)])
+        wg1 = [_wgrad(g1[s], hn_[s], 4 * d, d, M, 4 * d, d) for s in range(S)]
+        dhn = _gemm_s(g1, w1_, M=M, N=d, K=4 * d)
+    lnb = [ops.layernorm_bwd(dhn[s], x1_[s], mean2_[s], rstd2_[s], ln2w_[s], dres=dys[s]) for s in range(S)]
+    dx1_all = [t[0] for t in lnb]
+    wgo = [_wgrad(dx1_all[s], f_[s], d, d, M, d, d) for s in range(S)]
+    grads_tail = []
+    _tag_qo = ops.prof_tag(_TAG_QKV_OUT)
+    _tag_qo.__enter__()
+    if paired:
+        df = _gemm_s(dx1_all, outw_, M=M, N=d, K=d)
+        wgf = [_wgrad(df[s], a[s], d, 2 * d, M, d, 2 * d) for s in range(S)]
+        _gemm_s(df, fcw_, M=M, N=2 * d, K=d, out=[da[s] for s in range(S)])
+        for s in range(S):
+            grads_tail.append((wgf[s][0], wgf[s][1], wgo[s][0], wgo[s][1], lnb[s][1], lnb[s][2], wg1[s][0], wg1[s][1],
+                               wg2[s][0], wg2[s][1]))
+    else:
+        _gemm_s(dx1_all, outw_, M=M, N=d, K=d, out=[da[s] for s in range(S)])
+        for s in range(S):
+            grads_tail.append((wgo[s][0], wgo[s][1], lnb[s][1], lnb[s][2], wg1[s][0], wg1[s][1], wg2[s][0], wg2[s][1]))
+    _tag_qo.__exit__(None, None, None)
+    dqkv = torch.empty_like(qkv)
+    qs = (L * 3 * d, hd, 3 * d)
+    os_ = (L * nseg * d, hd, nseg * d)
+    ops.attn_bwd(qkv, qkv[..., d:], qkv[..., 2 * d:], a, da, lse, n_problems=S * B, n_heads=H, n_segments=nseg,
+                 partner_shift=B if paired else 0, Lq=L, Lk=L, head_dim=hd, scale=1.0 / math.sqrt(hd),
+                 q_strides=qs, k_strides=qs, v_strides=qs, o_strides=os_, o_ss=d, do_strides=os_, do_ss=d,
+                 dq=dqkv, dq_strides=qs, dk=dqkv[..., d:], dk_strides=qs, dv=dqkv[..., 2 * d:], dv_strides=qs)
+    dx = torch.empty_like(x) if want_dx else None
+    masked = [None] * S
+    out_grads: List[Optional[torch.Tensor]] = []
+    wgq = [_wgrad(dqkv[s], xn_[s], 3 * d, d, M, 3 * d, d) for s in range(S)]
+    with ops.prof_tag(_TAG_QKV_OUT):
+        dxn = _gemm_s([dqkv[s] for s in range(S)], qkvw_, M=M, N=d, K=3 * d)
+    for s in range(S):
+        dwqkv, dbqkv = wgq[s]
+        if emit is None:
+            _, dg1, dbt1 = ops.layernorm_bwd(dxn[s], x[s].reshape(M, d), SV[s][1], SV[s][2], SV[s][15], dres=dx1_all[s],
+                                             out=dx[s].reshape(M, d))
+        else:
+            _, dg1, dbt1, masked[s] = ops.layernorm_bwd(dxn[s], x[s].reshape(M, d), SV[s][1], SV[s][2], SV[s][15], dres=dx1_all[s],
+                                                        out=dx[s].reshape(M, d) if want_dx else None, masked=emit[s], want_dx=want_dx)
+        out_grads += [dg1, dbt1, dwqkv[0:d], dbqkv[0:d], dwqkv[d:2 * d], dbqkv[d:2 * d], dwqkv[2 * d:],
+                      dbqkv[2 * d:]]
+        out_grads += list(grads_tail[s])
+    return dx, masked, tuple(out_grads)
+
+
 class TransformerBlockFn(torch.autograd.Function):
 
     @staticmethod
     def forward(ctx, x, paired, H, p_drop, training, eps, *params):
         S, B, L, d = x.shape
-        assert S == (2 if paired else 1)
-        cdt = x.dtype
-        M = B * L
-        npar = _n_params(paired)
-        streams = [_Stream(params[s * npar:(s + 1) * npar], paired, cdt) for s in range(S)]
         x = x.contiguous()
-        xs = [x[s].reshape(M, d) for s in range(S)]
-        nseg = 2 if paired else 1
-        hd = d // H
-        p_eff = float(p_drop) if (training and p_drop > 0) else 0.0
-
-        qkv = torch.empty((S, M, 3 * d), dtype=cdt, device=x.device)
-        xn, stats1 = [], []
-        for s, st in enumerate(streams):
-            y, mean, rstd = ops.layernorm_fwd(xs[s], st.ln1w.detach(), st.ln1b.detach(), eps)
-            xn.append(y)
-            stats1.append((mean, rstd))
-        with ops.prof_tag(_TAG_QKV_OUT):
-            _gemm_s(xn, [st.qkv_w for st in streams], M=M, N=3 * d, K=d, bias=[st.qkv_b for st in streams],
-                    out=[qkv[s] for s in range(S)])
-        a = torch.empty((S, M, nseg * d), dtype=cdt, device=x.device)
-        qs = (L * 3 * d, hd, 3 * d)
-        os_ = (L * nseg * d, hd, nseg * d)
-        lse = ops.attn_fwd(qkv, qkv[..., d:], qkv[..., 2 * d:], n_problems=S * B, n_heads=H, n_segments=nseg,
-                           partner_shift=B if paired else 0, Lq=L, Lk=L, head_dim=hd, scale=1.0 / math.sqrt(hd),
-                           q_strides=qs, k_strides=qs, v_strides=qs, out=a, o_strides=os_, o_ss=d)
         out = torch.empty_like(x)
-        saved: List[torch.Tensor] = [x, qkv, a, lse]
-        seeds = [((ops.next_seed(), ops.next_seed()) if p_eff > 0 else (0, 0)) for _ in range(S)]
-        with ops.prof_tag(_TAG_QKV_OUT):
-            if paired:
-                f = _gemm_s([a[s] for s in range(S)], [st.fc_w for st in streams], M=M, N=d, K=2 * d, bias=[st.fc_b for st in streams])
-            else:
-                f = [a[s] for s in range(S)]
-            x1 = _gemm_s(f, [st.out_w for st in streams], M=M, N=d, K=d, bias=[st.out_b for st in streams], residual=xs)
-        ln2 = [ops.layernorm_fwd(x1[s], st.ln2w.detach(), st.ln2b.detach(), eps) for s, st in enumerate(streams)]
-        hn = [t[0] for t in ln2]
-        pre = [torch.empty((M, 4 * d), dtype=cdt, device=x.device) for _ in range(S)]
-        with ops.prof_tag(_TAG_FFN):
-            act = _gemm_s(hn, [st.w1 for st in streams], M=M, N=4 * d, K=d, bias=[st.b1 for st in streams], act=1, pre_out=pre,
-                          dropout_p=p_eff, seed=[sd[0] for sd in seeds])
-            _gemm_s(act, [st.w2 for st in streams], M=M, N=d, K=4 * d, bias=[st.b2 for st in streams], dropout_p=p_eff,
-                    seed=[sd[1] for sd in seeds], residual=x1, out=[out[s].reshape(M, d) for s in range(S)])
-        for s, st in enumerate(streams):
-            saved += [xn[s], stats1[s][0], stats1[s][1], f[s], x1[s], hn[s], ln2[s][1], ln2[s][2], pre[s], act[s],
-                      st.qkv_wT, st.out_wT, st.w1T, st.w2T, st.fc_wT if paired else st.out_wT,
-                      st.ln1w.detach(), st.ln2w.detach()]
+        saved, ctx.cfg = _block_forward(x, [out[s].reshape(B * L, d) for s in range(S)], paired, H, p_drop, training, eps, params)
         ctx.save_for_backward(*saved)
-        ctx.cfg = (paired, H, p_eff, S, B, L, d, seeds)
         return out
 
     @staticmethod
     @_deferring
     def backward(ctx, dout):
-        paired, H, p_eff, S, B, L, d, seeds = ctx.cfg
-        sv = ctx.saved_tensors
-        x, qkv, a, lse = sv[:4]
-        per = 17
-        M = B * L
-        nseg = 2 if paired else 1
-        hd = d // H
-        cdt = x.dtype
+        S, B, L, d = ctx.cfg[3:7]
         dout = dout.contiguous()
-        da = torch.empty_like(a)
-        SV = [sv[4 + s * per: 4 + (s + 1) * per] for s in range(S)]
-        col = lambda i: [SV[s][i] for s in range(S)]
-        (xn_, _m1, _r1, f_, x1_, hn_, mean2_, rstd2_, pre_, act_, qkvw_, outw_, w1_, w2_, fcw_, _l1, ln2w_) = [col(i) for i in range(per)]
-        dys = [dout[s].reshape(M, d) for s in range(S)]
-        g2 = [ops.dropout_apply(dys[s], p_eff, seeds[s][1]) if p_eff > 0 else dys[s] for s in range(S)]
-        wg2 = [_wgrad(g2[s], act_[s], d, 4 * d, M, d, 4 * d) for s in range(S)]
-        with ops.prof_tag(_TAG_FFN):
-            g1 = _gemm_s(g2, w2_, M=M, N=4 * d, K=d, dact_pre=pre_, dropout_p=p_eff, seed=[seeds[s][0] for s in range(S)])
-            wg1 = [_wgrad(g1[s], hn_[s], 4 * d, d, M, 4 * d, d) for s in range(S)]
-            dhn = _gemm_s(g1, w1_, M=M, N=d, K=4 * d)
-        lnb = [ops.layernorm_bwd(dhn[s], x1_[s], mean2_[s], rstd2_[s], ln2w_[s], dres=dys[s]) for s in range(S)]
-        dx1_all = [t[0] for t in lnb]
-        wgo = [_wgrad(dx1_all[s], f_[s], d, d, M, d, d) for s in range(S)]
-        grads_tail = []
-        _tag_qo = ops.prof_tag(_TAG_QKV_OUT)
-        _tag_qo.__enter__()
-        if paired:
-            df = _gemm_s(dx1_all, outw_, M=M, N=d, K=d)
-            wgf = [_wgrad(df[s], a[s], d, 2 * d, M, d, 2 * d) for s in range(S)]
-            _gemm_s(df, fcw_, M=M, N=2 * d, K=d, out=[da[s] for s in range(S)])
-            for s in range(S):
-                grads_tail.append((wgf[s][0], wgf[s][1], wgo[s][0], wgo[s][1], lnb[s][1], lnb[s][2], wg1[s][0], wg1[s][1],
-                                   wg2[s][0], wg2[s][1]))
-        else:
-            _gemm_s(dx1_all, outw_, M=M, N=d, K=d, out=[da[s] for s in range(S)])
-            for s in range(S):
-                grads_tail.append((wgo[s][0], wgo[s][1], lnb[s][1], lnb[s][2], wg1[s][0], wg1[s][1], wg2[s][0], wg2[s][1]))
-        _tag_qo.__exit__(None, None, None)
-        dqkv = torch.empty_like(qkv)
-        qs = (L * 3 * d, hd, 3 * d)
-        os_ = (L * nseg * d, hd, nseg * d)
-        ops.attn_bwd(qkv, qkv[..., d:], qkv[..., 2 * d:], a, da, lse, n_problems=S * B, n_heads=H, n_segments=nseg,
-                     partner_shift=B if paired else 0, Lq=L, Lk=L, head_dim=hd, scale=1.0 / math.sqrt(hd),
-                     q_strides=qs, k_strides=qs, v_strides=qs, o_strides=os_, o_ss=d, do_strides=os_, do_ss=d,
-                     dq=dqkv, dq_strides=qs, dk=dqkv[..., d:], dk_strides=qs, dv=dqkv[..., 2 * d:], dv_strides=qs)
-        dx = torch.empty_like(x)
-        out_grads: List[Optional[torch.Tensor]] = []
-        wgq = [_wgrad(dqkv[s], xn_[s], 3 * d, d, M, 3 * d, d) for s in range(S)]
-        with ops.prof_tag(_TAG_QKV_OUT):
-            dxn = _gemm_s([dqkv[s] for s in range(S)], qkvw_, M=M, N=d, K=3 * d)
-        for s in range(S):
-            dwqkv, dbqkv = wgq[s]
-            _, dg1, dbt1 = ops.layernorm_bwd(dxn[s], x[s].reshape(M, d), SV[s][1], SV[s][2], SV[s][15], dres=dx1_all[s],
-                                             out=dx[s].reshape(M, d))
-            out_grads += [dg1, dbt1, dwqkv[0:d], dbqkv[0:d], dwqkv[d:2 * d], dbqkv[d:2 * d], dwqkv[2 * d:],
-                          dbqkv[2 * d:]]
-            out_grads += list(grads_tail[s])
-        return (dx, None, None, None, None, None) + tuple(out_grads)
+        dx, _, grads = _block_backward(ctx.saved_tensors, ctx.cfg, [dout[s].reshape(B * L, d) for s in range(S)])
+        return (dx, None, None, None, None, None) + grads
 
 
 def transformer_block(x, paired: bool, H: int, p_drop: float, training: bool, eps: float, params):
@@ -424,6 +438,127 @@
 
 def layer_norm(x, weight, bias, eps):
     return LayerNormFn.apply(x, weight, bias, eps)
+
+
+def pmma_node_enabled() -> bool:
+    return os.environ.get("DL_PMMA_NODE", "1") != "0"
+
+
+class PMMAEncoderFn(torch.autograd.Function):
+
+    @staticmethod
+    def forward(ctx, prot, mol, H, p_drop, training, mol_w, mol_b, pe_mol, pe_prot, norm_w, norm_b, *params):
+        cdt = prot.dtype
+        B, L, d = prot.shape
+        M = B * L
+        N, K = mol_w.shape[0], mol.shape[-1]
+        assert N == d and K == d
+        n_paired = min(len(params) // (2 * _n_params(True)), 2)
+        n = n_paired + (len(params) - n_paired * 2 * _n_params(True)) // _n_params(False)
+        assert n >= 1 and n_paired >= 1
+        p_eff = float(p_drop) if (training and p_drop > 0) else 0.0
+        x = torch.empty((2, B, L, d), dtype=cdt, device=prot.device)
+        mol2 = mol.reshape(M, K).contiguous()
+        w = lowp((mol_w,), cdt)
+        wT = lowp((mol_w,), cdt, transpose=True) if (ctx.needs_input_grad[1] and cdt == torch.bfloat16 and N % 8 == 0) else None
+        seed_mol = ops.next_seed() if p_eff > 0 else 0
+        pe2 = lowp((pe_mol,), cdt).reshape(-1, N)
+        ops.gemm(mol2, w, M=M, N=N, K=K, bias=_f32(mol_b), residual=pe2, res_row_mod=pe2.shape[0], res_before_dropout=True,
+                 dropout_p=p_eff, seed=seed_mol, out=x[1].reshape(M, d))
+        seed_prot = ops.next_seed() if p_eff > 0 else 0
+        ops.add_rowmod_dropout(prot.reshape(M, d).contiguous(), lowp((pe_prot,), cdt).reshape(-1, d), p_eff, seed_prot,
+                               out=x[0].reshape(M, d))
+        saved: List[Optional[torch.Tensor]] = []
+        blocks = []
+        pos = 0
+        for i in range(n):
+            paired = i < n_paired
+            cnt = (2 if paired else 1) * _n_params(paired)
+            if paired and i == n_paired - 1:
+                nxt = torch.empty((1, B, L, 2 * d), dtype=cdt, device=prot.device)
+                c2 = nxt.view(M, 2 * d)
+                outs = [c2[:, :d], c2[:, d:]]
+            elif paired:
+                nxt = torch.empty((2, B, L, d), dtype=cdt, device=prot.device)
+                outs = [nxt[s].reshape(M, d) for s in range(2)]
+            else:
+                nxt = torch.empty((1, B, L, 2 * d), dtype=cdt, device=prot.device)
+                outs = [nxt.view(M, 2 * d)]
+            sv, cfg = _block_forward(x, outs, paired, H, p_drop, training, 1e-6, params[pos:pos + cnt])
+            blocks.append((cfg, len(sv)))
+            saved += sv
+            pos += cnt
+            x = nxt
+        xl = x.view(M, 2 * d)
+        y, mean, rstd = ops.layernorm_fwd(xl, norm_w.detach(), norm_b.detach(), 1e-6)
+        ctx.save_for_backward(mol2, w, wT, xl, mean, rstd, norm_w.detach(), *saved)
+        ctx.cfg = (B, L, d, p_eff, seed_mol, seed_prot, n_paired, blocks, tuple(prot.shape), tuple(mol.shape), tuple(pe_mol.shape),
+                   tuple(pe_prot.shape))
+        return y.reshape(B, L, 2 * d)
+
+    @staticmethod
+    def backward(ctx, dy):
+        B, L, d, p, seed_mol, seed_prot, n_paired, blocks, prot_shape, mol_shape, pe_mol_shape, pe_prot_shape = ctx.cfg
+        sv = ctx.saved_tensors
+        mol2, w, wT, xl, mean, rstd, nw = sv[:7]
+        M, n = B * L, len(blocks)
+        bsv, pos = [], 7
+        for _, cnt in blocks:
+            bsv.append(sv[pos:pos + cnt])
+            pos += cnt
+        seeds = [cfg[7] for cfg, _ in blocks]
+
+        def spec(c, wide):
+            if c >= n_paired:
+                return ([[(p, seeds[c][0][1])]], True) if p > 0 else (None, True)
+            if wide:
+                return ([[(p, seeds[c][0][1]), (p, seeds[c][1][1])]], True) if p > 0 else ([[(0.0, 0), (0.0, 0)]], False)
+            if c >= 0:
+                return ([[(p, seeds[c][s][1])] for s in range(2)], True) if p > 0 else (None, True)
+            return ([[(p, seed_prot)], [(p, seed_mol)]], False) if p > 0 else (None, True)
+
+        def hand_over(c, wide, dx, masked):
+            if c >= n_paired:
+                return [dx.view(M, 2 * d)], ([masked[0][0]] if p > 0 else None)
+            if wide:
+                if p > 0:
+                    d2 = dx.view(M, 2 * d)
+                    return [d2[:, :d], d2[:, d:]], list(masked[0])
+                return list(masked[0]), None
+            return [dx[s].reshape(M, d) for s in range(2)], ([masked[s][0] for s in range(2)] if p > 0 else None)
+
+        emit, want_dx = spec(n - 1, True)
+        kw = dict(masked=emit[0], want_dx=want_dx) if emit is not None else {}
+        if dy.dim() == 3 and dy.stride(1) == 0 and dy.stride(2) == 1 and dy.shape[1] > 1:
+            res = ops.layernorm_bwd(dy[:, 0], xl, mean, rstd, nw, dy_share=dy.shape[1], **kw)
+        else:
+            res = ops.layernorm_bwd(dy.reshape(xl.shape).contiguous(), xl, mean, rstd, nw, **kw)
+        dx, dnw, dnb = res[:3]
+        masked = [res[3]] if emit is not None else None
+        grads = [None] * n
+        for i in range(n - 1, -1, -1):
+            wide = i >= n_paired
+            dys, g2 = hand_over(i, i == n - 1 or i + 1 >= n_paired, dx, masked)
+            emit, want_dx = spec(i - 1, wide)
+            with _maybe_deferring():
+                dx, masked, grads[i] = _block_backward(bsv[i], blocks[i][0], dys, g2, emit=emit, want_dx=want_dx)
+        g = [masked[s][0] for s in range(2)] if p > 0 else [dx[s].reshape(M, d) for s in range(2)]
+        N = K = d
+        dmol = None
+        if ctx.needs_input_grad[1]:
+            dmol = (ops.gemm(g[1], wT, M=M, N=K, K=N) if wT is not None
+                    else ops.gemm(g[1], w, M=M, N=K, K=N, w_kslow=True, ldw=K)).reshape(mol_shape)
+        want_b = ctx.needs_input_grad[6]
+        if ctx.needs_input_grad[5]:
+            dw, db = _wgrad(g[1], mol2, N, K, M, N, K, want_bias=want_b)
+        else:
+            dw, db = None, (ops.colsum(g[1]) if want_b else None)
+        dpe_mol = ops.rowmod_sum(g[1], pe_mol_shape[-2]).reshape(pe_mol_shape) if ctx.needs_input_grad[7] else None
+        dpe_prot = ops.rowmod_sum(g[0], pe_prot_shape[-2]).reshape(pe_prot_shape) if ctx.needs_input_grad[8] else None
+        out = (g[0].reshape(prot_shape), dmol, None, None, None, dw, db, dpe_mol, dpe_prot, dnw, dnb)
+        for gr in grads:
+            out += gr
+        return out
 
 
 class GuidedCrossAttentionFn(torch.autograd.Function):
diff --git a/druglamp_amd/model/PMMA.py b/druglamp_amd/model/PMMA.py
--- a/druglamp_amd/model/PMMA.py
+++ b/druglamp_amd/model/PMMA.py
@@ -124,6 +124,15 @@
         H, p, tr = self.num_heads, self.p_drop, self.training
         prot = Fn.cast(prot, cdt)
         mol = Fn.cast(mol, cdt)
+        n = len(enc.layer_with_mol)
+        if (not self.vis and n >= 1 and prot.is_cuda and Fn.pmma_node_enabled()
+                and (prot.shape[-1] * prot.element_size()) % 16 == 0):
+            params = []
+            for i, blk in enumerate(enc.layer_with_mol):
+                params += blk.stream_params(0) + (blk.stream_params(1) if i < 2 else [])
+            encoded = Fn.PMMAEncoderFn.apply(prot, mol, H, p, tr, emb.mol_embeddings.weight, emb.mol_embeddings.bias, emb.pe_mol,
+                                             emb.pe_prot, enc.encoder_norm.weight, enc.encoder_norm.bias, *params)
+            return (encoded if self.keep_compute_dtype else Fn.cast(encoded, torch.float32)), [], []
         mol = Fn.LinearFn.apply(mol, emb.mol_embeddings.weight, emb.mol_embeddings.bias, emb.pe_mol, p, tr)
         prot = Fn.AddPeDropoutFn.apply(prot, emb.pe_prot, p, tr)
         x = torch.stack((prot, mol), dim=0)
diff --git a/druglamp_amd/ops.py b/druglamp_amd/ops.py
--- a/druglamp_amd/ops.py
+++ b/druglamp_amd/ops.py
@@ -278,12 +278,15 @@
     return y, mean, rstd
 
 
-def layernorm_bwd(dy2d, x2d, mean, rstd, gamma, dres=None, need_param_grads=True, out=None, dy_share=1):
+def layernorm_bwd(dy2d, x2d, mean, rstd, gamma, dres=None, need_param_grads=True, out=None, dy_share=1, masked=None,
+                  want_dx=True, masked_out=None):
     L = _lib.lib()
     M, D = x2d.shape
     if dy2d.shape[0] * dy_share != M:
         raise ValueError("layernorm_bwd: dy has %d rows, x %d, dy_share %d" % (dy2d.shape[0], M, dy_share))
-    dx = torch.empty_like(x2d) if out is None else out
+    if not want_dx and not masked:
+        raise ValueError("layernorm_bwd: want_dx=False needs at least one masked output")
+    dx = None if not want_dx else (torch.empty_like(x2d) if out is None else out)
     dgamma = dbeta = None
     if need_param_grads:
         gb = torch.empty((2, D), dtype=torch.float32, device=x2d.device)
@@ -295,13 +298,29 @@
         item = _lib.ReduceItem()
     else:
         ws = _ws.get(nbytes, x2d.device)
-    check(L.dl_layernorm_bwd(dy2d.data_ptr(), dy2d.stride(0), int(dy_share), x2d.data_ptr(), x2d.stride(0), mean.data_ptr(),
-                             rstd.data_ptr(), gamma.data_ptr(), _ptr(dres), 0 if dres is None else dres.stride(0),
-                             dx.data_ptr(), dx.stride(0), _ptr(dgamma), _ptr(dbeta), 0, M, D, _dt(x2d),
-                             ws.data_ptr(), ws.numel(), None if item is None else C.pointer(item), _stream()), "dl_layernorm_bwd")
+    args = (dy2d.data_ptr(), dy2d.stride(0), int(dy_share), x2d.data_ptr(), x2d.stride(0), mean.data_ptr(),
+            rstd.data_ptr(), gamma.data_ptr(), _ptr(dres), 0 if dres is None else dres.stride(0),
+            _ptr(dx), 0 if dx is None else dx.stride(0), _ptr(dgamma), _ptr(dbeta), 0, M, D, _dt(x2d),
+            ws.data_ptr(), ws.numel(), None if item is None else C.pointer(item))
+    gms = None
+    if masked:
+        n = len(masked)
+        if n > 2 or D % (4 * n):
+            raise ValueError("layernorm_bwd: %d masked outputs over D=%d" % (n, D))
+        W = D // n
+        gms = list(masked_out) if masked_out is not None else [torch.empty((M, W), dtype=x2d.dtype, device=x2d.device) for _ in range(n)]
+        arr = (_lib.LnMask * n)()
+        for j, (p, seed) in enumerate(masked):
+            if tuple(gms[j].shape) != (M, W) or gms[j].stride(1) != 1 or gms[j].dtype != x2d.dtype:
+                raise ValueError("layernorm_bwd: masked output %d must be a (%d, %d) %s tensor" % (j, M, W, x2d.dtype))
+            arr[j].out, arr[j].ld, arr[j].p, arr[j].seed = gms[j].data_ptr(), gms[j].stride(0), float(p), int(seed)
+            arr[j].seed_offset = _seed_offset_ptr(x2d.device) if p > 0 else None
+        check(L.dl_layernorm_bwd_masked(*args, arr, n, _stream()), "dl_layernorm_bwd_masked")
+    else:
+        check(L.dl_layernorm_bwd(*args, _stream()), "dl_layernorm_bwd")
     if item is not None and item.kind != 0:
         _pending.append((item, ws, gb, None))
-    return dx, dgamma, dbeta
+    return (dx, dgamma, dbeta, gms) if masked else (dx, dgamma, dbeta)
 
 
 def cast(src: torch.Tensor, dtype: torch.dtype) -> torch.Tensor:
@@ -523,9 +542,11 @@
     return out
 
 
-def add_rowmod_dropout(x2d: torch.Tensor, pe2d: Optional[torch.Tensor], p: float, seed: int) -> torch.Tensor:
+def add_rowmod_dropout(x2d: torch.Tensor, pe2d: Optional[torch.Tensor], p: float, seed: int, out: Optional[torch.Tensor] = None) -> torch.Tensor:
     M, D = x2d.shape
-    y = torch.empty_like(x2d)
+    y = torch.empty_like(x2d) if out is None else out
+    if tuple(y.shape) != (M, D) or not y.is_contiguous() or y.dtype != x2d.dtype:
+        raise ValueError("add_rowmod_dropout: out must be a contiguous (%d, %d) %s tensor" % (M, D, x2d.dtype))
     Lr = pe2d.shape[0] if pe2d is not None else 1
     check(_lib.lib().dl_add_rowmod_dropout(x2d.data_ptr(), _ptr(pe2d), y.data_ptr(), M, D, Lr, float(p), int(seed),
                                            _seed_offset_ptr(x2d.device) if p > 0 else None, _dt(x2d), _stream()),
diff --git a/include/druglamp_hip.h b/include/druglamp_hip.h
--- a/include/druglamp_hip.h
+++ b/include/druglamp_hip.h
@@ -116,6 +116,18 @@
                      void* dx, int64_t lddx, float* dgamma, float* dbeta, int32_t accumulate,
                      int64_t M, int64_t D, int32_t dtype, void* workspace, size_t workspace_bytes,
                      dl_reduce_item* deferred, dl_stream s);
+typedef struct dl_ln_mask {
+  void* out;
+  int64_t ld;
+  float p;
+  uint64_t seed;
+  const uint64_t* seed_offset;
+} dl_ln_mask;
+int dl_layernorm_bwd_masked(const void* dy, int64_t lddy, int64_t dy_share, const void* x, int64_t ldx, const float* mean,
+                            const float* rstd, const float* gamma, const void* dres, int64_t lddres,
+                            void* dx, int64_t lddx, float* dgamma, float* dbeta, int32_t accumulate,
+                            int64_t M, int64_t D, int32_t dtype, void* workspace, size_t workspace_bytes,
+                            dl_reduce_item* deferred, const dl_ln_mask* masks, int32_t nseg, dl_stream s);
 
 typedef struct {
   const void* Q; const void* K; const void* V; void* O; float* LSE; float* raw_logits;
```

New measurement: 21380 pairs/s (median of 6 runs). 1.5% higher.
